# nellogrb/MultigridAnisotropicDiffusion

Measured on AMD Instinct MI355X. Metric: Mvoxel-smooths/s (and V-cycles/s) at 512^3 fp32; achieved HBM GB/s vs peak, higher is better.
Workload: dtype f32

## Files before the change

include/mad.h:

```cpp
#ifndef MAD_H
#define MAD_H

#include <stddef.h>
#include <stdint.h>

#ifdef __cplusplus
extern "C" {
#endif

#define MAD_ABI_VERSION 1

typedef enum mad_status {
  MAD_OK = 0,
  MAD_ERR_INVALID = 1,
  MAD_ERR_STATE = 2,
  MAD_ERR_DEVICE = 3,
  MAD_ERR_COMM = 4,
  MAD_ERR_SINGULAR = 5,
  MAD_ERR_UNSUPPORTED = 6,
  MAD_ERR_NOMEM = 7,
  MAD_ERR_NUMERIC = 8,
  MAD_ERR_NOT_CONVERGED = 9
} mad_status;

// ... 17 lines not shown
#define MAD_REFINE_SWITCH_RELRES 1e-5
#define MAD_REFINE_FP32_MIN_RATE 0.5
#define MAD_MIN_SLAB_PLANES 4
#define MAD_MIN_SLAB_VOXELS 131072
#define MAD_COARSE_DENSE_MAX 8192
#define MAD_COARSE_BLOCK_UNKNOWNS 2048
#define MAD_COARSE_DENSE_LIMIT 16384

typedef enum mad_tensor_kind {
  MAD_TENSOR_AUTO = 0,
  MAD_TENSOR_ISOTROPIC = 1,
  MAD_TENSOR_DIAGONAL = 2,
  MAD_TENSOR_FULL = 3
} mad_tensor_kind;

typedef enum mad_which { MAD_X = 0 , MAD_B = 1 , MAD_R = 2  } mad_which;

typedef struct mad_desc {
  uint32_t abi_version;
  int32_t dim;
  int64_t size[3];
  double spacing[3];
  int32_t cycle;
  int32_t smoother;
  uint32_t iterations_per_grid;
  uint32_t max_cycles;
  uint32_t number_of_steps;
  double time_step;
  double tolerance;
  double omega;
  int32_t verbose;
  int32_t precision;
  int32_t stall_guard;
  int32_t device;
  int32_t tensor_kind;
  int32_t nranks;
  int32_t rank;
  int32_t gs_kernel;
  uint32_t options;
  int32_t min_slab_planes;
  int32_t min_slab_voxels;
  int32_t coarse_dense_max;
  int32_t coarse_block_unknowns;
  int32_t reserved[3];
} mad_desc;

#define MAD_OPT_EAGER_RANK_VCYCLE 1u
#define MAD_OPT_OVERLAP_RANK_SWEEP 2u
#define MAD_OPT_PEER_HALO 4u
#define MAD_OPT_COARSE_NO_CHAIN 8u
#define MAD_OPT_BENCHMARK_TRACE 16u
#define MAD_OPT_NO_PLACEMENT_TUNE 32u
#define MAD_OPT_NO_RECORD_B 64u

typedef struct mad_stats {
  uint32_t steps;
  uint32_t total_cycles;
  uint32_t last_cycles;
  int32_t stalled;
  double last_relres;
  double setup_ms;
  double solve_ms;
  uint32_t num_levels;
  int32_t tensor_kind;
  int32_t colors;
  int32_t reserved[5];
} mad_stats;

typedef struct mad_ctx mad_ctx;

int mad_desc_init(mad_desc *d);
int mad_max_depth(int32_t dim, const int64_t size[3]);
int mad_create(const mad_desc *d, mad_ctx **out);
void mad_destroy(mad_ctx *ctx);
const char *mad_last_error(const mad_ctx *ctx);
int mad_get_desc(const mad_ctx *ctx, mad_desc *out);

int mad_set_tensor(mad_ctx *ctx, const void *host_aos, int32_t dtype);
int mad_set_tensor_device(mad_ctx *ctx, const void *dev_aos, int32_t dtype);
int mad_tensor_planes(const mad_ctx *ctx, int64_t *first_plane, int64_t *nplanes);
int mad_set_tensor_planes(mad_ctx *ctx, const void *host_aos, int32_t dtype,
                          int64_t first_plane, int64_t nplanes);

int mad_setup(mad_ctx *ctx);

int mad_run(mad_ctx *ctx, const void *host_in, int32_t in_dtype, void *host_out,
            int32_t out_dtype, mad_stats *stats);
int mad_run_device(mad_ctx *ctx, const void *dev_in, int32_t in_dtype, void *dev_out,
                   int32_t out_dtype, mad_stats *stats);
int mad_get_step_stats(const mad_ctx *ctx, uint32_t step, uint32_t *cycles, double *relres);
int mad_get_cycle_trace(const mad_ctx *ctx, uint32_t cap, uint32_t *step, double *relres,
                        double *seconds, uint32_t *count);
int mad_placement_trials(const mad_ctx *ctx, uint32_t cap, double *ms, uint32_t *count);

int mad_num_levels(const mad_ctx *ctx);
int mad_plan_level(const mad_desc *d, int32_t level, int64_t size[3], double spacing[3],
                   int32_t centering[3], int64_t *z_begin, int64_t *z_end,
                   int32_t *distributed);
int mad_level_info(const mad_ctx *ctx, int32_t level, int64_t size[3], double spacing[3],
                   int32_t centering[3]);

int mad_upload(mad_ctx *ctx, int32_t level, int32_t which, const double *host);
int mad_download(mad_ctx *ctx, int32_t level, int32_t which, double *host);
int mad_fill(mad_ctx *ctx, int32_t level, int32_t which, double value);
int mad_smooth(mad_ctx *ctx, int32_t level, uint32_t sweeps);
int mad_residual(mad_ctx *ctx, int32_t level, double *norm_out);
// ... 34 lines not shown
```

multigridanisotropicdiffusion_amd/_capi.py:

```python
import ctypes
import os

_HERE = os.path.dirname(os.path.abspath(__file__))
LIB_PATH = os.path.join(_HERE, "libmad_hip.so")

ABI_VERSION = 1

OK, ERR_INVALID, ERR_STATE, ERR_DEVICE, ERR_COMM, ERR_SINGULAR, ERR_UNSUPPORTED, ERR_NOMEM, \
    ERR_NUMERIC, ERR_NOT_CONVERGED = range(10)
VCYCLE, FMG, SMOOTHER = 0, 1, 2
GAUSS_SEIDEL, GAUSS_SEIDEL_LEX, WEIGHTED_JACOBI = 0, 1, 2
U8, I8, U16, I16, U32, I32, F32, F64 = range(8)
FP32, FP64, FP32_REFINE, PRECISION_AUTO = 0, 1, 2, 3
VED_HESSIAN_RECURSIVE, VED_HESSIAN_FIR = 0, 1
TENSOR_AUTO, TENSOR_ISOTROPIC, TENSOR_DIAGONAL, TENSOR_FULL = range(4)
X, B, R = 0, 1, 2
OPT_EAGER_RANK_VCYCLE = 1
OPT_OVERLAP_RANK_SWEEP = 2
OPT_PEER_HALO = 4
OPT_COARSE_NO_CHAIN = 8
OPT_BENCHMARK_TRACE = 16
OPT_NO_PLACEMENT_TUNE = 32
OPT_NO_RECORD_B = 64
VED_OPT_LINE_WALK = 1
CED_EED, CED_CED = 0, 1
PM_WEICKERT, PM_EXPONENTIAL, PM_RATIONAL = 0, 1, 2

EXPORTS = (
    "mad_desc_init", "mad_max_depth", "mad_create", "mad_destroy", "mad_last_error",
    "mad_get_desc", "mad_set_tensor", "mad_set_tensor_device", "mad_tensor_planes",
    "mad_set_tensor_planes", "mad_setup", "mad_run",
    "mad_run_device", "mad_get_step_stats", "mad_get_cycle_trace", "mad_placement_trials", "mad_num_levels", "mad_plan_level",
    "mad_level_info", "mad_upload",
    "mad_download", "mad_fill", "mad_smooth", "mad_residual", "mad_norm", "mad_restrict",
    "mad_residual_restrict",
    "mad_interpolate", "mad_prolongate_add", "mad_coarse_solve", "mad_vcycle", "mad_fmg",
    "mad_synchronize", "mad_bench_smooth", "mad_bench_launch_times", "mad_smooth_kernel_name", "mad_bench_vcycle", "mad_bench_synth_tensor",
    "mad_bench_synth_level", "mad_comm_unique_id", "mad_comm_init", "mad_comm_init_local", "mad_comm_init_solo",
    "mad_comm_init_rccl_solo",
    "mad_comm_selftest", "mad_slab_range", "mad_comm_allreduce_host", "mad_comm_version",
    "mad_ved_desc_init", "mad_ved_create", "mad_ved_destroy", "mad_ved_last_error",
    "mad_ved_run", "mad_ved_run_device", "mad_ved_comm_init", "mad_ved_comm_init_local",
    "mad_ved_comm_init_solo",
    "mad_ved_tensor", "mad_ved_hessian",
)

CED_EXPORTS = (
    "mad_ced_desc_init", "mad_ced_create", "mad_ced_destroy", "mad_ced_last_error",
    "mad_ced_run", "mad_ced_run_device", "mad_ced_tensor", "mad_ced_structure_tensor",
)

PM_EXPORTS = (
    "mad_pm_desc_init", "mad_pm_create", "mad_pm_destroy", "mad_pm_last_error",
    "mad_pm_run", "mad_pm_run_device", "mad_pm_tensor", "mad_pm_gradient",
)

VED_MAX_SCALES = 16


class MadDesc(ctypes.Structure):
    _fields_ = [
        ("abi_version", ctypes.c_uint32),
        ("dim", ctypes.c_int32),
        ("size", ctypes.c_int64 * 3),
        ("spacing", ctypes.c_double * 3),
        ("cycle", ctypes.c_int32),
        ("smoother", ctypes.c_int32),
        ("iterations_per_grid", ctypes.c_uint32),
        ("max_cycles", ctypes.c_uint32),
        ("number_of_steps", ctypes.c_uint32),
        ("time_step", ctypes.c_double),
        ("tolerance", ctypes.c_double),
        ("omega", ctypes.c_double),
        ("verbose", ctypes.c_int32),
        ("precision", ctypes.c_int32),
        ("stall_guard", ctypes.c_int32),
# ... 304 lines not shown
```

multigridanisotropicdiffusion_amd/csrc/mad_kernels.hpp:

```cpp
#pragma once
#include <hip/hip_runtime.h>

#include <climits>
#include <type_traits>
#include <cstdint>

namespace mad {

enum { KISO = 1, KDIAG = 2, KFULL = 3 };

template <int DIM, int KIND>
struct CoefLayout {
  static constexpr int NA = (KIND == KISO) ? 1 : DIM;
  static constexpr int NG = DIM;
  static constexpr int NE = (KIND == KFULL) ? DIM * (DIM - 1) / 2 : 0;
  static constexpr int N = NA + NG + NE;
};

inline int coef_count(int dim, int kind) {
  int na = (kind == KISO) ? 1 : dim;
  int ne = (kind == KFULL) ? dim * (dim - 1) / 2 : 0;
  return na + dim + ne;
}

// ... 248 lines not shown
#pragma unroll
    for (int q = 0; q < NW / 3; ++q) {
      auto v = __builtin_amdgcn_raw_buffer_load_b96(r, (int)voff, 12 * q, 0);
      w[3 * q] = v[0]; w[3 * q + 1] = v[1]; w[3 * q + 2] = v[2];
    }
  } else {
    int q = 0;
#pragma unroll
    for (; q + 4 <= NW; q += 4) {
      auto v = __builtin_amdgcn_raw_buffer_load_b128(r, (int)voff, 4 * q, 0);
      w[q] = v[0]; w[q + 1] = v[1]; w[q + 2] = v[2]; w[q + 3] = v[3];
    }
    if constexpr (NW % 4 == 3) {
      auto v = __builtin_amdgcn_raw_buffer_load_b96(r, (int)voff, 4 * (NW - 3), 0);
      w[NW - 3] = v[0]; w[NW - 2] = v[1]; w[NW - 1] = v[2];
    } else if constexpr (NW % 4 == 2) {
      auto v = __builtin_amdgcn_raw_buffer_load_b64(r, (int)voff, 4 * (NW - 2), 0);
      w[NW - 2] = v[0]; w[NW - 1] = v[1];
    } else if constexpr (NW % 4 == 1) {
      w[NW - 1] = __builtin_amdgcn_raw_buffer_load_b32(r, (int)voff, 4 * (NW - 1), 0);
    }
  }
  __builtin_memcpy(out, w, NB);
}

template <int NC, int TX, int TY>
struct FusedGeom {
  static constexpr int H = NC;
  static constexpr int RX = TX + 2 * H;
  static constexpr int RY = TY + 2 * H;
  static constexpr int HALF = ((RX / 2 + 15) / 32) * 32 + 16;
  static constexpr int PITCH = 2 * HALF + 1;
  static constexpr int PLANE = RY * PITCH;
  static constexpr int NP = NC + 2;
  static constexpr int rows(int c) { return (NC == 4) ? (TY + 2 * (NC - 1 - c)) / 2 : TY + 2 * (NC - 1 - c); }
  static constexpr int cols(int c) { return (TX + 2 * (NC - 1 - c)) / 2; }
};



template <typename T>
struct PeerOut {
  T* dst[2];
  uint32_t* sig[2];
};

template <typename T, int KIND, int TX, int TY, int NT, int MINW, int LEAD = 2, bool BREC = false,
          bool PEER = false, bool BL = false, bool ZU = false, bool BS = false>
__global__ void __launch_bounds__(NT, MINW) gs_fused3_k(const T* __restrict__ uin, T* __restrict__ uout,
                                                        const T* __restrict__ b, const T* __restrict__ cf,
                                                        Geo g, Rat<T> rat, int zc, int ntx, int nty,
                                                        int zbase, int zstride, int flip_last,
                                                        uint32_t* __restrict__ sig, PeerOut<T> po) {
  constexpr int NC = (KIND == KFULL) ? 4 : 2;
  using FG = FusedGeom<NC, TX, TY>;
  constexpr int H = FG::H, RX = FG::RX, RY = FG::RY, HALF = FG::HALF, PITCH = FG::PITCH;
  constexpr int PLANE = FG::PLANE, NP = FG::NP;
  constexpr int UPT = (RX * RY + NT - 1) / NT;
  constexpr int OPT = (TX * TY + NT - 1) / NT;
  constexpr int NCF = CoefLayout<3, KIND>::N;
  constexpr int RS = NCF + (BREC ? 1 : 0);
  constexpr uint32_t TS = sizeof(T);
  static_assert(TX % 2 == 0 && TY % 2 == 0 && (H % 2) == 0, "even tile geometry");
  static_assert(FG::rows(0) * FG::cols(0) <= NT, "one stage point per thread");
  static_assert(!(BL && BREC), "b rides in the record");
  static_assert(!(BS && (BL || BREC)), "one form of b");
  constexpr int NB = BL ? NC : 0;
  extern __shared__ __align__(16) unsigned char fused_smem[];

  int bid = blockIdx.x;
  {
    const int nb = gridDim.x, q = nb >> 3, r = nb & 7, xcd = bid & 7, idx = bid >> 3;
    bid = (xcd < r ? xcd * (q + 1) : r * (q + 1) + (xcd - r) * q) + idx;
  }
  const int tiles = ntx * nty;
  const int chunk = bid / tiles;
  const int tile = bid - chunk * tiles;
  const int tyi = tile / ntx;
  const int txi = tile - tyi * ntx;
  const int rx0 = txi * TX - H;
  const int ry0 = tyi * TY - H;
  const int tid = threadIdx.x;
  const int wbase = __builtin_amdgcn_readfirstlane(tid & ~63);
  auto wave_in = [&](int c) { return wbase < FG::rows(c) * FG::cols(c); };
  const int nx = g.nx, ny = g.ny;
  const int sy = (int)g.sy, hx0 = g.hx0;
  const bool interior = rx0 >= 2 && rx0 + RX <= nx - 2 && ry0 >= 2 && ry0 + RY <= ny - 2;

  const int p0 = zbase + chunk * zstride;
  const int p1 = min(p0 + zc, g.nz);
  const bool flip = flip_last != 0 && chunk == (int)(gridDim.x / tiles) - 1;
  int64_t sz = g.sz;
  int zlo_g = g.zlo_ghost, zhi_g = g.zhi_ghost, zpar = g.zoff;
  int z0 = p0, z1 = p1;
  if (flip) {
    const int64_t top = (int64_t)(g.nz - 1) * g.sz;
    uin += top;
    uout += top;
    b += top;
    cf += top * RS;
    sz = -g.sz;
    zlo_g = g.zhi_ghost;
    zhi_g = g.zlo_ghost;
    zpar = g.zoff + g.nz - 1;
    z0 = g.nz - p1;
    z1 = g.nz - p0;
  }
  const int zlo = zlo_g ? -GHOST : 0;
  const int zhi = zhi_g ? g.nz + GHOST : g.nz;
  const int ulo = zlo_g ? -(GHOST - 1) : 0;
  const int uhi = zhi_g ? g.nz + GHOST - 1 : g.nz;
  T* const pdst = PEER ? po.dst[flip ? 1 : 0] : nullptr;
  uint32_t* const psig = PEER ? po.sig[flip ? 1 : 0] : (sig ? sig + (flip ? 1 : 0) : nullptr);
  const bool signals = (PEER ? pdst != nullptr : sig != nullptr) && z0 == 0 && zlo_g;
  const int kbeg = (z0 - (NC - 1)) - ((z0 - (NC - 1) + zpar) & 1);
  const int kend = z1 + NC - 2;

  auto mirror = [](int v, int n) { return v < 0 ? min(-v, n - 1) : (v >= n ? max(2 * (n - 1) - v, 0) : v); };

  uint32_t usrc[UPT];
  int udst[UPT];
#pragma unroll
  for (int e = 0; e < UPT; ++e) {
    const int q = tid + e * NT;
    const int lj = q / RX, li = q - (q / RX) * RX;
    int gi = rx0 + li, gj = ry0 + lj;
    if (!interior) {
      gi = mirror(gi, nx);
      gj = mirror(gj, ny);
    }
    usrc[e] = (uint32_t)(gj * sy + gi) * TS;
    udst[e] = (q < RX * RY) ? (int)((lj * PITCH + (li & 1) * HALF + (li >> 1)) * TS) : -1;
  }
  int olds[OPT], oglb[OPT];
#pragma unroll
  for (int e = 0; e < OPT; ++e) {
    const int q = tid + e * NT;
    const int lj = H + q / TX, li = H + (q - (q / TX) * TX);
    const int gi = rx0 + li, gj = ry0 + lj;
    const bool ok = q < TX * TY && gi < nx && gj < ny;
    olds[e] = (int)((lj * PITCH + (li & 1) * HALF + (li >> 1)) * TS);
    oglb[e] = ok ? (int)((gj * sy + gi) * TS) : -1;
  }

  constexpr int NPM = (NC == 4) ? 1 : 2;
  uint32_t pl[NC][NPM], pg[NC][NPM], pb[NC][NPM];
  uint32_t vmask = 0, gmask = 0;
  uint32_t omask = 0;
#pragma unroll
  for (int c = 0; c < NC; ++c) {
    const int cols = FG::cols(c);
    const bool has = tid < FG::rows(c) * cols;
    const int r = has ? tid / cols : 0;
    const int t = has ? tid - (tid / cols) * cols : 0;
    const int l0 = c + 1;
#pragma unroll
    for (int PM = 0; PM < 2; ++PM) {
      int li, lj;
      if (NC == 4) {
        li = l0 + (1 ^ PM) + 2 * t;
        lj = l0 + (((c >> 1) ^ PM ^ l0) & 1) + 2 * r;
      } else {
        lj = l0 + r;
        li = l0 + ((c ^ PM ^ r) & 1) + 2 * t;
      }
      const int gi = rx0 + li, gj = ry0 + lj;
      const bool ok = has && gi >= 0 && gi < nx && gj >= 0 && gj < ny;
      vmask |= (ok ? 1u : 0u) << (c * 2 + PM);
      const uint32_t gb = (ok && gi == 1 ? 1u : 0u) | (ok && gi == nx - 2 ? 2u : 0u) |
                          (ok && gj == 1 ? 4u : 0u) | (ok && gj == ny - 2 ? 8u : 0u);
      gmask |= gb << (4 * (c * 2 + PM));
      omask |= (uint32_t)(li & 1) << (c * 2 + PM);
      if (PM < NPM) {
        pl[c][PM] = (uint32_t)(lj * PITCH + (li & 1) * HALF + (li >> 1)) * TS;
        pg[c][PM] = (uint32_t)(lj * sy + (li & 1) * hx0 + (li >> 1)) * (TS * RS);
        pb[c][PM] = (uint32_t)(lj * sy + li) * TS;
      }
    }
  }
  struct PD {
    int l;
    int64_t g, b;
  };
  auto pdelta = [&](int c, int PM) -> PD {
    if (NC != 4 || PM == 0) return PD{0, 0, 0};
    const int dy = 1 - 2 * (((c >> 1) ^ (c + 1)) & 1);
    const bool odd0 = (c & 1) != 0;
    return PD{dy * PITCH + (odd0 ? -HALF : HALF - 1), (int64_t)dy * sy + (odd0 ? -hx0 : hx0 - 1),
              (int64_t)dy * sy - 1};
  };
  const int64_t cbase = (int64_t)ry0 * sy + (rx0 >> 1);
  const int64_t bbase = (int64_t)ry0 * sy + rx0;

  auto slot = [](int m) { return (m + NP * 64) % NP; };
  auto plane_ok = [&](int m) { return m >= zlo && m < zhi; };
  auto stage_on = [&](int c, int m) {
    const int h = NC - 1 - c;
    return m >= z0 - h && m < z1 + h && m >= ulo && m < uhi;
  };
  unsigned char* lbytes = fused_smem;

  T up[UPT];
  T bp[BL ? UPT : 1];
  T raw[NC][RS];
  T bv[NC];
  auto bslot = [](int m) { return NP + (m + NB * 64) % (NB > 0 ? NB : 1); };
  auto load_bplane = [&](int m) {
    if constexpr (BL) {
      m = min(max(m, zlo), zhi - 1);
      const __amdgpu_buffer_rsrc_t rs = buf_rsrc(b + (int64_t)m * sz);
#pragma unroll
      for (int e = 0; e < UPT; ++e) bp[e] = buf_load<T>(rs, usrc[e], 0u);
    }
  };
  auto put_bplane = [&](int m) {
    if constexpr (BL) {
      unsigned char* P = lbytes + bslot(m) * (PLANE * TS);
#pragma unroll
      for (int e = 0; e < UPT; ++e) {
        if (e < UPT - 1 || udst[e] >= 0) *reinterpret_cast<T*>(P + udst[e]) = bp[e];
      }
    }
  };
  auto load_plane = [&](int m) {
    if constexpr (ZU) {
#pragma unroll
      for (int e = 0; e < UPT; ++e) up[e] = T(0);
    } else {
      m = min(max(m, zlo), zhi - 1);
      const __amdgpu_buffer_rsrc_t rs = buf_rsrc(uin + (int64_t)m * sz);
#pragma unroll
      for (int e = 0; e < UPT; ++e) up[e] = buf_load<T>(rs, usrc[e], 0u);
    }
  };
  auto put_plane = [&](int m) {
    unsigned char* P = lbytes + slot(m) * (PLANE * TS);
#pragma unroll
    for (int e = 0; e < UPT; ++e) {
      if (e < UPT - 1 || udst[e] >= 0) *reinterpret_cast<T*>(P + udst[e]) = up[e];
    }
  };
  auto load_stage = [&](int c, int k, int PM) {
    const int m = min(max(k - c, zlo), zhi - 1);
    {
      const PD d = pdelta(c, PM);
      buf_load_rec<T, RS>(buf_rsrc(cf + ((int64_t)m * sz + cbase + d.g) * RS), pg[c][PM % NPM],
                          raw[c]);
      if constexpr (BS)
        bv[c] = buf_load<T>(buf_rsrc(b + (int64_t)m * sz + cbase + d.g), pg[c][PM % NPM] / (uint32_t)RS, 0u);
      else if constexpr (!BREC && !BL)
        bv[c] = buf_load<T>(buf_rsrc(b + (int64_t)m * sz + bbase + d.b), pb[c][PM % NPM], 0u);
    }
  };
  auto stage = [&](int c, int k, int PM) {
    const int m = k - c;
    if (!stage_on(c, m) || !wave_in(c)) return;
    const int zm = (m == 0 && !zlo_g) ? 1 : m - 1;
    const int zp = (m == g.nz - 1 && !zhi_g) ? g.nz - 2 : m + 1;
    const uint32_t o = pl[c][PM % NPM] + (uint32_t)(pdelta(c, PM).l * (int)TS);
    unsigned char* A0 = lbytes + slot(m) * (PLANE * TS) + o;
    const unsigned char* Am = lbytes + slot(flip ? zp : zm) * (PLANE * TS) + o;
    const unsigned char* Ap = lbytes + slot(flip ? zm : zp) * (PLANE * TS) + o;
    bool odd;
    if (NC == 4) {
      odd = ((c + 1 + (1 ^ PM)) & 1) != 0;
    } else {
      odd = ((omask >> (c * 2 + PM)) & 1u) != 0;
    }
    const int ox_p = odd ? 1 - HALF : HALF;
    const int ox_m = odd ? -HALF : HALF - 1;
    auto rd = [](const unsigned char* p, int off) { return *reinterpret_cast<const T*>(p + off * (int)TS); };
    T nb[18];
    nb[0] = rd(A0, ox_p);
    nb[1] = rd(A0, ox_m);
    nb[2] = rd(A0, PITCH);
    nb[3] = rd(A0, -PITCH);
    nb[4] = rd(Ap, 0);
    nb[5] = rd(Am, 0);
    if (KIND == KFULL) {
      nb[6] = rd(A0, ox_p + PITCH);
      nb[7] = rd(A0, ox_p - PITCH);
      nb[8] = rd(A0, ox_m + PITCH);
      nb[9] = rd(A0, ox_m - PITCH);
      nb[10] = rd(Ap, ox_p);
      nb[11] = rd(Am, ox_p);
      nb[12] = rd(Ap, ox_m);
      nb[13] = rd(Am, ox_m);
      nb[14] = rd(Ap, PITCH);
      nb[15] = rd(Am, PITCH);
      nb[16] = rd(Ap, -PITCH);
      nb[17] = rd(Am, -PITCH);
    }
    Coefs<T> q;
    coefs_from_raw<T, 3, KIND>(raw[c], rat, q);
    T D, S;
    stencil_combine<T, 3, KIND>(q, nb, D, S);
    T bval;
    if constexpr (BREC)
      bval = raw[c][NCF];
    else if constexpr (BL)
      bval = *reinterpret_cast<const T*>(lbytes + bslot(m) * (PLANE * TS) + o);
    else
      bval = bv[c];
    const T v = gs_update(bval, S, D);
    const int bit = c * 2 + PM;
    if (interior) {
      if (NC == 2 || FG::rows(c) * FG::cols(c) < NT) {
        if ((vmask >> bit) & 1u) *reinterpret_cast<T*>(A0) = v;
      } else {
        *reinterpret_cast<T*>(A0) = v;
      }
    } else if ((vmask >> bit) & 1u) {
      *reinterpret_cast<T*>(A0) = v;
      const uint32_t gb = (gmask >> (4 * bit)) & 15u;
      if (gb) {
        const int xs[3] = {0, (gb & 1u) ? -1 : 0, (gb & 2u) ? 1 : 0};
        const int ys[3] = {0, (gb & 4u) ? -2 * PITCH : 0, (gb & 8u) ? 2 * PITCH : 0};
#pragma unroll
        for (int a = 0; a < 3; ++a)
#pragma unroll
          for (int bq = 0; bq < 3; ++bq) {
            if ((a == 0 && bq == 0) || (a > 0 && xs[a] == 0) || (bq > 0 && ys[bq] == 0)) continue;
            *reinterpret_cast<T*>(A0 + (xs[a] + ys[bq]) * (int)TS) = v;
          }
      }
    }
  };

  for (int m = kbeg - 1; m <= kbeg; ++m)
    if (plane_ok(m)) {
      load_plane(m);
      put_plane(m);
    }
  load_plane(kbeg + 1);
  load_bplane(kbeg);
#pragma unroll
  for (int c = 0; c < LEAD; ++c) load_stage(c, kbeg, c & 1);

  for (int k0 = kbeg; k0 <= kend; k0 += 2) {
#pragma unroll
    for (int u = 0; u < 2; ++u) {
      const int k = k0 + u;
      if (k <= kend) {
        asm volatile("" : "+v"(vmask), "+v"(gmask), "+v"(omask));
        if (plane_ok(k + 1)) put_plane(k + 1);
        load_plane(k + 2);
        put_bplane(k);
        load_bplane(k + 1);
        __syncthreads();
#pragma unroll
        for (int c = 0; c < NC; ++c) {
          stage(c, k, (u ^ c) & 1);
          {
            constexpr int L = LEAD < NC ? LEAD : NC;
            const int c2 = (c + L) % NC, dk = (c + L) / NC;
            load_stage(c2, k + dk, (u ^ dk ^ c2) & 1);
          }
          __syncthreads();
        }
        const int mo = k - NC + 1;
        if (mo >= z0 && mo < z1) {
          const unsigned char* P = lbytes + slot(mo) * (PLANE * TS);
          const __amdgpu_buffer_rsrc_t ro = buf_rsrc(uout + (int64_t)mo * sz);
#pragma unroll
          for (int e = 0; e < OPT; ++e)
            if (oglb[e] >= 0)
              buf_store<T>(*reinterpret_cast<const T*>(P + olds[e]), ro, (uint32_t)oglb[e]);
          if constexpr (PEER) {
            if (signals && mo < GHOST) {
              const __amdgpu_buffer_rsrc_t rp = buf_rsrc(pdst + (int64_t)mo * sz);
#pragma unroll
              for (int e = 0; e < OPT; ++e)
                if (oglb[e] >= 0)
                  buf_store<T>(*reinterpret_cast<const T*>(P + olds[e]), rp, (uint32_t)oglb[e]);
            }
          }
          if (signals && mo == GHOST - 1) {
            if (PEER) {
              __builtin_amdgcn_s_waitcnt(0);
              __syncthreads();
              if (tid == 0) __hip_atomic_fetch_add(psig, 1u, __ATOMIC_RELAXED, __HIP_MEMORY_SCOPE_SYSTEM);
            } else {
              __threadfence();
              __syncthreads();
              if (tid == 0) __hip_atomic_fetch_add(psig, 1u, __ATOMIC_RELEASE, __HIP_MEMORY_SCOPE_SYSTEM);
            }
          }
        }
      }
    }
  }
}

__device__ __forceinline__ uint32_t peer_pattern(int rank, int64_t e) {
  return (uint32_t)(rank + 1) * 1021u + (uint32_t)(e % 4093);
}
template <typename T>
__global__ void __launch_bounds__(256) peer_ping_k(PeerOut<T> po, int64_t ghost_n, int64_t top_off, int rank) {
  const int side = blockIdx.y;
  T* d = po.dst[side];
  if (!d) return;
  T* base = d - (side ? top_off : 0);
  const int64_t stride = (int64_t)gridDim.x * 256;
  for (int64_t e0 = (int64_t)blockIdx.x * 256; e0 < ghost_n; e0 += stride) {
    const int64_t e = e0 + threadIdx.x;
    const __amdgpu_buffer_rsrc_t r = buf_rsrc(base + e0);
    if (e < ghost_n) buf_store<T>((T)peer_pattern(rank, e), r, threadIdx.x * (uint32_t)sizeof(T));
  }
  __builtin_amdgcn_s_waitcnt(0);
  __syncthreads();
  if (threadIdx.x == 0) __hip_atomic_fetch_add(po.sig[side], 1u, __ATOMIC_RELAXED, __HIP_MEMORY_SCOPE_SYSTEM);
}

template <typename T>
__global__ void __launch_bounds__(256) peer_pong_k(const T* mlo, const T* mhi, const uint32_t* clo,
                                                   const uint32_t* chi, int rlo, int rhi, int64_t ghost_n,
                                                   uint32_t expect, uint32_t* okw, uint64_t tmo) {
  __shared__ int arrived;
  const int side = blockIdx.y;
  const T* m = side ? mhi : mlo;
  const uint32_t* cnt = side ? chi : clo;
  const int sender = side ? rhi : rlo;
  if (!m) return;
  if (threadIdx.x == 0) {
    int ok = 1;
    const uint64_t t0 = wall_clock64();
    while (__hip_atomic_load(cnt, __ATOMIC_ACQUIRE, __HIP_MEMORY_SCOPE_SYSTEM) < expect) {
      __builtin_amdgcn_s_sleep(2);
      if (wall_clock64() - t0 > tmo) {
        ok = 0;
        break;
      }
    }
    arrived = ok;
  }
  __syncthreads();
  bool bad = !arrived;
  if (arrived) {
    const int64_t stride = (int64_t)gridDim.x * 256;
    for (int64_t e = (int64_t)blockIdx.x * 256 + threadIdx.x; e < ghost_n; e += stride)
      bad |= m[e] != (T)peer_pattern(sender, e);
  }
  if (__syncthreads_or(bad) && threadIdx.x == 0) atomicAnd(okw, 0u);
}
// ... 88 lines not shown
__device__ __forceinline__ double block_sum(double v) {
  __shared__ double red[NT / 64];
  const int tid = threadIdx.x + blockDim.x * (threadIdx.y + blockDim.y * threadIdx.z);
  v = wave_sum(v);
  if ((tid & 63) == 0) red[tid >> 6] = v;
  __syncthreads();
  double s = 0.0;
  if (tid == 0) {
#pragma unroll
    for (int w = 0; w < NT / 64; ++w) s += red[w];
  }
  return s;
}

template <typename T, int DIM, int KIND>
__global__ void __launch_bounds__(256) wj_k(const T* __restrict__ u, T* __restrict__ uo,
                                            const T* __restrict__ b, const T* __restrict__ cf,
                                            Geo g, Rat<T> rat, T omega) {
  const int k = (DIM == 3) ? (int)blockIdx.z : 0;
  const int j = blockIdx.y * blockDim.y + threadIdx.y;
  const int i = blockIdx.x * blockDim.x + threadIdx.x;
  if (i >= g.nx || j >= g.ny) return;
  const int64_t p = i + g.sy * j + g.sz * k;
  T D, S;
  stencil_terms<T, DIM, KIND>(u, cf, g, rat, i, j, k, p, D, S);
  T v = (b[p] + S) * div_fast(omega, D);
  v += (T(1) - omega) * u[p];
  uo[p] = v;
}

template <typename T, int DIM, int KIND>
__global__ void __launch_bounds__(256) residual_k(const T* __restrict__ u, const T* __restrict__ b,
                                                  T* __restrict__ r, const T* __restrict__ cf,
                                                  Geo g, Rat<T> rat, double* __restrict__ part) {
  const int k = (DIM == 3) ? (int)blockIdx.z : 0;
  const int j = blockIdx.y * blockDim.y + threadIdx.y;
  const int i = blockIdx.x * blockDim.x + threadIdx.x;
  double sq = 0.0;
  if (i < g.nx && j < g.ny) {
    const int64_t p = i + g.sy * j + g.sz * k;
    T D, S;
    stencil_terms<T, DIM, KIND>(u, cf, g, rat, i, j, k, p, D, S);
    const T rv = resid_value(b[p], D, u[p], S);
    r[p] = rv;
    sq = (double)rv * (double)rv;
  }
  if (part) {
    const double s = block_sum<256>(sq);
    if (threadIdx.x == 0 && threadIdx.y == 0)
      part[blockIdx.x + gridDim.x * (blockIdx.y + gridDim.y * blockIdx.z)] = s;
  }
}

template <typename T, int KIND, int TX, int TY, bool BREC = false, typename TE = T, typename TB = T>
__global__ void __launch_bounds__(TX * TY) resid3_k(const T* __restrict__ u, const TB* __restrict__ b,
                                                    T* __restrict__ r, const T* __restrict__ cf,
                                                    Geo g, Rat<T> rat, int zc, int ntx,
                                                    double* __restrict__ part,
                                                    TE* __restrict__ be = nullptr,
                                                    TE* __restrict__ xe = nullptr,
                                                    const TE* __restrict__ ue = nullptr,
                                                    T* __restrict__ uo = nullptr,
                                                    TE* __restrict__ bse = nullptr) {
  constexpr int NT = TX * TY;
  constexpr int RX = TX + 2, RY = TY + 2, PL = RX * RY;
  constexpr int UPT = (PL + NT - 1) / NT;
  constexpr int NCF = CoefLayout<3, KIND>::N;
  constexpr int RS = NCF + (BREC ? 1 : 0);
  constexpr uint32_t TS = sizeof(T);
  __shared__ T ring[4 * PL];
  const int tiles_per_plane = ntx * ((g.ny + TY - 1) / TY);
  const int chunk = blockIdx.x / tiles_per_plane;
  const int tile = blockIdx.x - chunk * tiles_per_plane;
  const int tyi = tile / ntx, txi = tile - (tile / ntx) * ntx;
  const int x0 = txi * TX, y0 = tyi * TY;
  const int tid = threadIdx.x;
  const int tx = tid % TX, ty = tid / TX;
  const int nx = g.nx, ny = g.ny, sy = (int)g.sy, hx0 = g.hx0;
  const int64_t sz = g.sz;
  const int z0 = chunk * zc, z1 = min(z0 + zc, g.nz);
  const int zlo = g.zlo_ghost ? -1 : 0, zhi = g.zhi_ghost ? g.nz + 1 : g.nz;
  auto mirror = [](int v, int n) { return v < 0 ? min(-v, n - 1) : (v >= n ? max(2 * (n - 1) - v, 0) : v); };
  int u_dst[UPT];
  uint32_t u_src[UPT];
#pragma unroll
  for (int e = 0; e < UPT; ++e) {
    const int q = tid + e * NT;
    const int lj = q / RX, li = q - (q / RX) * RX;
    u_dst[e] = q < PL ? q : -1;
    u_src[e] = (uint32_t)(mirror(y0 - 1 + lj, ny) * sy + mirror(x0 - 1 + li, nx)) * TS;
  }
  const int i = x0 + tx, j = y0 + ty;
  const bool ok = i < nx && j < ny;
  const uint32_t rec_off = ok ? (uint32_t)(ty * sy + (tx & 1) * hx0 + (tx >> 1)) * (TS * RS) : 0u;
  const uint32_t pt_off = ok ? (uint32_t)(ty * sy + tx) * TS : 0u;
  const uint32_t pt_off_b = ok ? (uint32_t)(ty * sy + tx) * (uint32_t)sizeof(TB) : 0u;
  const int64_t rbase = (int64_t)y0 * sy + (x0 >> 1), pbase = (int64_t)y0 * sy + x0;
  const int il = (ty + 1) * RX + (tx + 1);
  constexpr int oyp = RX, oym = -RX;

  T up[UPT];
  T raw[RS];
  T bv = T(0);
  auto load_plane = [&](int m) {
    m = min(max(m, zlo), zhi - 1);
    const __amdgpu_buffer_rsrc_t rs = buf_rsrc(u + (int64_t)m * sz);
#pragma unroll
    for (int e = 0; e < UPT; ++e) up[e] = buf_load<T>(rs, u_src[e], 0u);
    if (ue) {
      const __amdgpu_buffer_rsrc_t re = buf_rsrc(ue + (int64_t)m * sz);
#pragma unroll
      for (int e = 0; e < UPT; ++e)
        up[e] = up[e] + (T)buf_load<TE>(re, (u_src[e] / TS) * (uint32_t)sizeof(TE), 0u);
    }
  };
  auto put_plane = [&](int m) {
    T* P = ring + (m & 3) * PL;
#pragma unroll
    for (int e = 0; e < UPT; ++e)
      if (e < UPT - 1 || u_dst[e] >= 0) P[u_dst[e]] = up[e];
  };
  auto load_pt = [&](int m) {
    m = min(max(m, 0), g.nz - 1);
    buf_load_rec<T, RS>(buf_rsrc(cf + ((int64_t)m * sz + rbase) * RS), rec_off, raw);
    if constexpr (!BREC) bv = (T)buf_load<TB>(buf_rsrc(b + (int64_t)m * sz + pbase), pt_off_b, 0u);
  };

  if (z0 - 1 >= zlo) {
    load_plane(z0 - 1);
    put_plane(z0 - 1);
  }
  load_plane(z0);
  put_plane(z0);
  load_plane(z0 + 1);
  load_pt(z0);
  double sq = 0.0;
  for (int m = z0; m < z1; ++m) {
    if (m + 1 < zhi) put_plane(m + 1);
    load_plane(m + 2);
    __syncthreads();
    const int zm = (m == 0 && !g.zlo_ghost) ? m + 1 : m - 1;
    const int zp = (m == g.nz - 1 && !g.zhi_ghost) ? m - 1 : m + 1;
    const T* P0 = ring + (m & 3) * PL + il;
    const T* Pm = ring + (zm & 3) * PL + il;
    const T* Pp = ring + (zp & 3) * PL + il;
    T nb[18];
    nb[0] = P0[1];
    nb[1] = P0[-1];
    nb[2] = P0[oyp];
    nb[3] = P0[oym];
    nb[4] = Pp[0];
    nb[5] = Pm[0];
    if (KIND == KFULL) {
      nb[6] = P0[1 + oyp];
      nb[7] = P0[1 + oym];
      nb[8] = P0[-1 + oyp];
      nb[9] = P0[-1 + oym];
      nb[10] = Pp[1];
      nb[11] = Pm[1];
      nb[12] = Pp[-1];
      nb[13] = Pm[-1];
      nb[14] = Pp[oyp];
      nb[15] = Pm[oyp];
      nb[16] = Pp[oym];
      nb[17] = Pm[oym];
    }
    Coefs<T> q;
    coefs_from_raw<T, 3, KIND>(raw, rat, q);
    T D, S;
    stencil_combine<T, 3, KIND>(q, nb, D, S);
    const T rv = resid_value(BREC ? raw[NCF] : bv, D, P0[0], S);
    load_pt(m + 1);
    if (ok) {
      if (r) buf_store<T>(rv, buf_rsrc(r + (int64_t)m * sz + pbase), pt_off);
      if (be) {
        const int64_t p = (int64_t)m * sz + pbase + ty * sy + tx;
        be[p] = (TE)rv;
        if (bse) bse[(int64_t)m * sz + rbase + rec_off / (TS * RS)] = (TE)rv;
        if (xe) xe[p] = TE(0);
        if (uo) uo[p] = P0[0];
      }
      sq += (double)rv * (double)rv;
    }
  }
  if (part) {
    const double s = block_sum<NT>(sq);
    if (tid == 0) part[blockIdx.x] = s;
  }
}

template <typename T, int KIND, int TX, int TY, bool BREC = false>
__global__ void __launch_bounds__(TX * TY) wj3_k(const T* __restrict__ u, T* __restrict__ uo,
                                                 const T* __restrict__ b, const T* __restrict__ cf,
                                                 Geo g, Rat<T> rat, T omega, int zc, int ntx) {
  constexpr int NT = TX * TY;
  constexpr int RX = TX + 2, RY = TY + 2, PL = RX * RY;
  constexpr int UPT = (PL + NT - 1) / NT;
  constexpr int NCF = CoefLayout<3, KIND>::N;
  constexpr int RS = NCF + (BREC ? 1 : 0);
  constexpr uint32_t TS = sizeof(T);
  __shared__ T ring[4 * PL];
  const int tiles_per_plane = ntx * ((g.ny + TY - 1) / TY);
  const int chunk = blockIdx.x / tiles_per_plane;
  const int tile = blockIdx.x - chunk * tiles_per_plane;
  const int tyi = tile / ntx, txi = tile - (tile / ntx) * ntx;
  const int x0 = txi * TX, y0 = tyi * TY;
  const int tid = threadIdx.x;
  const int tx = tid % TX, ty = tid / TX;
  const int nx = g.nx, ny = g.ny, sy = (int)g.sy, hx0 = g.hx0;
  const int64_t sz = g.sz;
  const int z0 = chunk * zc, z1 = min(z0 + zc, g.nz);
  const int zlo = g.zlo_ghost ? -1 : 0, zhi = g.zhi_ghost ? g.nz + 1 : g.nz;
  auto mirror = [](int v, int n) { return v < 0 ? min(-v, n - 1) : (v >= n ? max(2 * (n - 1) - v, 0) : v); };
  int u_dst[UPT];
  uint32_t u_src[UPT];
#pragma unroll
  for (int e = 0; e < UPT; ++e) {
    const int q = tid + e * NT;
    const int lj = q / RX, li = q - (q / RX) * RX;
    u_dst[e] = q < PL ? q : -1;
    u_src[e] = (uint32_t)(mirror(y0 - 1 + lj, ny) * sy + mirror(x0 - 1 + li, nx)) * TS;
  }
  const int i = x0 + tx, j = y0 + ty;
  const bool ok = i < nx && j < ny;
  const uint32_t rec_off = ok ? (uint32_t)(ty * sy + (tx & 1) * hx0 + (tx >> 1)) * (TS * RS) : 0u;
  const uint32_t pt_off = ok ? (uint32_t)(ty * sy + tx) * TS : 0u;
  const int64_t rbase = (int64_t)y0 * sy + (x0 >> 1), pbase = (int64_t)y0 * sy + x0;
  const int il = (ty + 1) * RX + (tx + 1);
  constexpr int oyp = RX, oym = -RX;

  T up[UPT];
  T raw[RS];
  T bv = T(0);
  auto load_plane = [&](int m) {
    m = min(max(m, zlo), zhi - 1);
    const __amdgpu_buffer_rsrc_t rs = buf_rsrc(u + (int64_t)m * sz);
#pragma unroll
    for (int e = 0; e < UPT; ++e) up[e] = buf_load<T>(rs, u_src[e], 0u);
// ... 192 lines not shown
  rtaps4<A>(min(J, gc.ny - 1), gc.ny, cy, iy, wy);
  int src_off[EPT];
#pragma unroll
  for (int q = 0; q < EPT; ++q) {
    const int e = min(tid + q * NT, FP - 1);
    const int ly = e / FX, lx = e - (e / FX) * FX;
    src_off[q] = min(max(fy0 + ly, 0), gf.ny - 1) * (int)gf.sy + min(max(fx0 + lx, 0), gf.nx - 1);
  }
  const int K0 = chunk * kc, K1 = min(K0 + kc, gc.nz);
  int iz[4];
  A wz[4];
  rtaps4<A>(K0 + gc.zoff, ncz, cz, iz, wz);
  const int f_lo = iz[0];
  rtaps4<A>(K1 - 1 + gc.zoff, ncz, cz, iz, wz);
  const int f_hi = max(max(iz[0], iz[1]), max(iz[2], iz[3]));
  T reg[EPT];
  auto fetch = [&](int f) {
    const T* src = fine + gf.sz * (int64_t)(f - fz_shift);
#pragma unroll
    for (int q = 0; q < EPT; ++q) reg[q] = src[src_off[q]];
  };
  A win[4];
  int K = K0;
  rtaps4<A>(K + gc.zoff, ncz, cz, iz, wz);
  fetch(f_lo);
  for (int f = f_lo; f <= f_hi; ++f) {
    __syncthreads();
#pragma unroll
    for (int q = 0; q < EPT; ++q)
      if (tid + q * NT < FP) tile[tid + q * NT] = reg[q];
    if (f < f_hi) fetch(f + 1);
    __syncthreads();
    A vz = A(0);
#pragma unroll
    for (int bq = 0; bq < 4; ++bq) {
      const T* row = tile + (iy[bq] - fy0) * FX - fx0;
      A vy = A(0);
#pragma unroll
      for (int a = 0; a < 4; ++a) vy = fma(wx[a], (A)row[ix[a]], vy);
      vz = fma(wy[bq], vy, vz);
    }
    win[f & 3] = vz;
    while (K < K1 && max(max(iz[0], iz[1]), max(iz[2], iz[3])) == f) {
      A v = A(0);
#pragma unroll
      for (int c = 0; c < 4; ++c) v = fma(wz[c], win[iz[c] & 3], v);
      if (ok) coarse[I + gc.sy * J + gc.sz * (int64_t)K] = (T)v;
      ++K;
      if (K < K1) rtaps4<A>(K + gc.zoff, ncz, cz, iz, wz);
    }
  }
}

template <typename T, int KIND, int CX, int CY, int NT, bool BREC = false>
__global__ void __launch_bounds__(NT) resid_restrict3_k(
    const T* __restrict__ u, const T* __restrict__ b, const T* __restrict__ cf, Geo gf, Rat<T> rat,
    T* __restrict__ coarse, T* __restrict__ zx, Geo gc, int cx, int cy, int cz, int kc, int ntx,
    int fzs, int ncz) {
  static_assert(CX * CY <= NT, "one coarse point per thread");
  constexpr int FX = 2 * CX + 2, FY = 2 * CY + 2, FP = FX * FY;
  constexpr int UX = FX + 2, UY = FY + 2, UP = UX * UY;
  constexpr int UPT = (UP + NT - 1) / NT;
  constexpr int RPT = (FP + NT - 1) / NT;
  constexpr int NCF = CoefLayout<3, KIND>::N;
  constexpr int RS = NCF + (BREC ? 1 : 0);
  constexpr uint32_t TS = sizeof(T);
  __shared__ T ring[4 * UP];
  __shared__ T rt[FP];
  const int tiles = ntx * ((gc.ny + CY - 1) / CY);
  const int chunk = blockIdx.x / tiles;
  const int t = blockIdx.x - chunk * tiles;
  const int tyi = t / ntx, txi = t - (t / ntx) * ntx;
  const int I0 = txi * CX, J0 = tyi * CY;
  const int tid = threadIdx.x;
  const int nx = gf.nx, ny = gf.ny, nz = gf.nz, sy = (int)gf.sy, hx0 = gf.hx0;
  const int64_t sz = gf.sz;
  const int fx0 = 2 * I0 - 1, fy0 = 2 * J0 - 1;
  const int ux0 = fx0 - 1, uy0 = fy0 - 1;
  auto mirror = [](int v, int n) { return v < 0 ? min(-v, n - 1) : (v >= n ? max(2 * (n - 1) - v, 0) : v); };
  const bool cthr = tid < CX * CY;
  const int I = I0 + tid % CX, J = J0 + (tid / CX) % CY;
  const bool ok = cthr && I < gc.nx && J < gc.ny;
  int ix[4], iy[4];
  T wx[4], wy[4];
  rtaps4<T>(min(I, gc.nx - 1), gc.nx, cx, ix, wx);
  rtaps4<T>(min(J, gc.ny - 1), gc.ny, cy, iy, wy);
  int u_dst[UPT];
  uint32_t u_src[UPT];
#pragma unroll
  for (int e = 0; e < UPT; ++e) {
    const int q = tid + e * NT;
    const int lj = min(q, UP - 1) / UX, li = min(q, UP - 1) - (min(q, UP - 1) / UX) * UX;
    u_dst[e] = q < UP ? q : -1;
    u_src[e] = (uint32_t)(mirror(uy0 + lj, ny) * sy + mirror(ux0 + li, nx)) * TS;
  }
  int r_il[RPT];
  uint32_t r_rec[RPT], r_pt[RPT];
#pragma unroll
  for (int e = 0; e < RPT; ++e) {
    const int q = min(tid + e * NT, FP - 1);
    const int ry = q / FX, rx = q - (q / FX) * FX;
    const int xf = min(max(fx0 + rx, 0), nx - 1), yf = min(max(fy0 + ry, 0), ny - 1);
    r_il[e] = (yf - uy0) * UX + (xf - ux0);
    r_rec[e] = (uint32_t)(yf * sy + (xf & 1) * hx0 + (xf >> 1)) * (TS * RS);
    r_pt[e] = (uint32_t)(yf * sy + xf) * TS;
  }
  const int K0 = chunk * kc, K1 = min(K0 + kc, gc.nz);
  int iz[4];
  T wz[4];
  auto ztaps = [&](int Kl) {
    rtaps4<T>(Kl + gc.zoff, ncz, cz, iz, wz);
#pragma unroll
    for (int c = 0; c < 4; ++c) iz[c] -= fzs;
  };
  ztaps(K0);
  const int f_lo = iz[0];
  ztaps(K1 - 1);
  const int f_hi = max(max(iz[0], iz[1]), max(iz[2], iz[3]));
  const int ulo = gf.zlo_ghost ? -2 : 0, uhi = gf.zhi_ghost ? nz + 2 : nz;

  T up[UPT];
  T raw[RPT][RS];
  T bv[RPT];
  auto load_plane = [&](int m) {
    m = min(max(m, ulo), uhi - 1);
    const __amdgpu_buffer_rsrc_t rs = buf_rsrc(u + (int64_t)m * sz);
#pragma unroll
    for (int e = 0; e < UPT; ++e) up[e] = buf_load<T>(rs, u_src[e], 0u);
  };
  auto put_plane = [&](int m) {
    T* P = ring + (m & 3) * UP;
#pragma unroll
    for (int e = 0; e < UPT; ++e)
      if (u_dst[e] >= 0) P[u_dst[e]] = up[e];
  };
  const int wbase = __builtin_amdgcn_readfirstlane(tid & ~63);
  auto wave_in = [&](int e) { return wbase + e * NT < FP; };
  auto load_pts = [&](int m) {
    m = min(max(m, ulo), uhi - 1);
    const __amdgpu_buffer_rsrc_t rr = buf_rsrc(cf + (int64_t)m * sz * RS);
    const __amdgpu_buffer_rsrc_t rb = buf_rsrc(b + (int64_t)m * sz);
#pragma unroll
    for (int e = 0; e < RPT; ++e) {
      if (e > 0 && !wave_in(e)) continue;
      buf_load_rec<T, RS>(rr, r_rec[e], raw[e]);
      if constexpr (!BREC) bv[e] = buf_load<T>(rb, r_pt[e], 0u);
    }
  };

  if (f_lo - 1 >= ulo) {
    load_plane(f_lo - 1);
    put_plane(f_lo - 1);
  }
  load_plane(f_lo);
  put_plane(f_lo);
  load_plane(f_lo + 1);
  load_pts(f_lo);
  T win[4];
  int K = K0;
  ztaps(K);
  for (int f = f_lo; f <= f_hi; ++f) {
    if (f + 1 < uhi) put_plane(f + 1);
    load_plane(f + 2);
    __syncthreads();
    const int zm = (f == 0 && !gf.zlo_ghost) ? f + 1 : f - 1;
    const int zp = (f == nz - 1 && !gf.zhi_ghost) ? f - 1 : f + 1;
#pragma unroll
    for (int e = 0; e < RPT; ++e) {
      if (e > 0 && !wave_in(e)) continue;
      const T* P0 = ring + (f & 3) * UP + r_il[e];
      const T* Pm = ring + (zm & 3) * UP + r_il[e];
      const T* Pp = ring + (zp & 3) * UP + r_il[e];
      T nb[18];
      nb[0] = P0[1];
      nb[1] = P0[-1];
      nb[2] = P0[UX];
      nb[3] = P0[-UX];
      nb[4] = Pp[0];
      nb[5] = Pm[0];
      if (KIND == KFULL) {
        nb[6] = P0[1 + UX];
        nb[7] = P0[1 - UX];
        nb[8] = P0[-1 + UX];
        nb[9] = P0[-1 - UX];
        nb[10] = Pp[1];
        nb[11] = Pm[1];
        nb[12] = Pp[-1];
        nb[13] = Pm[-1];
        nb[14] = Pp[UX];
        nb[15] = Pm[UX];
        nb[16] = Pp[-UX];
        nb[17] = Pm[-UX];
      }
      Coefs<T> q;
      coefs_from_raw<T, 3, KIND>(raw[e], rat, q);
      T D, S;
      stencil_combine<T, 3, KIND>(q, nb, D, S);
      const T rv = resid_value(BREC ? raw[e][NCF] : bv[e], D, P0[0], S);
      if (tid + e * NT < FP) rt[tid + e * NT] = rv;
    }
    if (f < f_hi) load_pts(f + 1);
    __syncthreads();
    {
#pragma clang fp contract(off)
      T vz = T(0);
#pragma unroll
      for (int bq = 0; bq < 4; ++bq) {
        const T* row = rt + (iy[bq] - fy0) * FX - fx0;
        T vy = T(0);
#pragma unroll
        for (int a = 0; a < 4; ++a) vy = fma(wx[a], row[ix[a]], vy);
        vz = fma(wy[bq], vy, vz);
      }
      win[f & 3] = vz;
      while (K < K1 && max(max(iz[0], iz[1]), max(iz[2], iz[3])) == f) {
        T v = T(0);
#pragma unroll
        for (int c = 0; c < 4; ++c) v = fma(wz[c], win[iz[c] & 3], v);
        if (ok) {
          const int64_t o = I + gc.sy * J + gc.sz * (int64_t)K;
          coarse[o] = v;
          if (zx) {
            zx[o] = T(0);
            if (K == 0 && gc.zlo_ghost) {
#pragma unroll
              for (int g = 1; g <= GHOST; ++g) zx[o - gc.sz * (int64_t)g] = T(0);
            }
            if (K == gc.nz - 1 && gc.zhi_ghost) {
#pragma unroll
              for (int g = 1; g <= GHOST; ++g) zx[o + gc.sz * (int64_t)g] = T(0);
            }
          }
        }
        ++K;
        if (K < K1) ztaps(K);
      }
    }
  }
}

template <typename T, int V>
struct alignas(sizeof(T) * V) VecT {
  T v[V];
};
template <typename T, int ADD, int TX, int TY, int G = 8, int VX = 1>
__global__ void __launch_bounds__(TX * TY) interp3_k(const T* __restrict__ coarse, Geo gc,
                                                     T* __restrict__ fine, Geo gf, int cx, int cy,
                                                     int cz, int ncz, int kc, int ntx, int kbase,
                                                     int kend) {
#pragma clang fp contract(off)
  constexpr int NT = TX * TY;
  constexpr int FX = TX * VX;
// ... 475 lines not shown
```

multigridanisotropicdiffusion_amd/csrc/mad_solver.hip:

```cpp
#include <hip/hip_runtime.h>
#include <rocblas/rocblas.h>
#include <rocsolver/rocsolver.h>

#include <algorithm>
#include <chrono>
#include <cmath>
#include <cstdio>
#include <cstdlib>
#include <cstring>
#include <memory>
#include <mutex>
#include <stdexcept>
#include <string>
#include <thread>
#include <type_traits>
#include <vector>

#include "../../include/mad.h"
#include "mad_alloc.hpp"
#include "mad_coarse.hpp"
#include "mad_comm.hpp"
#include "mad_kernels.hpp"

using namespace mad;
// ... 239 lines not shown
  virtual void bench_vcycle(unsigned n, double* total_ms) = 0;
  virtual void synth_level(int l, int which, uint64_t seed) = 0;
  virtual std::string smooth_kernel(int l) = 0;
  virtual std::vector<double> placement_ms() const { return {}; }
};

mad_ctx::~mad_ctx() {
  solver.reset();
  if (tensor64) (void)hipFree(tensor64);
  comm.destroy();
  if (stream) (void)hipStreamDestroy(stream);
  if (comm_stream) (void)hipStreamDestroy(comm_stream);
}

namespace {

template <typename T>
struct LevelData {
  Geo g{};
  int cent[3] = {0, 0, 0};
  T* alloc[4] = {nullptr, nullptr, nullptr, nullptr};
  T* x = nullptr;
  T* b = nullptr;
  T* r = nullptr;
  T* t = nullptr;
  T* cf = nullptr;
  T* cf_alloc = nullptr;
  T* bs = nullptr;
  T* bs_alloc = nullptr;
  Rat<T> rat{};
  int64_t ghost = 0;
  bool b_halo_ok = false;
  bool brec = false;
  bool brec_ok = false;
  bool x_halo_ok = false;
  bool x_halo_pending = false;
  hipEvent_t ev_bnd = nullptr;
  hipEvent_t ev_halo = nullptr;
  uint32_t* sig = nullptr;
  uint32_t sig_epoch = 0;
  T* phys[2] = {nullptr, nullptr};
  char* win = nullptr;
  char* win_lo = nullptr;
  char* win_hi = nullptr;
  bool win_ipc = false;
  bool peer = false;
  bool x_peer_pending = false;
  uint32_t peer_tiles = 0;
  bool peer_pc = false;
  int peer_seq = 0;
  int peer_buf = 0;
  bool b_peer_pending = false;
  bool x_zero_lazy = false;
};
constexpr int BOUNDARY_PLANES = 8;
#ifndef MAD_FUSED_B_SPLIT
#define MAD_FUSED_B_SPLIT 1
#endif
inline int boundary_planes() { return BOUNDARY_PLANES; }

template <typename T>
class Solver final : public SolverBase {
 public:
  ~Solver() override { release(); }

  void setup(mad_ctx* c) override {
    c_ = c;
    release();
    const int dim = c->dim;
    const int nl = c->nlev;
    lv_.resize(nl);
    ncoef_ = coef_count(dim, c->kind);
    int64_t part_need = 1;
    for (int l = 0; l < nl; ++l) {
      const LevelGeom& G = c->geom[l];
      LevelData<T>& L = lv_[l];
      L.g.nx = (int)G.n[0];
      L.g.ny = (int)G.n[1];
      L.g.nz = (int)(G.z1 - G.z0);
      L.g.zoff = (int)G.z0;
      L.g.zlo_ghost = (G.distributed && G.z0 > 0) ? 1 : 0;
      L.g.zhi_ghost = (G.distributed && G.z1 < G.n[2]) ? 1 : 0;
      L.g.sy = G.n[0];
      L.g.sz = G.n[0] * G.n[1];
      L.g.N = L.g.sz * L.g.nz;
      L.g.hx0 = (L.g.nx + 1) / 2;
      for (int d = 0; d < 3; ++d) L.cent[d] = G.cent[d];
      L.rat.r[0] = T(1);
      L.rat.r[1] = (T)((G.h[0] * G.h[0]) / (G.h[1] * G.h[1]));
      L.rat.r[2] = (T)((G.h[0] * G.h[0]) / (G.h[2] * G.h[2]));
      L.ghost = (dim == 3) ? (int64_t)GHOST * L.g.sz : 0;
      const int64_t margin = margin_elems(L.g);
      const int64_t tot = L.g.N + 2 * (L.ghost + margin);
      bool brec_on = c->d.cycle == MAD_SMOOTHER && !(c->d.options & MAD_OPT_NO_RECORD_B);
      if (c->d.precision == MAD_FP32_REFINE) brec_on = false;
      L.brec = (dim == 3 && l == 0 && brec_on);
      L.g.rs = ncoef_ + (L.brec ? 1 : 0);
      const int64_t cplane = L.g.sz * L.g.rs;
      const int64_t cgp = (dim == 3) ? GHOST : 0;
      const int64_t cmargin = margin * L.g.rs;
      const int64_t ctot = (L.g.nz + 2 * cgp) * cplane + 2 * cmargin;
      for (int a = 0; a < 4; ++a) {
        level_alloc((void**)&L.alloc[a], sizeof(T) * tot);
        HIP_CHECK(hipMemsetAsync(L.alloc[a], 0, sizeof(T) * tot, c->stream));
      }
      level_alloc((void**)&L.cf_alloc, sizeof(T) * ctot);
// ... 311 lines not shown
    L.x_peer_pending = false;
    const int buf = L.peer_buf;
    if (c_->comm.mode() == Comm::LOCAL) c_->comm.local_barrier(c_->stream);
    const size_t bytes = (size_t)L.ghost * sizeof(T);
    char* dlo = L.g.zlo_ghost ? (char*)(L.x - L.ghost) : nullptr;
    char* dhi = L.g.zhi_ghost ? (char*)(L.x + (int64_t)L.g.nz * L.g.sz) : nullptr;
    const unsigned blocks = (unsigned)std::min<size_t>(64, std::max<size_t>(1, (bytes / 16 + 255) / 256));
    hipLaunchKernelGGL(peer_unpack_k, dim3(blocks, 2), dim3(256), 0, c_->stream, dlo,
                       (const char*)mailbox(L.win, L, buf, 0), dhi, (const char*)mailbox(L.win, L, buf, 1),
                       (uint64_t)bytes, peer_ctl(L.win, L), buf * 2, L.peer_tiles, peer_timeout_ticks_);
    HIP_CHECK(hipGetLastError());
  }
  void peer_resolve_all() {
    for (size_t l = 0; l < lv_.size(); ++l) {
      peer_resolve((int)l);
      peer_resolve_b((int)l);
    }
  }
  void peer_resolve_b(int l) {
    LevelData<T>& L = lv_[l];
    if (!L.b_peer_pending) return;
    L.b_peer_pending = false;
    if (c_->comm.mode() == Comm::LOCAL) c_->comm.local_barrier(c_->stream);
    const size_t bytes = (size_t)L.ghost * sizeof(T);
    char* dlo = L.g.zlo_ghost ? (char*)(L.b - L.ghost) : nullptr;
    char* dhi = L.g.zhi_ghost ? (char*)(L.b + (int64_t)L.g.nz * L.g.sz) : nullptr;
    const unsigned blocks = push_blocks(L);
    hipLaunchKernelGGL(peer_unpack_k, dim3(blocks, 2), dim3(256), 0, c_->stream, dlo,
                       (const char*)mailbox(L.win, L, 2, 0), dhi, (const char*)mailbox(L.win, L, 2, 1),
                       (uint64_t)bytes, peer_ctl(L.win, L), 8, blocks, peer_timeout_ticks_);
    HIP_CHECK(hipGetLastError());
  }
  void peer_push_b(int l) {
    LevelData<T>& L = lv_[l];
    const int64_t top_off = (int64_t)(L.g.nz - GHOST) * L.g.sz;
    hipLaunchKernelGGL((peer_push_k<T>), dim3(push_blocks(L), 2), dim3(256), 0, c_->stream, L.b, top_off,
                       peer_out(L, 2), (int64_t)L.ghost, (int64_t)(GHOST - 1) * L.g.sz);
    HIP_CHECK(hipGetLastError());
    L.b_halo_ok = true;
    L.b_peer_pending = true;
  }
  void b_halo(int l) {
    LevelData<T>& L = lv_[l];
    if (L.b_peer_pending) peer_resolve_b(l);
    if (!L.b_halo_ok) {
      halo(l, L.b, GHOST);
      L.b_halo_ok = true;
    }
  }
  void b_changed(int l) {
    LevelData<T>& L = lv_[l];
    if (L.b_peer_pending) peer_resolve_b(l);
    L.b_halo_ok = L.brec_ok = false;
  }
  static uint32_t push_blocks(const LevelData<T>& L) {
    const size_t bytes = (size_t)L.ghost * sizeof(T);
    return (uint32_t)std::min<size_t>(64, std::max<size_t>(1, (bytes / 16 + 255) / 256));
  }
  void peer_push(int l) {
    LevelData<T>& L = lv_[l];
    const int buf = L.peer_seq & 1;
    ++L.peer_seq;
    const int64_t top_off = (int64_t)(L.g.nz - GHOST) * L.g.sz;
    hipLaunchKernelGGL((peer_push_k<T>), dim3(push_blocks(L), 2), dim3(256), 0, c_->stream, L.x, top_off,
                       peer_out(L, buf), (int64_t)L.ghost, (int64_t)(GHOST - 1) * L.g.sz);
    HIP_CHECK(hipGetLastError());
    L.peer_buf = buf;
    L.x_halo_ok = true;
    L.x_peer_pending = true;
  }
  void check_device_errors() override { peer_check(); }
  void peer_check() {
    for (auto& L : lv_) {
      if (!L.win) continue;
      uint32_t err = 0;
      HIP_CHECK(hipMemcpyAsync(&err, peer_ctl(L.win, L) + 5, sizeof err, hipMemcpyDeviceToHost, c_->stream));
      HIP_CHECK(hipStreamSynchronize(c_->stream));
      if (err) throw CommError("peer halo: a neighbour's edge planes never arrived (wait timed out)");
    }
  }

  T* arr(int l, int which) {
    LevelData<T>& L = lv_[l];
    if (which == MAD_X) return L.x;
    if (which == MAD_B) return L.b;
    return L.r;
  }

  void upload(int l, int which, const double* h) override {
    LevelData<T>& L = lv_[l];
    if (which == MAD_B) b_changed(l);
    if (which == MAD_X) x_changed(l);
    double* tmp = scratch64(L.g.N);
    HIP_CHECK(hipMemcpyAsync(tmp, h, sizeof(double) * L.g.N, hipMemcpyHostToDevice, c_->stream));
    hipLaunchKernelGGL((convert_k<double, T>), dim3(flat_blocks(L.g.N)), dim3(256), 0, c_->stream,
                       tmp, arr(l, which), L.g.N);
    HIP_CHECK(hipGetLastError());
    HIP_CHECK(hipStreamSynchronize(c_->stream));
  }

  void download(int l, int which, double* h) override {
    peer_check();
    LevelData<T>& L = lv_[l];
    double* tmp = scratch64(L.g.N);
    hipLaunchKernelGGL((convert_k<T, double>), dim3(flat_blocks(L.g.N)), dim3(256), 0, c_->stream,
                       arr(l, which), tmp, L.g.N);
    HIP_CHECK(hipGetLastError());
    HIP_CHECK(hipMemcpyAsync(h, tmp, sizeof(double) * L.g.N, hipMemcpyDeviceToHost, c_->stream));
    HIP_CHECK(hipStreamSynchronize(c_->stream));
  }

  void fill(int l, int which, double v) override {
    LevelData<T>& L = lv_[l];
    if (which == MAD_B) b_changed(l);
    if (which == MAD_X) x_changed(l);
    hipLaunchKernelGGL((fill_k<T>), dim3(flat_blocks(L.g.N)), dim3(256), 0, c_->stream, arr(l, which),
                       L.g.N, (T)v);
    HIP_CHECK(hipGetLastError());
  }

  void synth_level(int l, int which, uint64_t seed) override {
    LevelData<T>& L = lv_[l];
    if (which == MAD_B) b_changed(l);
    if (which == MAD_X) x_changed(l);
    const LevelGeom& G = c_->geom[l];
    hipLaunchKernelGGL((synth_image_k<T>), grid_for(L.g.nx, L.g.ny, L.g.nz, BLK), BLK, 0, c_->stream,
                       arr(l, which), L.g, G.n[0], G.n[1], seed);
    HIP_CHECK(hipGetLastError());
  }

  void wait_all_pending() {
    for (auto& L : lv_)
      if (L.x_halo_pending) {
        HIP_CHECK(hipStreamWaitEvent(c_->stream, L.ev_halo, 0));
        L.x_halo_pending = false;
      }
  }

  void halo(int l, T* a, int depth = 1) {
    if (!c_->comm.active() || !c_->geom[l].distributed) return;
    LevelData<T>& L = lv_[l];
    if (a == L.x && L.x_peer_pending) peer_resolve(l);
    wait_all_pending();
    if (a == L.x && L.x_halo_ok && depth <= GHOST) return;
    c_->comm.exchange_planes(a, L.g.sz, L.g.nz, depth, L.g.zlo_ghost, L.g.zhi_ghost, sizeof(T),
                             std::is_same<T, double>::value, c_->stream);
    if (a == L.x && depth == GHOST) L.x_halo_ok = true;
  }

  void x_changed(int l) {
    if (lv_[l].x_peer_pending) peer_resolve(l);
    lv_[l].x_halo_ok = false;
    lv_[l].x_zero_lazy = false;
  }

  static constexpr int XFER_BLOCKS = 1024;
  static int xfer_blocks() { return XFER_BLOCKS; }

  static int64_t margin_elems(const Geo& g) { return 48 * g.sy + 512; }

  bool use_fused(int l) const {
    const int v = c_->d.gs_kernel;
    if (c_->dim != 3 || c_->d.smoother != MAD_GAUSS_SEIDEL) return false;
    if (v == 1) return false;
    if (v >= 2) return true;
    const Geo& g = lv_[l].g;
#ifndef MAD_FUSED_RANK_MIN_VOXELS
#define MAD_FUSED_RANK_MIN_VOXELS ((int64_t)4 << 20)
#define MAD_FUSED_RANK_MIN_PLANES 64
#endif
    if (c_->geom[l].distributed)
      return (int64_t)g.nx * g.ny * g.nz >= (int64_t)MAD_FUSED_RANK_MIN_VOXELS && g.nz >= MAD_FUSED_RANK_MIN_PLANES;
    return (int64_t)g.nx * g.ny * g.nz >= (int64_t)4 << 20 && g.nz >= 64;
  }

  struct FusedCfg {
    int blocks = 256;
  };
#ifndef MAD_FUSED_BLOCKS
#define MAD_FUSED_BLOCKS 256
#endif
  static FusedCfg fused_cfg() {
    FusedCfg f;
    f.blocks = MAD_FUSED_BLOCKS;
    return f;
  }

  struct ZRange {
    int zbase, zc, zstride, nchunks;
  };
  static ZRange whole_range(int nz, int tiles, const FusedCfg& fc) {
    int chunks = (fc.blocks + tiles - 1) / tiles;
    chunks = std::max(1, std::min(chunks, std::max(1, nz / 16)));
    const int zc = (nz + chunks - 1) / chunks;
    return ZRange{0, zc, zc, (nz + zc - 1) / zc};
  }

  ZRange part_range(LevelData<T>& L, int tiles, const FusedCfg& fc, int part, int* flip,
                    uint32_t** sig) {
    const int nz = L.g.nz;
    ZRange zr = whole_range(nz, tiles, fc);
    *flip = (c_->d.gs_kernel == 4 && part == 0) ? 1 : 0;
    *sig = nullptr;
    if (part == 3 || part == 4) {
      REQUIRE(zr.nchunks >= 2 && zr.zc >= GHOST, MAD_ERR_UNSUPPORTED, "slab too thin for the single-launch sweep");
      *flip = 1;
      *sig = part == 3 ? L.sig : nullptr;
    } else if (part == 1) {
      zr = ZRange{0, boundary_planes(), nz - boundary_planes(), 2};
    } else if (part == 2) {
      const int ni = nz - 2 * boundary_planes();
      int chunks = std::max(1, std::min((fc.blocks + tiles - 1) / tiles, std::max(1, ni / 16)));
      const int zc = (ni + chunks - 1) / chunks;
      zr = ZRange{boundary_planes(), zc, zc, (ni + zc - 1) / zc};
    }
    return zr;
  }

  template <int KD, int TX, int TY, int NT>
  void launch_fused(LevelData<T>& L, const FusedCfg& fc, int part, bool zu = false) {
    const int ntx = (L.g.nx + TX - 1) / TX, nty = (L.g.ny + TY - 1) / TY;
    const int tiles = ntx * nty;
    int flip = 0;
    uint32_t* sig = nullptr;
    const ZRange zr = part_range(L, tiles, fc, part, &flip, &sig);
    const unsigned nb = (unsigned)(tiles * zr.nchunks);
    constexpr int NC = (KD == KFULL) ? 4 : 2;
    using FG = FusedGeom<NC, TX, TY>;
    constexpr size_t lds_u = sizeof(T) * FG::NP * FG::PLANE;
    REQUIRE(lds_u <= 160 * 1024, MAD_ERR_UNSUPPORTED,
            "fused GS tile needs " + std::to_string(lds_u) + " B of LDS (> 160 KiB)");
    constexpr size_t lds_bl = sizeof(T) * (FG::NP + NC) * FG::PLANE;
    constexpr bool bl_fits = lds_bl <= 160 * 1024;
    const bool bl = fused_b_lds(L);
    const size_t lds = bl ? lds_bl : lds_u;
    constexpr int MW = sizeof(T) == 8 ? 2 : 4;
    const PeerOut<T> po = part == 4 ? peer_out(L, buffer_index(L, L.t)) : PeerOut<T>{{nullptr, nullptr}, {nullptr, nullptr}};
    auto run = [&](auto kern) {
      {
        static std::mutex attr_mu;
        static std::vector<const void*> attr;
        std::lock_guard<std::mutex> lk(attr_mu);
        if (std::find(attr.begin(), attr.end(), (const void*)kern) == attr.end()) {
          HIP_CHECK(hipFuncSetAttribute((const void*)kern, hipFuncAttributeMaxDynamicSharedMemorySize,
                                        (int)lds));
          attr.push_back((const void*)kern);
        }
      }
      hipLaunchKernelGGL(kern, dim3(nb), dim3(NT), lds, c_->stream, L.x, L.t, L.bs ? L.bs : L.b, L.cf, L.g,
                         L.rat, zr.zc, ntx, nty, zr.zbase, zr.zstride, flip, sig, po);
    };
    if (part == 4) {
      if (L.brec)
        run(gs_fused3_k<T, KD, TX, TY, NT, MW, 2, true, true>);
      else if constexpr (bl_fits) {
        if (L.bs)
          run(gs_fused3_k<T, KD, TX, TY, NT, MW, 2, false, true, false, false, true>);
        else
          bl ? run(gs_fused3_k<T, KD, TX, TY, NT, MW, 2, false, true, true>)
             : run(gs_fused3_k<T, KD, TX, TY, NT, MW, 2, false, true>);
      } else
        run(gs_fused3_k<T, KD, TX, TY, NT, MW, 2, false, true>);
    } else if (L.brec) {
      run(gs_fused3_k<T, KD, TX, TY, NT, MW, 2, true>);
    } else if constexpr (bl_fits) {
      if (zu) {
        REQUIRE(part == 0, MAD_ERR_STATE, "zero-iterate sweep on a rank slab");
        if (L.bs)
          run(gs_fused3_k<T, KD, TX, TY, NT, MW, 2, false, false, false, true, true>);
        else
          bl ? run(gs_fused3_k<T, KD, TX, TY, NT, MW, 2, false, false, true, true>)
             : run(gs_fused3_k<T, KD, TX, TY, NT, MW, 2, false, false, false, true>);
      } else if (L.bs) {
        run(gs_fused3_k<T, KD, TX, TY, NT, MW, 2, false, false, false, false, true>);
      } else {
        bl ? run(gs_fused3_k<T, KD, TX, TY, NT, MW, 2, false, false, true>)
           : run(gs_fused3_k<T, KD, TX, TY, NT, MW, 2>);
      }
    } else {
      REQUIRE(!zu, MAD_ERR_STATE, "zero-iterate sweep without its instance");
      run(gs_fused3_k<T, KD, TX, TY, NT, MW, 2>);
    }
  }

#ifndef MAD_FUSED_B_LDS
#define MAD_FUSED_B_LDS 1
#endif
  bool fused_b_lds(const LevelData<T>& L) const {
    return MAD_FUSED_B_LDS && sizeof(T) == 4 && !L.brec && !L.bs && &L == &lv_[0];
  }

#ifndef MAD_FUSED_F32_TY
#define MAD_FUSED_F32_TY 32
#endif
  void fused_shape(const LevelData<T>& L, int* tiles, int* nchunks) const {
    const FusedCfg fc = fused_cfg();
    const int tx = 64, ty = (c_->kind == KFULL && sizeof(T) == 4) ? MAD_FUSED_F32_TY : 16;
    *tiles = ((L.g.nx + tx - 1) / tx) * ((L.g.ny + ty - 1) / ty);
    *nchunks = whole_range(L.g.nz, *tiles, fc).nchunks;
  }

  void launch_fused_part(LevelData<T>& L, int part, bool zu = false) {
    const FusedCfg fc = fused_cfg();
    if (c_->kind == KFULL) {
      if constexpr (sizeof(T) == 4)
        launch_fused<KFULL, 64, MAD_FUSED_F32_TY, MAD_FUSED_F32_TY * 32>(L, fc, part, zu);
      else
        launch_fused<KFULL, 64, 16, 512>(L, fc, part, zu);
    } else if (c_->kind == KDIAG) {
      launch_fused<KDIAG, 64, 16, 1024>(L, fc, part, zu);
    } else {
      launch_fused<KISO, 64, 16, 1024>(L, fc, part, zu);
    }
    HIP_CHECK(hipGetLastError());
  }

  std::string smooth_kernel(int l) override {
    (void)l;
    const char* tn = sizeof(T) == 4 ? "float" : "double";
    const int dim = c_->dim, kind = c_->kind;
    char buf[160];
    if (c_->d.smoother == MAD_WEIGHTED_JACOBI) {
      const LevelData<T>& L = lv_[l];
      if (dim == 3 && L.g.nx >= 16 && L.g.ny >= 16)
        std::snprintf(buf, sizeof buf, "wj3_k<%s, %d, 64, 16, %s>", tn, kind, L.brec ? "true" : "false");
      else
        std::snprintf(buf, sizeof buf, "wj_k<%s, %d, %d>", tn, dim, kind);
    } else if (c_->d.smoother == MAD_GAUSS_SEIDEL_LEX) {
      std::snprintf(buf, sizeof buf, "gs_lex_plane_k<%s, %d, %d>", tn, dim, kind);
    } else if (!use_fused(l)) {
      std::snprintf(buf, sizeof buf, "gs_color_k<%s, %d, %d>", tn, dim, kind);
      if (lv_[l].peer) return std::string(buf) + " [rank slab: peer halo, edge planes pushed after the last colour pass]";
    } else {
      const int tx = 64, ty = (kind == KFULL && sizeof(T) == 4) ? MAD_FUSED_F32_TY : 16;
      const int nt = (kind == KFULL && sizeof(T) == 8) ? 512 : (kind == KFULL ? MAD_FUSED_F32_TY * 32 : 1024);
      const bool brec = lv_[l].brec;
      const LevelData<T>& L = lv_[l];
      std::snprintf(buf, sizeof buf, "gs_fused3_k<%s, %d, %d, %d, %d, %d, 2, %s, %s, %s, false, %s>", tn, kind, tx,
                    ty, nt, sizeof(T) == 8 ? 2 : 4, brec ? "true" : "false", L.peer ? "true" : "false",
                    fused_b_lds(L) ? "true" : "false", L.bs ? "true" : "false");
      if (L.peer) return std::string(buf) + " [rank slab: peer halo, edge planes stored by the sweep]";
      if (sweep_overlap(l)) {
        int tiles = 0, nchunks = 0;
        fused_shape(L, &tiles, &nchunks);
        const bool single = L.sig && nchunks >= 2;
        return std::string(buf) + (single ? " [rank slab: single launch, edge signals]"
                                          : " [rank slab: boundary + interior launches]");
      }
    }
    return buf;
  }

  void sync_brec(int l) {
    LevelData<T>& L = lv_[l];
    if (!L.brec || L.brec_ok) return;
    int p0 = 0, p1 = L.g.nz;
    if (c_->comm.active() && c_->geom[l].distributed) {
      if (!L.b_halo_ok) {
        halo(l, L.b, GHOST);
        L.b_halo_ok = true;
      }
      if (L.g.zlo_ghost) p0 = -GHOST;
      if (L.g.zhi_ghost) p1 = L.g.nz + GHOST;
    }
    dim3 gr = grid_for(L.g.nx, L.g.ny, p1 - p0, BLK);
    hipLaunchKernelGGL((brec_scatter_k<T>), gr, BLK, 0, c_->stream, L.b, L.cf, L.g, ncoef_, p0);
    HIP_CHECK(hipGetLastError());
    L.brec_ok = true;
  }
  void sync_bsplit(int l) {
    LevelData<T>& L = lv_[l];
    if (!L.bs || L.brec_ok) return;
    int p0 = 0, p1 = L.g.nz;
    if (c_->comm.active() && c_->geom[l].distributed) {
      b_halo(l);
      if (L.g.zlo_ghost) p0 = -GHOST;
      if (L.g.zhi_ghost) p1 = L.g.nz + GHOST;
    }
    dim3 gr = grid_for(L.g.nx, L.g.ny, p1 - p0, BLK);
    hipLaunchKernelGGL((bsplit_k<T>), gr, BLK, 0, c_->stream, L.b, L.bs, L.g, p0);
    HIP_CHECK(hipGetLastError());
    L.brec_ok = true;
  }

  bool sweep_overlap(int l) const {
    const LevelData<T>& L = lv_[l];
    if (!(c_->comm.active() && c_->geom[l].distributed && L.g.nz >= 3 * boundary_planes()))
      return false;
    if (c_->d.gs_kernel == 4) return true;
    if (!(c_->d.options & MAD_OPT_OVERLAP_RANK_SWEEP)) return false;
    if (c_->d.gs_kernel != 0) return true;
    int tiles = 0, nchunks = 0;
    fused_shape(L, &tiles, &nchunks);
    return 2 * tiles >= 128;
  }

  float fused_sweep(int l, hipEvent_t e0 = nullptr, hipEvent_t e1 = nullptr) {
    LevelData<T>& L = lv_[l];
    halo(l, L.x, GHOST);
    if (L.brec) {
      sync_brec(l);
    } else {
      b_halo(l);
      sync_bsplit(l);
    }
    if (e0) HIP_CHECK(hipEventRecord(e0, c_->stream));
    if (L.peer) {
      L.peer_buf = buffer_index(L, L.t);
      launch_fused_part(L, 4);
      if (e1) HIP_CHECK(hipEventRecord(e1, c_->stream));
      std::swap(L.x, L.t);
      std::swap(L.alloc[0], L.alloc[3]);
      L.x_halo_ok = true;
      L.x_peer_pending = true;
      return 0.f;
    }
    const bool overlap = sweep_overlap(l);
    int tiles = 0, nchunks = 0;
    if (overlap) fused_shape(L, &tiles, &nchunks);
    if (overlap && L.sig && nchunks >= 2) {
      launch_fused_part(L, 3);
      wait_all_pending();
      const uint32_t target = ++L.sig_epoch * (uint32_t)tiles;
      if (L.g.zlo_ghost)
        HIP_CHECK(hipStreamWaitValue32(c_->comm_stream, L.sig, target, hipStreamWaitValueGte, 0xFFFFFFFFu));
      if (L.g.zhi_ghost)
        HIP_CHECK(hipStreamWaitValue32(c_->comm_stream, L.sig + 1, target, hipStreamWaitValueGte,
                                       0xFFFFFFFFu));
      c_->comm.exchange_planes(L.t, L.g.sz, L.g.nz, GHOST, L.g.zlo_ghost, L.g.zhi_ghost, sizeof(T),
                               std::is_same<T, double>::value, c_->comm_stream);
      HIP_CHECK(hipEventRecord(L.ev_halo, c_->comm_stream));
    } else if (!overlap) {
      const bool zu = (zero_x0_ && &L == &lv_[0]) || L.x_zero_lazy;
      zero_x0_ = false;
      L.x_zero_lazy = false;
      launch_fused_part(L, 0, zu);
    } else {
      launch_fused_part(L, 1);
      wait_all_pending();
      HIP_CHECK(hipEventRecord(L.ev_bnd, c_->stream));
      HIP_CHECK(hipStreamWaitEvent(c_->comm_stream, L.ev_bnd, 0));
      c_->comm.exchange_planes(L.t, L.g.sz, L.g.nz, GHOST, L.g.zlo_ghost, L.g.zhi_ghost, sizeof(T),
                               std::is_same<T, double>::value, c_->comm_stream);
      HIP_CHECK(hipEventRecord(L.ev_halo, c_->comm_stream));
      launch_fused_part(L, 2);
    }
    if (e1) HIP_CHECK(hipEventRecord(e1, c_->stream));
    std::swap(L.x, L.t);
    std::swap(L.alloc[0], L.alloc[3]);
    if (overlap) {
      L.x_halo_ok = true;
      L.x_halo_pending = true;
    } else {
      L.x_halo_ok = false;
    }
    return 0.f;
  }

  void prep_wj(int l) {
    LevelData<T>& L = lv_[l];
    halo(l, L.x);
    if (L.brec) sync_brec(l);
  }
  void launch_wj(int l) {
    LevelData<T>& L = lv_[l];
    const T omega = (T)c_->d.omega;
    if (c_->dim == 3 && L.g.nx >= 16 && L.g.ny >= 16) {
      constexpr int TX = 64, TY = 16;
      const int ntx = (L.g.nx + TX - 1) / TX, nty = (L.g.ny + TY - 1) / TY;
      int chunks = std::max(1, std::min((1024 + ntx * nty - 1) / (ntx * nty), L.g.nz / 8));
      const int zc = (L.g.nz + chunks - 1) / chunks;
      chunks = (L.g.nz + zc - 1) / zc;
      const unsigned nb = (unsigned)(ntx * nty * chunks);
      auto go = [&](auto K) {
        constexpr int KD = decltype(K)::value;
        if (L.brec)
          hipLaunchKernelGGL((wj3_k<T, KD, TX, TY, true>), dim3(nb), dim3(TX * TY), 0, c_->stream,
                             L.x, L.t, L.b, L.cf, L.g, L.rat, omega, zc, ntx);
        else
          hipLaunchKernelGGL((wj3_k<T, KD, TX, TY>), dim3(nb), dim3(TX * TY), 0, c_->stream, L.x,
                             L.t, L.b, L.cf, L.g, L.rat, omega, zc, ntx);
      };
      if (c_->kind == KFULL) go(std::integral_constant<int, KFULL>{});
      else if (c_->kind == KDIAG) go(std::integral_constant<int, KDIAG>{});
      else go(std::integral_constant<int, KISO>{});
    } else {
      dispatch(c_->dim, c_->kind, [&](auto D, auto K) {
        hipLaunchKernelGGL((wj_k<T, D.value, K.value>), grid_for(L.g.nx, L.g.ny, L.g.nz, BLK), BLK,
                           0, c_->stream, L.x, L.t, L.b, L.cf, L.g, L.rat, omega);
      });
    }
    HIP_CHECK(hipGetLastError());
  }

  bool colour_ca(int l) const {
    return c_->dim == 3 && c_->comm.active() && c_->geom[l].distributed &&
           c_->ncolors <= GHOST;
  }

  void smooth(int l, unsigned n) override {
    LevelData<T>& L = lv_[l];
    const int dim = c_->dim;
    const int sm = c_->d.smoother;
    for (unsigned s = 0; s < n; ++s) {
      if (sm == MAD_WEIGHTED_JACOBI) {
        prep_wj(l);
        launch_wj(l);
        std::swap(L.x, L.t);
        std::swap(L.alloc[0], L.alloc[3]);
        x_changed(l);
      } else if (sm == MAD_GAUSS_SEIDEL_LEX) {
        REQUIRE(!c_->comm.active(), MAD_ERR_UNSUPPORTED,
                "lexicographic GS is a single-GPU parity mode");
        const int tmax = (L.g.nx - 1) + 2 * (L.g.ny - 1) + (dim == 3 ? 3 * (L.g.nz - 1) : 0);
        dim3 gr((unsigned)((L.g.ny + 255) / 256), (unsigned)(dim == 3 ? L.g.nz : 1), 1);
        for (int t = 0; t <= tmax; ++t) {
          dispatch(dim, c_->kind, [&](auto D, auto K) {
            hipLaunchKernelGGL((gs_lex_plane_k<T, D.value, K.value>), gr, dim3(256), 0, c_->stream,
                               L.x, L.b, L.cf, L.g, L.rat, t);
          });
        }
        HIP_CHECK(hipGetLastError());
      } else if (use_fused(l)) {
        fused_sweep(l);
      } else {
        const int nc = c_->ncolors;
        const int rows = (nc == 4) ? (L.g.ny + 1) / 2 : L.g.ny;
        if (colour_ca(l)) {
          halo(l, L.x, nc);
          b_halo(l);
          for (int col = 0; col < nc; ++col) {
            const int ext = nc - 1 - col;
            const int k0 = L.g.zlo_ghost ? -ext : 0, k1 = L.g.nz + (L.g.zhi_ghost ? ext : 0);
            dim3 gr = grid_for((L.g.nx + 1) / 2, rows, k1 - k0, BLK);
            dispatch(dim, c_->kind, [&](auto D, auto K) {
              hipLaunchKernelGGL((gs_color_k<T, D.value, K.value>), gr, BLK, 0, c_->stream, L.x, L.b,
                                 L.cf, L.g, L.rat, col, nc, k0);
            });
          }
          if (L.peer)
            peer_push(l);
          else
            x_changed(l);
        } else {
          dim3 gr = grid_for((L.g.nx + 1) / 2, rows, L.g.nz, BLK);
          for (int col = 0; col < nc; ++col) {
            halo(l, L.x);
            dispatch(dim, c_->kind, [&](auto D, auto K) {
              hipLaunchKernelGGL((gs_color_k<T, D.value, K.value>), gr, BLK, 0, c_->stream, L.x,
                                 L.b, L.cf, L.g, L.rat, col, nc, 0);
            });
            x_changed(l);
          }
        }
        HIP_CHECK(hipGetLastError());
      }
    }
  }

  double finish_norm2(int64_t nparts, bool global) {
    hipLaunchKernelGGL(reduce_final_k, dim3(1), dim3(256), 0, c_->stream, part_, nparts, scal_);
    HIP_CHECK(hipGetLastError());
    if (global && c_->comm.active()) {
      wait_all_pending();
      c_->comm.allreduce_sum_f64(scal_, 1, c_->stream);
    }
    HIP_CHECK(hipMemcpyAsync(hscal_, scal_, sizeof(double), hipMemcpyDeviceToHost, c_->stream));
    HIP_CHECK(hipStreamSynchronize(c_->stream));
    return hscal_[0];
  }

  double residual(int l, bool want_norm) override { return residual_impl(l, want_norm, true); }

  bool refine_emitted_ = false;
  bool refine_emitted_bs_ = false;
  bool refine_fold_ok() const {
    const LevelData<T>& L = lv_[0];
// ... 61 lines not shown
#ifdef MAD_NO_B32_RHS
        launch((const double*)b64_);
#else
        if (b32_exact_)
          launch((const float*)b32_);
        else
          launch((const double*)b64_);
#endif
      };
      refine_emitted_ = true;
      if (c_->kind == KFULL) go(std::integral_constant<int, KFULL>{});
      else if (c_->kind == KDIAG) go(std::integral_constant<int, KDIAG>{});
      else go(std::integral_constant<int, KISO>{});
      if (fold) {
        std::swap(u64_, r64_);
        if (!zero_sweep_ok())
          hipLaunchKernelGGL((fill_k<T>), dim3(flat_blocks(L.g.N)), dim3(256), 0, c_->stream, L.x, L.g.N, T(0));
      }
    } else {
      dim3 gr = grid_for(g.nx, g.ny, g.nz, BLK);
      nparts = (int64_t)gr.x * gr.y * gr.z;
      REQUIRE(nparts <= part_cap_, MAD_ERR_UNSUPPORTED, "residual partials buffer too small");
      dispatch(c_->dim, c_->kind, [&](auto D, auto K) {
        hipLaunchKernelGGL((residual_k<double, D.value, K.value>), gr, BLK, 0, c_->stream, u64_, b64_,
                           r64_, cf64_, g, rat64_, part_);
      });
      refine_emitted_ = refine_emitted_bs_ = false;
    }
    HIP_CHECK(hipGetLastError());
    return std::sqrt(finish_norm2(nparts, c_->geom[0].distributed));
  }

  double norm64(const double* a) {
    const int64_t n = lv_[0].g.N;
    unsigned nb = flat_blocks(n, 2048);
    hipLaunchKernelGGL((sumsq_k<double>), dim3(nb), dim3(256), 0, c_->stream, a, n, part_);
    HIP_CHECK(hipGetLastError());
    return std::sqrt(finish_norm2(nb, c_->geom[0].distributed));
  }

  double residual_impl(int l, bool want_norm, bool write_r) {
    LevelData<T>& L = lv_[l];
    halo(l, L.x);
    int64_t nparts = 0;
    if (c_->dim == 3 && L.g.nx >= 16 && L.g.ny >= 16) {
      constexpr int TX = 64, TY = 16;
      const int ntx = (L.g.nx + TX - 1) / TX, nty = (L.g.ny + TY - 1) / TY;
      int chunks = std::max(1, std::min((1024 + ntx * nty - 1) / (ntx * nty), L.g.nz / 8));
      const int zc = (L.g.nz + chunks - 1) / chunks;
      chunks = (L.g.nz + zc - 1) / zc;
      nparts = (int64_t)ntx * nty * chunks;
      REQUIRE(nparts <= part_cap_, MAD_ERR_UNSUPPORTED, "residual partials buffer too small");
      sync_brec(l);
      auto go = [&](auto K) {
        constexpr int KD = decltype(K)::value;
        T* rout = write_r ? L.r : nullptr;
        if (L.brec)
          hipLaunchKernelGGL((resid3_k<T, KD, TX, TY, true>), dim3((unsigned)nparts),
                             dim3(TX * TY), 0, c_->stream, L.x, L.b, rout, L.cf, L.g, L.rat, zc, ntx,
                             want_norm ? part_ : nullptr);
        else
          hipLaunchKernelGGL((resid3_k<T, KD, TX, TY>), dim3((unsigned)nparts), dim3(TX * TY), 0,
                             c_->stream, L.x, L.b, rout, L.cf, L.g, L.rat, zc, ntx,
                             want_norm ? part_ : nullptr);
      };
      if (c_->kind == KFULL) go(std::integral_constant<int, KFULL>{});
      else if (c_->kind == KDIAG) go(std::integral_constant<int, KDIAG>{});
      else go(std::integral_constant<int, KISO>{});
    } else {
      dim3 gr = grid_for(L.g.nx, L.g.ny, L.g.nz, BLK);
      nparts = (int64_t)gr.x * gr.y * gr.z;
      dispatch(c_->dim, c_->kind, [&](auto D, auto K) {
        hipLaunchKernelGGL((residual_k<T, D.value, K.value>), gr, BLK, 0, c_->stream, L.x, L.b,
                           L.r, L.cf, L.g, L.rat, want_norm ? part_ : nullptr);
      });
    }
    HIP_CHECK(hipGetLastError());
    if (!want_norm) return 0.0;
    return std::sqrt(finish_norm2(nparts, c_->geom[l].distributed));
  }

  double norm(int l, int which) override {
    LevelData<T>& L = lv_[l];
    unsigned nb = flat_blocks(L.g.N, 2048);
    hipLaunchKernelGGL((sumsq_k<T>), dim3(nb), dim3(256), 0, c_->stream, arr(l, which), L.g.N, part_);
    HIP_CHECK(hipGetLastError());
    return std::sqrt(finish_norm2(nb, c_->geom[l].distributed));
  }

  void restrict_(int l) override { restrict_arr(l, lv_[l].r, lv_[l + 1].b); }

  bool residual_restrict(int l) override { return resid_restrict(l); }
#ifndef MAD_RR_SMALL_VOXELS
#define MAD_RR_SMALL_VOXELS 65536
#endif
  bool resid_restrict(int l, bool zero_x = false) {
    LevelData<T>& F = lv_[l];
    LevelData<T>& C = lv_[l + 1];
    const bool dist = c_->geom[l].distributed;
    const LevelGeom& Gc = c_->geom[l + 1];
    const bool handover = dist && !Gc.distributed && C.cent[2] == 1 && F.g.nz % 2 == 0 &&
                          F.g.zoff % 2 == 0 && (int64_t)(F.g.nz / 2) * c_->comm.nranks() == (int64_t)Gc.n[2];
    if (c_->dim != 3 || (dist != Gc.distributed && !handover) || F.g.nx < 16 || F.g.ny < 16 || F.g.nz < 2)
      return false;
    if (dist) {
      halo(l, F.x, GHOST);
      if (!F.brec) b_halo(l);
    }
    sync_brec(l);
    b_changed(l + 1);
    T* zx = (zero_x && !handover) ? C.x : nullptr;
    if (zx && C.x_peer_pending) peer_resolve(l + 1);
    if (zx && lazy_zero_ok(l + 1)) {
      zx = nullptr;
      C.x_zero_lazy = true;
    }
    if (zero_x && !handover) C.x_halo_ok = dist;
    T* cb = C.b;
    Geo gcv = C.g;
    if (handover) {
      gcv.nz = F.g.nz / 2;
      gcv.zoff = F.g.zoff / 2;
      gcv.N = gcv.sz * gcv.nz;
      gcv.zlo_ghost = gcv.zhi_ghost = 0;
      cb = coarse_slab((int64_t)gcv.N);
    }
    constexpr int target = 1024;
    const int ncz = (int)c_->geom[l + 1].n[2];
    auto run = [&](auto CXc, auto CYc, auto NTc) {
      constexpr int CX = decltype(CXc)::value, CY = decltype(CYc)::value, NT = decltype(NTc)::value;
      const int ntx = (gcv.nx + CX - 1) / CX, nty = (gcv.ny + CY - 1) / CY;
      const int zdiv = gcv.N <= MAD_RR_SMALL_VOXELS ? 1 : 4;
      int chunks = std::max(1, std::min((target + ntx * nty - 1) / (ntx * nty), gcv.nz / zdiv));
      const int kc = (gcv.nz + chunks - 1) / chunks;
      chunks = (gcv.nz + kc - 1) / kc;
      const dim3 grid((unsigned)(ntx * nty * chunks)), block(NT);
      auto go = [&](auto K) {
        constexpr int KD = decltype(K)::value;
        if (F.brec)
          hipLaunchKernelGGL((resid_restrict3_k<T, KD, CX, CY, NT, true>), grid, block, 0, c_->stream,
                             F.x, F.b, F.cf, F.g, F.rat, cb, zx, gcv, C.cent[0], C.cent[1], C.cent[2],
                             kc, ntx, F.g.zoff, ncz);
        else
          hipLaunchKernelGGL((resid_restrict3_k<T, KD, CX, CY, NT>), grid, block, 0, c_->stream, F.x,
                             F.b, F.cf, F.g, F.rat, cb, zx, gcv, C.cent[0], C.cent[1], C.cent[2], kc,
                             ntx, F.g.zoff, ncz);
      };
      if (c_->kind == KFULL) go(std::integral_constant<int, KFULL>{});
      else if (c_->kind == KDIAG) go(std::integral_constant<int, KDIAG>{});
      else go(std::integral_constant<int, KISO>{});
    };
    run(std::integral_constant<int, 32>{}, std::integral_constant<int, 8>{},
        std::integral_constant<int, 512>{});
    HIP_CHECK(hipGetLastError());
    if (handover) {
      wait_all_pending();
      c_->comm.allgather_slabs(cb, C.b, (int64_t)gcv.nx * gcv.ny, (int64_t)Gc.n[2], sizeof(T), c_->stream);
      if (zero_x) fill(l + 1, MAD_X, 0.0);
    }
    if (dist && C.peer) peer_push_b(l + 1);
    return true;
  }

  void restrict_arr(int l, T* fine, T* coarse) {
    LevelData<T>& F = lv_[l];
    LevelData<T>& C = lv_[l + 1];
    b_changed(l + 1);
    REQUIRE(!c_->geom[l].distributed || c_->geom[l + 1].distributed, MAD_ERR_UNSUPPORTED,
            "restriction onto a replicated level");
    halo(l, fine);
    const int fz_shift = (c_->dim == 3) ? F.g.zoff : 0;
    dim3 gr = grid_for(C.g.nx, C.g.ny, C.g.nz, BLK);
    Geo gc = C.g;
    if (c_->dim == 3) gc.zoff = C.g.zoff;
    if (c_->dim == 3) {
      constexpr int CX = 32, CY = 8;
      const int ntx = (C.g.nx + CX - 1) / CX, nty = (C.g.ny + CY - 1) / CY;
      int chunks = std::max(1, std::min((xfer_blocks() + ntx * nty - 1) / (ntx * nty), C.g.nz / 4));
      const int kc = (C.g.nz + chunks - 1) / chunks;
      chunks = (C.g.nz + kc - 1) / kc;
      hipLaunchKernelGGL((restrict3_k<T, T, CX, CY>), dim3((unsigned)(ntx * nty * chunks)),
                         dim3(CX * CY), 0, c_->stream, fine, F.g, coarse, gc, C.cent[0], C.cent[1],
                         C.cent[2], fz_shift, (int)c_->geom[l + 1].n[2], kc, ntx);
      (void)gr;
    } else {
      hipLaunchKernelGGL((restrict_k<T, T, 2>), gr, BLK, 0, c_->stream, fine, F.g, coarse, C.g,
                         C.cent[0], C.cent[1], C.cent[2], 0);
    }
    HIP_CHECK(hipGetLastError());
  }

  void interpolate(int l, bool add) override {
    LevelData<T>& F = lv_[l];
    LevelData<T>& C = lv_[l + 1];
    const bool ghosts = interp_ghosts(l, add);
    halo(l + 1, C.x, ghosts ? 3 : 1);
    dim3 gr = grid_for(F.g.nx, F.g.ny, F.g.nz, BLK);
    if (c_->dim == 3) {
      launch_interp3(l, add, ghosts);
      if (ghosts) F.x_halo_ok = true;
      else x_changed(l);
    } else {
      if (add)
        hipLaunchKernelGGL((interp_k<T, 2, 1>), gr, BLK, 0, c_->stream, C.x, C.g, F.x, F.g,
                           C.cent[0], C.cent[1], C.cent[2]);
      else
        hipLaunchKernelGGL((interp_k<T, 2, 0>), gr, BLK, 0, c_->stream, C.x, C.g, F.x, F.g,
                           C.cent[0], C.cent[1], C.cent[2]);
    }
    HIP_CHECK(hipGetLastError());
  }

  void coarse_solve() override {
    const int l = c_->nlev - 1;
    LevelData<T>& L = lv_[l];
    const int n = (int)L.g.N;
    REQUIRE(!c_->geom[l].distributed, MAD_ERR_UNSUPPORTED, "coarsest level must be replicated");
    if (cblk_.active())
      cblk_.solve<T>(L.b, L.x, c_->stream);
    else
      hipLaunchKernelGGL((coarse_solve_k<T>), dim3((unsigned)((n + 3) / 4)), dim3(256), 0, c_->stream,
                         inv_, L.b, L.x, n);
    HIP_CHECK(hipGetLastError());
  }

  void vcycle_rec(int l) {
    const int nl = c_->nlev;
    if (l == nl - 1) {
      coarse_solve();
      if (c_->d.verbose) (void)verbose_line(l, -1, "direct solver");
      return;
    }
    const unsigned nu = c_->d.iterations_per_grid;
    const bool bt = l == 0 && c_->bench_trace() && c_->trace_active;
    if (c_->d.verbose || bt) {
      for (unsigned n = 0; n < nu; ++n) {
        smooth(l, 1);
        per_sweep_line(l, (int)n + 1, nullptr, bt);
      }
    } else {
      smooth(l, nu);
    }
    if (!resid_restrict(l, true)) {
      residual(l, false);
      restrict_down(l);
      fill(l + 1, MAD_X, 0.0);
    }
    vcycle_rec(l + 1);
    interpolate_up(l, true);
    if (c_->d.verbose || bt) per_sweep_line(l, 0, "initial", bt);
    if (c_->d.verbose || bt) {
      for (unsigned n = 0; n < nu; ++n) {
        smooth(l, 1);
        per_sweep_line(l, (int)n + 1, nullptr, bt);
      }
    } else {
      smooth(l, nu);
    }
  }

  void restrict_down(int l) {
    if (c_->geom[l].distributed && !c_->geom[l + 1].distributed) {
      gather_level(l, lv_[l].r);
      restrict_full(l, gathered_, lv_[l + 1].b);
    } else {
      restrict_arr(l, lv_[l].r, lv_[l + 1].b);
    }
  }

  void restrict_rhs_down(int l) {
    if (c_->geom[l].distributed && !c_->geom[l + 1].distributed) {
      gather_level(l, lv_[l].b);
      restrict_full(l, gathered_, lv_[l + 1].b);
    } else {
      restrict_arr(l, lv_[l].b, lv_[l + 1].b);
    }
  }

  void interpolate_up(int l, bool add) {
    if (c_->geom[l].distributed && !c_->geom[l + 1].distributed) {
      interp_from_replicated(l, add);
    } else {
      interpolate(l, add);
    }
  }

  void fmg_rec(int l) {
    const int nl = c_->nlev;
    if (l == nl - 1) {
      fill(l, MAD_X, 0.0);
    } else {
      restrict_rhs_down(l);
      fmg_rec(l + 1);
      interpolate_up(l, false);
    }
    for (unsigned n = 0; n < c_->d.iterations_per_grid; ++n) vcycle_rec(l);
  }

  bool vgraph_ranks_ok() const {
    return !(c_->d.options & MAD_OPT_EAGER_RANK_VCYCLE) &&
           (c_->comm.mode() == Comm::RCCL || c_->comm.mode() == Comm::SOLO) && c_->d.gs_kernel != 4;
  }

  struct HaloFlags {
    bool x_ok, b_ok, brec_ok;
  };
  std::vector<HaloFlags> halo_flags() const {
    std::vector<HaloFlags> v;
    for (auto& L : lv_) v.push_back({L.x_halo_ok, L.b_halo_ok, L.brec_ok});
    return v;
  }
  void ranks_graph_entry() {
    peer_resolve_all();
    if (lv_[0].peer)
      halo(0, lv_[0].x, GHOST);
    else
      lv_[0].x_halo_ok = false;
    if (!lv_[0].brec && !lv_[0].b_halo_ok) {
      halo(0, lv_[0].b, GHOST);
      lv_[0].b_halo_ok = true;
    }
    wait_all_pending();
    for (size_t l = 1; l < lv_.size(); ++l) {
      lv_[l].x_halo_ok = false;
      lv_[l].b_halo_ok = lv_[l].brec_ok = false;
    }
  }

  void vcycle_fast() {
    const bool ranks = c_->comm.active();
    if (c_->d.verbose || c_->bench_trace() || vgraph_failed_ || (ranks && !vgraph_ranks_ok()) ||
        (ranks && vcycles_eager_ < 1)) {
      if (ranks) ++vcycles_eager_;
      vcycle_rec(0);
      return;
    }
    sync_brec(0);
    sync_bsplit(0);
    if (ranks) ranks_graph_entry();
    const bool zu = zero_x0_;
    if (vgraph_) {
      bool same = vgraph_ptrs_.size() == lv_.size() && vgraph_zu_ == zu;
      for (size_t l = 0; same && l < lv_.size(); ++l)
        same = vgraph_ptrs_[l].first == lv_[l].x && vgraph_ptrs_[l].second == lv_[l].t &&
               vgraph_seq_[l] == (lv_[l].peer_seq & 1);
      if (!same) {
        HIP_CHECK(hipStreamSynchronize(c_->stream));
        (void)hipGraphExecDestroy(vgraph_);
        vgraph_ = nullptr;
      }
    }
    if (!vgraph_) {
      struct Snap {
        T* x;
        T* t;
        T* a0;
        T* a3;
        bool bh;
        int seq;
      };
      auto snap = [&] {
        std::vector<Snap> v;
        for (auto& L : lv_) v.push_back({L.x, L.t, L.alloc[0], L.alloc[3], L.b_halo_ok, L.peer_seq});
        return v;
      };
      auto restore = [&](const std::vector<Snap>& v) {
        for (size_t l = 0; l < lv_.size(); ++l) {
          lv_[l].x = v[l].x;
          lv_[l].t = v[l].t;
          lv_[l].alloc[0] = v[l].a0;
          lv_[l].alloc[3] = v[l].a3;
          lv_[l].b_halo_ok = v[l].bh;
          lv_[l].peer_seq = v[l].seq;
        }
      };
      const std::vector<Snap> before = snap();
      const std::vector<HaloFlags> flags_before = halo_flags();
      hipGraph_t gph = nullptr;
      HIP_CHECK(hipStreamBeginCapture(c_->stream, hipStreamCaptureModeThreadLocal));
      bool captured = true;
      try {
        vcycle_rec(0);
        if (ranks) {
          wait_all_pending();
          peer_resolve_all();
        }
      } catch (...) {
        (void)hipStreamEndCapture(c_->stream, &gph);
        if (gph) (void)hipGraphDestroy(gph);
        gph = nullptr;
        restore(before);
        if (!ranks) throw;
        captured = false;
      }
      if (captured && hipStreamEndCapture(c_->stream, &gph) != hipSuccess) {
        gph = nullptr;
        captured = false;
      }
      const std::vector<Snap> after = snap();
      bool same = captured;
      for (size_t l = 0; same && l < before.size(); ++l)
        same = before[l].x == after[l].x && before[l].t == after[l].t &&
               ((before[l].seq ^ after[l].seq) & 1) == 0;
      vgraph_exit_flags_ = halo_flags();
      restore(before);
      if (ranks) {
        for (size_t l = 0; l < lv_.size(); ++l) {
          lv_[l].x_halo_ok = flags_before[l].x_ok;
          lv_[l].b_halo_ok = flags_before[l].b_ok;
          lv_[l].brec_ok = flags_before[l].brec_ok;
          lv_[l].x_halo_pending = false;
        }
      }
      if (same && hipGraphInstantiate(&vgraph_, gph, nullptr, nullptr, 0) != hipSuccess) {
        vgraph_ = nullptr;
        same = false;
      }
      if (gph) (void)hipGraphDestroy(gph);
      zero_x0_ = zu;
      if (!same) {
        (void)hipGetLastError();
        vgraph_failed_ = true;
        vcycle_rec(0);
        return;
      }
      vgraph_zu_ = zu;
      zero_x0_ = false;
      vgraph_ptrs_.clear();
      vgraph_seq_.clear();
      for (auto& L : lv_) {
        vgraph_ptrs_.emplace_back(L.x, L.t);
        vgraph_seq_.push_back(L.peer_seq & 1);
      }
    }
    HIP_CHECK(hipGraphLaunch(vgraph_, c_->stream));
    zero_x0_ = false;
    if (ranks) c_->comm.graph_launched(c_->stream);
    if (ranks) {
      for (size_t l = 0; l < lv_.size(); ++l) {
        lv_[l].x_halo_ok = vgraph_exit_flags_[l].x_ok;
        lv_[l].b_halo_ok = vgraph_exit_flags_[l].b_ok;
        lv_[l].brec_ok = vgraph_exit_flags_[l].brec_ok;
        lv_[l].x_halo_pending = false;
      }
    } else {
      for (size_t l = 1; l < lv_.size(); ++l) lv_[l].b_halo_ok = lv_[l].brec_ok = false;
    }
  }

  void vcycle() override { vcycle_fast(); }

  void fmg() override { fmg_rec(0); }

  void per_sweep_line(int l, int it, const char* what, bool bench) {
    if (!c_->d.verbose) {
      const double rn = residual(l, true);
      c_->trace_push(c_->trace_rhs > 0.0 ? rn / c_->trace_rhs : rn);
      return;
    }
    const double rel = verbose_line(l, it, what);
    if (bench) {
      const double rn = rel * norm(l, MAD_B);
      c_->trace_push(c_->trace_rhs > 0.0 ? rn / c_->trace_rhs : rn);
    }
  }

  double verbose_line(int l, int it, const char* what) {
    const double bn = norm(l, MAD_B);
    const double rn = residual(l, true);
    const double rel = rn / bn;
    if (c_->comm.rank() != 0) return rel;
    std::string ind(l + 1, ' ');
    if (what && std::strcmp(what, "direct solver") == 0)
      std::printf("%sLevel %d, direct solver: relative residual = %g\n", ind.c_str(), l, rel);
    else if (what)
      std::printf("%sLevel %d, initial relative residual = %g\n", ind.c_str(), l, rel);
    else
      std::printf("%sLevel %d, iteration %d: relative residual = %g\n", ind.c_str(), l, it, rel);
    std::fflush(stdout);
    return rel;
  }

  void run(const void* in, int in_dtype, void* out, int out_dtype, bool dev_io,
           mad_stats* st) override {
    LevelData<T>& L0 = lv_[0];
    const int64_t N = L0.g.N;
    const mad_desc& d = c_->d;
    const unsigned nb = flat_blocks(N);
    const void* src = in;
    if (!dev_io) {
      void* stage = scratch_bytes(N * dtype_size(in_dtype));
      HIP_CHECK(hipMemcpyAsync(stage, in, N * dtype_size(in_dtype), hipMemcpyHostToDevice,
                               c_->stream));
      src = stage;
    }
    if (refine_) {
      convert_to(src, in_dtype, b64_, N, c_->stream);
      b32_exact_ = in_dtype == MAD_U8 || in_dtype == MAD_I8 || in_dtype == MAD_U16 || in_dtype == MAD_I16 ||
                   in_dtype == MAD_F32;
      if (b32_exact_) {
        hipLaunchKernelGGL((convert_k<double, float>), dim3(nb), dim3(256), 0, c_->stream, b64_, b32_, N);
        HIP_CHECK(hipGetLastError());
      }
    } else {
      convert_in(src, in_dtype, L0.b, N);
      L0.b_halo_ok = L0.brec_ok = false;
    }
    auto to_fp32_rhs = [&](const double* a) {
      hipLaunchKernelGGL((convert_k<double, T>), dim3(nb), dim3(256), 0, c_->stream, a, L0.b, N);
      HIP_CHECK(hipGetLastError());
      L0.b_halo_ok = L0.brec_ok = false;
    };
    auto x_to_u64 = [&] {
      hipLaunchKernelGGL((convert_k<T, double>), dim3(nb), dim3(256), 0, c_->stream, L0.x, u64_, N);
      HIP_CHECK(hipGetLastError());
    };
    auto rhs_norm = [&] { return refine_ ? norm64(b64_) : norm(0, MAD_B); };
    Event e0, e1;
    HIP_CHECK(hipEventRecord(e0, c_->stream));
    c_->step_cycles.clear();
    c_->step_relres.clear();
    c_->trace.clear();
    const bool bt = c_->bench_trace();
    FlagScope tracing(c_->trace_active);
    c_->trace_t0 = std::chrono::steady_clock::now();
    bool stalled_any = false;
    unsigned total = 0;
    double relres = 0.0;
    for (unsigned step = 0; step < d.number_of_steps; ++step) {
      if (d.verbose && d.number_of_steps > 1 && c_->comm.rank() == 0)
        std::printf("\n------------ Time step n. %u / %u------------\n", step + 1, d.number_of_steps);
#ifdef MAD_NO_REFINE_FP32_PHASE
      const bool fp32_phase = false;
#else
      const bool fp32_phase = refine_ && d.cycle != MAD_SMOOTHER && d.max_cycles >= 2;
#endif
      if (bt) {
        c_->trace_t0 = std::chrono::steady_clock::now();
        c_->trace_step = step;
        c_->trace_rhs = rhs_norm();
      }
      if (refine_ && (d.cycle == MAD_FMG || fp32_phase)) to_fp32_rhs(b64_);
      if (d.cycle == MAD_FMG) {
        if (d.verbose && c_->comm.rank() == 0) std::printf("|--- Full Multigrid Cycle ---|\n");
        fmg_rec(0);
        if (refine_ && !fp32_phase) x_to_u64();
      } else if (!refine_ || fp32_phase) {
        HIP_CHECK(hipMemcpyAsync(L0.x, L0.b, sizeof(T) * N, hipMemcpyDeviceToDevice, c_->stream));
        x_changed(0);
      } else {
        HIP_CHECK(hipMemcpyAsync(u64_, b64_, sizeof(double) * N, hipMemcpyDeviceToDevice, c_->stream));
      }
      const double rhsNorm = rhs_norm();
      REQUIRE(std::isfinite(rhsNorm), MAD_ERR_NUMERIC,
              "non-finite right-hand side norm (NaN/Inf in the input image)");
      unsigned it = 0;
      std::vector<double> hist;
      const unsigned window = (d.cycle == MAD_SMOOTHER) ? 50 : 5;
      bool stalled = false;
      auto rel = [&](double resNorm) {
        REQUIRE(std::isfinite(resNorm), MAD_ERR_NUMERIC,
                "non-finite residual norm (NaN/Inf in the tensor or the iterate)");
        return (rhsNorm > 0.0) ? resNorm / rhsNorm : resNorm;
      };
      auto cycle = [&](bool zero_x0) {
        if (d.cycle == MAD_SMOOTHER) {
          smooth(0, 1);
          return;
        }
        if (d.verbose && c_->comm.rank() == 0) std::printf("\n|--- VCycle n. %u ---|\n", it + 1);
        FlagScope zu(zero_x0_, zero_x0);
        vcycle_fast();
      };
      auto record = [&](double resNorm) {
        relres = rel(resNorm);
        if (d.verbose && d.cycle == MAD_SMOOTHER && c_->comm.rank() == 0)
          std::printf("Smoother iteration n. %u: relative residual = %g\n", it + 1, relres);
        ++it;
        hist.push_back(relres);
        if (!bt || d.cycle == MAD_SMOOTHER) {
          c_->trace_step = step;
          c_->trace_push(relres);
        }
      };
      if (fp32_phase) {
        do {
          cycle(false);
          record(residual_impl(0, true, false));
          if (hist.size() >= 2 && relres > MAD_REFINE_FP32_MIN_RATE * hist[hist.size() - 2]) break;
        } while (relres > std::max(d.tolerance, MAD_REFINE_SWITCH_RELRES) && it + 1 < d.max_cycles);
        x_to_u64();
      }
      auto patch_trace = [&] {
        if (!c_->trace.empty()) c_->trace.back().relres = relres;
      };
      if (refine_) {
        relres = rel(residual64());
        if (fp32_phase) {
          hist.back() = relres;
          patch_trace();
        }
      }
      if (!fp32_phase || (relres > d.tolerance && it < d.max_cycles)) do {
        if (!refine_) {
          cycle(false);
          record(residual_impl(0, true, false));
        } else {
          if (refine_emitted_) {
            L0.b_halo_ok = false;
            L0.brec_ok = refine_emitted_bs_;
            x_changed(0);
          } else {
            to_fp32_rhs(r64_);
            fill(0, MAD_X, 0.0);
          }
          cycle(refine_emitted_ && zero_sweep_ok());
          record(residual64(true));
          if (bt && d.cycle != MAD_SMOOTHER) patch_trace();
        }
        stalled = d.stall_guard && stalled_at(hist, window, d.tolerance);
      } while (relres > d.tolerance && it < d.max_cycles && !stalled);
      stalled_any |= stalled;
      total += it;
      c_->step_cycles.push_back(it);
      c_->step_relres.push_back(relres);
      if (refine_) {
        HIP_CHECK(hipMemcpyAsync(b64_, u64_, sizeof(double) * N, hipMemcpyDeviceToDevice, c_->stream));
        b32_exact_ = false;
      } else {
        HIP_CHECK(hipMemcpyAsync(L0.b, L0.x, sizeof(T) * N, hipMemcpyDeviceToDevice, c_->stream));
        L0.b_halo_ok = L0.brec_ok = false;
      }
    }
    HIP_CHECK(hipEventRecord(e1, c_->stream));
    if (refine_ && refine_emitted_ && zero_sweep_ok()) fill(0, MAD_X, 0.0);
    void* dst = out;
    if (!dev_io) dst = scratch_bytes(N * dtype_size(out_dtype));
    if (refine_) convert_from(u64_, dst, out_dtype, N, c_->stream);
    else convert_out(L0.x, dst, out_dtype, N);
    if (!dev_io)
      HIP_CHECK(hipMemcpyAsync(out, dst, N * dtype_size(out_dtype), hipMemcpyDeviceToHost,
                               c_->stream));
    HIP_CHECK(hipStreamSynchronize(c_->stream));
    peer_check();
    if (st) {
      std::memset(st, 0, sizeof(*st));
      st->steps = d.number_of_steps;
      st->total_cycles = total;
      st->last_cycles = c_->step_cycles.empty() ? 0 : c_->step_cycles.back();
      st->stalled = stalled_any ? 1 : 0;
      st->last_relres = relres;
      st->setup_ms = c_->setup_ms;
      st->solve_ms = elapsed(e0, e1);
      st->num_levels = (uint32_t)c_->nlev;
      st->tensor_kind = c_->kind;
      st->colors = c_->ncolors;
    }
  }

  void bench_smooth(int l, unsigned n, double* total_ms, double* kern_ms,
                    unsigned* launches) override {
    LevelData<T>& L = lv_[l];
    const int sm = c_->d.smoother;
    const bool fused = use_fused(l);
    const int nc = (sm == MAD_GAUSS_SEIDEL && !fused) ? c_->ncolors : 1;
    REQUIRE(sm != MAD_GAUSS_SEIDEL_LEX, MAD_ERR_UNSUPPORTED, "bench of the lexicographic mode");
    const unsigned nl = n * nc;
    std::vector<Event> ev(2 * nl);
    Event a, z;
    HIP_CHECK(hipEventRecord(a, c_->stream));
    const int rows = (nc == 4) ? (L.g.ny + 1) / 2 : L.g.ny;
    unsigned q = 0;
    for (unsigned s = 0; s < n; ++s) {
      if (sm == MAD_WEIGHTED_JACOBI) {
        prep_wj(l);
        HIP_CHECK(hipEventRecord(ev[2 * q], c_->stream));
        launch_wj(l);
        HIP_CHECK(hipEventRecord(ev[2 * q + 1], c_->stream));
        ++q;
        std::swap(L.x, L.t);
        std::swap(L.alloc[0], L.alloc[3]);
        x_changed(l);
      } else if (fused) {
        fused_sweep(l, ev[2 * q], ev[2 * q + 1]);
// ... 7 lines not shown
            hipLaunchKernelGGL((gs_color_k<T, D.value, K.value>), gr, BLK, 0, c_->stream, L.x,
                               L.b, L.cf, L.g, L.rat, col, nc);
          });
          HIP_CHECK(hipEventRecord(ev[2 * q + 1], c_->stream));
          ++q;
          x_changed(l);
        }
      }
    }
    HIP_CHECK(hipGetLastError());
    if (L.x_halo_pending) {
      HIP_CHECK(hipStreamWaitEvent(c_->stream, L.ev_halo, 0));
      L.x_halo_pending = false;
    }
    HIP_CHECK(hipEventRecord(z, c_->stream));
    HIP_CHECK(hipEventSynchronize(z));
    double ksum = 0.0;
    launch_ms.assign(q, 0.f);
    for (unsigned i = 0; i < q; ++i) {
      launch_ms[i] = elapsed(ev[2 * i], ev[2 * i + 1]);
      ksum += launch_ms[i];
    }
    *total_ms = elapsed(a, z);
    *kern_ms = q ? ksum / q : 0.0;
    *launches = q;
  }

  void bench_vcycle(unsigned n, double* total_ms) override {
    Event a, z;
    HIP_CHECK(hipEventRecord(a, c_->stream));
    for (unsigned s = 0; s < n; ++s) vcycle_fast();
    HIP_CHECK(hipEventRecord(z, c_->stream));
    HIP_CHECK(hipEventSynchronize(z));
    *total_ms = elapsed(a, z);
  }

 private:
  mad_ctx* c_ = nullptr;
  std::vector<LevelData<T>> lv_;
  bool refine_ = false;
  double* r64alloc_[3] = {nullptr, nullptr, nullptr};
  double* u64_ = nullptr;
  double* b64_ = nullptr;
  float* b32alloc_ = nullptr;
  float* b32_ = nullptr;
  bool b32_exact_ = false;
  double* r64_ = nullptr;
  double* cf64_alloc_ = nullptr;
  double* cf64_ = nullptr;
  Rat<double> rat64_{};
  int64_t part_cap_ = 0;
  hipGraphExec_t vgraph_ = nullptr;
  bool vgraph_zu_ = false;
  std::vector<std::pair<T*, T*>> vgraph_ptrs_;
  std::vector<int> vgraph_seq_;
  bool vgraph_failed_ = false;
  uint64_t peer_timeout_ticks_ = 0;
  int peer_fallbacks_ = 0;
  std::vector<HaloFlags> vgraph_exit_flags_;
  int vcycles_eager_ = 0;
  int ncoef_ = 0;
  double* part_ = nullptr;
  double* scal_ = nullptr;
  double* hscal_ = nullptr;
  double* inv_ = nullptr;
  CoarseBlocks cblk_;
  void* scratch_ = nullptr;
  size_t scratch_cap_ = 0;
  T* gathered_ = nullptr;
  T* full_x_ = nullptr;
  int64_t gathered_cap_ = 0;
  T* cslab_ = nullptr;
  int64_t cslab_cap_ = 0;

  void release() {
    if (c_ && c_->comm_stream) (void)hipStreamSynchronize(c_->comm_stream);
    if (c_ && c_->comm.mode() != Comm::LOCAL) {
      try {
        for (size_t l = 0; l < lv_.size(); ++l)
          if (lv_[l].x_peer_pending) peer_resolve((int)l);
      } catch (...) {
      }
    }
    if (c_ && c_->stream) (void)hipStreamSynchronize(c_->stream);
    if (vgraph_) (void)hipGraphExecDestroy(vgraph_);
    vgraph_ = nullptr;
    vgraph_ptrs_.clear();
    vgraph_seq_.clear();
    vgraph_failed_ = false;
    vcycles_eager_ = 0;
    for (auto& L : lv_) {
      if (L.ev_bnd) (void)hipEventDestroy(L.ev_bnd);
      if (L.ev_halo) (void)hipEventDestroy(L.ev_halo);
      if (L.sig) (void)hipFree(L.sig);
      Comm::close_window(L.win_lo, L.win_ipc);
      Comm::close_window(L.win_hi, L.win_ipc);
      if (L.win) (void)hipFree(L.win);
      for (auto& a : L.alloc)
        if (a) (void)hipFree(a);
      if (L.cf_alloc) (void)hipFree(L.cf_alloc);
      if (L.bs_alloc) (void)hipFree(L.bs_alloc);
    }
    lv_.clear();
    for (auto& a : r64alloc_)
      if (a) (void)hipFree(a), a = nullptr;
    if (cf64_alloc_) (void)hipFree(cf64_alloc_);
// ... 526 lines not shown
  d->iterations_per_grid = 2;
  d->max_cycles = 100;
  d->number_of_steps = 1;
  d->time_step = 0.01;
  d->tolerance = 1e-6;
  d->omega = 2.0 / 3.0;
  d->verbose = 0;
  d->precision = MAD_PRECISION_AUTO;
  d->stall_guard = 1;
  d->device = -1;
  d->tensor_kind = MAD_TENSOR_AUTO;
  d->nranks = 1;
  d->rank = 0;
  return MAD_OK;
}

int mad_max_depth(int32_t dim, const int64_t size[3]) {
  if ((dim != 2 && dim != 3) || !size) return -1;
  for (int q = 0; q < dim; ++q)
    if (size[q] < 1) return -1;
  int64_t n[3] = {size[0], size[1], dim == 3 ? size[2] : 1};
  return max_depth_rule(dim, n);
}

const char* mad_last_error(const mad_ctx* c) { return c ? c->err.c_str() : g_last_error.c_str(); }

int mad_create(const mad_desc* d, mad_ctx** out) {
  if (!out) return MAD_ERR_INVALID;
  *out = nullptr;
  std::unique_ptr<mad_ctx> c(new mad_ctx());
  int rc = guarded(nullptr, [&] {
    REQUIRE(d, MAD_ERR_INVALID, "null descriptor");
    REQUIRE(d->abi_version == MAD_ABI_VERSION, MAD_ERR_INVALID, "ABI version mismatch");
    REQUIRE(d->dim == 2 || d->dim == 3, MAD_ERR_INVALID, "dim must be 2 or 3");
    for (int q = 0; q < d->dim; ++q) {
      REQUIRE(d->size[q] >= 3, MAD_ERR_INVALID,
              "every image axis needs >= 3 voxels (one-sided tensor derivatives, GH.hxx:447-474)");
      REQUIRE(d->spacing[q] > 0.0, MAD_ERR_INVALID, "spacing must be positive");
    }
    REQUIRE(d->size[0] * d->size[1] * (d->dim == 3 ? d->size[2] : 1) < (int64_t)INT32_MAX * 8,
            MAD_ERR_INVALID, "image too large");
    REQUIRE(d->cycle >= MAD_VCYCLE && d->cycle <= MAD_SMOOTHER, MAD_ERR_INVALID, "bad cycle");
    REQUIRE(d->smoother >= MAD_GAUSS_SEIDEL && d->smoother <= MAD_WEIGHTED_JACOBI,
            MAD_ERR_INVALID, "bad smoother");
    REQUIRE(d->precision == MAD_FP32 || d->precision == MAD_FP64 || d->precision == MAD_FP32_REFINE ||
                d->precision == MAD_PRECISION_AUTO,
            MAD_ERR_INVALID, "bad precision");
    REQUIRE(d->nranks >= 1 && d->rank >= 0 && d->rank < d->nranks, MAD_ERR_INVALID,
            "bad rank / nranks");
    REQUIRE(d->gs_kernel == 0 || d->gs_kernel == 1 || d->gs_kernel == 3 || d->gs_kernel == 4,
            MAD_ERR_INVALID, "gs_kernel must be 0, 1, 3 or 4");
    REQUIRE((d->options & ~(MAD_OPT_EAGER_RANK_VCYCLE | MAD_OPT_OVERLAP_RANK_SWEEP | MAD_OPT_PEER_HALO |
                            MAD_OPT_COARSE_NO_CHAIN | MAD_OPT_BENCHMARK_TRACE |
                            MAD_OPT_NO_PLACEMENT_TUNE | MAD_OPT_NO_RECORD_B)) == 0,
            MAD_ERR_INVALID, "unknown option bits");
    REQUIRE(d->min_slab_planes >= 0, MAD_ERR_INVALID, "min_slab_planes must be >= 0");
    REQUIRE(d->min_slab_voxels >= 0, MAD_ERR_INVALID, "min_slab_voxels must be >= 0");
    REQUIRE(d->coarse_dense_max >= 0 && d->coarse_dense_max <= MAD_COARSE_DENSE_LIMIT, MAD_ERR_INVALID,
            "coarse_dense_max must be in [0, " + std::to_string(MAD_COARSE_DENSE_LIMIT) +
                "] (a dense inverse of n unknowns takes 8 n^2 bytes on the host and twice that on the device)");
    REQUIRE(d->coarse_block_unknowns >= 0, MAD_ERR_INVALID, "coarse_block_unknowns must be >= 0");
    REQUIRE(d->tensor_kind >= MAD_TENSOR_AUTO && d->tensor_kind <= MAD_TENSOR_FULL,
            MAD_ERR_INVALID, "bad tensor kind");
    c->d = *d;
    if (c->d.precision == MAD_PRECISION_AUTO)
      c->d.precision = d->tolerance < MAD_FP32_TOLERANCE_FLOOR ? MAD_FP32_REFINE : MAD_FP32;
    if (c->d.dim == 2) c->d.size[2] = 1;
    c->dim = d->dim;
    int dev = d->device;
    if (dev < 0) HIP_CHECK(hipGetDevice(&dev));
    c->device = dev;
    use_device(c.get());
    HIP_CHECK(hipStreamCreateWithFlags(&c->stream, hipStreamNonBlocking));
    HIP_CHECK(hipStreamCreateWithFlags(&c->comm_stream, hipStreamNonBlocking));
    compute_geometry(c.get());
  });
  if (rc != MAD_OK) return rc;
  *out = c.release();
  return MAD_OK;
}

void mad_destroy(mad_ctx* c) {
  if (!c) return;
  (void)hipSetDevice(c->device);
  if (c->stream) (void)hipStreamSynchronize(c->stream);
  delete c;
}

int mad_get_desc(const mad_ctx* c, mad_desc* out) {
  if (!c || !out) return MAD_ERR_INVALID;
  *out = c->d;
  return MAD_OK;
}

static int set_tensor_impl(mad_ctx* c, const void* p, int32_t dtype, bool dev, int64_t first,
                           int64_t nplanes) {
  if (!c) return MAD_ERR_INVALID;
  return guarded(c, [&] {
    REQUIRE(p, MAD_ERR_INVALID, "null tensor");
    REQUIRE(dtype == MAD_F32 || dtype == MAD_F64, MAD_ERR_INVALID, "tensor dtype must be F32/F64");
    REQUIRE(first <= c->tensor_lo && first + nplanes >= c->tensor_hi, MAD_ERR_INVALID,
            "tensor planes [" + std::to_string(first) + ", " + std::to_string(first + nplanes) +
                ") do not cover [" + std::to_string(c->tensor_lo) + ", " + std::to_string(c->tensor_hi) +
                ") (mad_tensor_planes)");
    use_device(c);
    const LevelGeom& G = c->geom[0];
    const int ncomp = c->dim * (c->dim + 1) / 2;
// ... 498 lines not shown
```

Measured before the change: 118,900.

## Emit residual from last fused GS sweep and reuse it in residual/restrict

Moves the fused 3D Gauss-Seidel kernel body into a header and adds an EMIT variant. For full tensors, the final color stage writes the pointwise residual to a compact buffer, and a validity flag tracks when that buffer is current. The residual, norm and residual-restrict kernels then read the stored residual instead of recomputing the full 19-point stencil from x, b and the coefficients. This cuts coefficient and iterate traffic after smoothing, but adds residual stores, per-level validity bookkeeping (including across graph replays) and an option to turn the reuse off.

```diff
diff --git a/include/mad.h b/include/mad.h
--- a/include/mad.h
+++ b/include/mad.h
@@ -93,6 +93,7 @@
 #define MAD_OPT_BENCHMARK_TRACE 16u
 #define MAD_OPT_NO_PLACEMENT_TUNE 32u
 #define MAD_OPT_NO_RECORD_B 64u
+#define MAD_OPT_NO_RESIDUAL_REUSE 128u
 
 typedef struct mad_stats {
   uint32_t steps;
diff --git a/multigridanisotropicdiffusion_amd/_capi.py b/multigridanisotropicdiffusion_amd/_capi.py
--- a/multigridanisotropicdiffusion_amd/_capi.py
+++ b/multigridanisotropicdiffusion_amd/_capi.py
@@ -22,6 +22,7 @@
 OPT_BENCHMARK_TRACE = 16
 OPT_NO_PLACEMENT_TUNE = 32
 OPT_NO_RECORD_B = 64
+OPT_NO_RESIDUAL_REUSE = 128
 VED_OPT_LINE_WALK = 1
 CED_EED, CED_CED = 0, 1
 PM_WEICKERT, PM_EXPONENTIAL, PM_RATIONAL = 0, 1, 2
diff --git a/multigridanisotropicdiffusion_amd/csrc/mad_gs_fused3_body.hpp b/multigridanisotropicdiffusion_amd/csrc/mad_gs_fused3_body.hpp
--- /dev/null
+++ b/multigridanisotropicdiffusion_amd/csrc/mad_gs_fused3_body.hpp
@@ -0,0 +1,347 @@
+  constexpr int NC = (KIND == KFULL) ? 4 : 2;
+  using FG = FusedGeom<NC, TX, TY>;
+  constexpr int H = FG::H, RX = FG::RX, RY = FG::RY, HALF = FG::HALF, PITCH = FG::PITCH;
+  constexpr int PLANE = FG::PLANE, NP = FG::NP;
+  constexpr int UPT = (RX * RY + NT - 1) / NT;
+  constexpr int OPT = (TX * TY + NT - 1) / NT;
+  constexpr int NCF = CoefLayout<3, KIND>::N;
+  constexpr int RS = NCF + (BREC ? 1 : 0);
+  constexpr uint32_t TS = sizeof(T);
+  static_assert(TX % 2 == 0 && TY % 2 == 0 && (H % 2) == 0, "even tile geometry");
+  static_assert(FG::rows(0) * FG::cols(0) <= NT, "one stage point per thread");
+  static_assert(!(BL && BREC), "b rides in the record");
+  static_assert(!(BS && (BL || BREC)), "one form of b");
+  static_assert(!EMIT || (KIND == KFULL && !PEER), "residual hand-over: FULL tensors, no rank slabs");
+  constexpr int NB = BL ? NC : 0;
+  extern __shared__ __align__(16) unsigned char fused_smem[];
+
+  int bid = blockIdx.x;
+  {
+    const int nb = gridDim.x, q = nb >> 3, r = nb & 7, xcd = bid & 7, idx = bid >> 3;
+    bid = (xcd < r ? xcd * (q + 1) : r * (q + 1) + (xcd - r) * q) + idx;
+  }
+  const int tiles = ntx * nty;
+  const int chunk = bid / tiles;
+  const int tile = bid - chunk * tiles;
+  const int tyi = tile / ntx;
+  const int txi = tile - tyi * ntx;
+  const int rx0 = txi * TX - H;
+  const int ry0 = tyi * TY - H;
+  const int tid = threadIdx.x;
+  const int wbase = __builtin_amdgcn_readfirstlane(tid & ~63);
+  auto wave_in = [&](int c) { return wbase < FG::rows(c) * FG::cols(c); };
+  const int nx = g.nx, ny = g.ny;
+  const int sy = (int)g.sy, hx0 = g.hx0;
+  const bool interior = rx0 >= 2 && rx0 + RX <= nx - 2 && ry0 >= 2 && ry0 + RY <= ny - 2;
+
+  const int p0 = zbase + chunk * zstride;
+  const int p1 = min(p0 + zc, g.nz);
+  const bool flip = !EMIT && flip_last != 0 && chunk == (int)(gridDim.x / tiles) - 1;
+  int64_t sz = g.sz;
+  int zlo_g = g.zlo_ghost, zhi_g = g.zhi_ghost, zpar = g.zoff;
+  int z0 = p0, z1 = p1;
+  if (flip) {
+    const int64_t top = (int64_t)(g.nz - 1) * g.sz;
+    uin += top;
+    uout += top;
+    b += top;
+    cf += top * RS;
+    sz = -g.sz;
+    zlo_g = g.zhi_ghost;
+    zhi_g = g.zlo_ghost;
+    zpar = g.zoff + g.nz - 1;
+    z0 = g.nz - p1;
+    z1 = g.nz - p0;
+  }
+  const int zlo = zlo_g ? -GHOST : 0;
+  const int zhi = zhi_g ? g.nz + GHOST : g.nz;
+  const int ulo = zlo_g ? -(GHOST - 1) : 0;
+  const int uhi = zhi_g ? g.nz + GHOST - 1 : g.nz;
+  T* const pdst = PEER ? po.dst[flip ? 1 : 0] : nullptr;
+  uint32_t* const psig = PEER ? po.sig[flip ? 1 : 0] : (sig ? sig + (flip ? 1 : 0) : nullptr);
+  const bool signals = !EMIT && (PEER ? pdst != nullptr : sig != nullptr) && z0 == 0 && zlo_g;
+  const int kbeg = (z0 - (NC - 1)) - ((z0 - (NC - 1) + zpar) & 1);
+  const int kend = z1 + NC - 2;
+
+  auto mirror = [](int v, int n) { return v < 0 ? min(-v, n - 1) : (v >= n ? max(2 * (n - 1) - v, 0) : v); };
+
+  uint32_t usrc[UPT];
+  int udst[UPT];
+#pragma unroll
+  for (int e = 0; e < UPT; ++e) {
+    const int q = tid + e * NT;
+    const int lj = q / RX, li = q - (q / RX) * RX;
+    int gi = rx0 + li, gj = ry0 + lj;
+    if (!interior) {
+      gi = mirror(gi, nx);
+      gj = mirror(gj, ny);
+    }
+    usrc[e] = (uint32_t)(gj * sy + gi) * TS;
+    udst[e] = (q < RX * RY) ? (int)((lj * PITCH + (li & 1) * HALF + (li >> 1)) * TS) : -1;
+  }
+  int olds[OPT], oglb[OPT];
+#pragma unroll
+  for (int e = 0; e < OPT; ++e) {
+    const int q = tid + e * NT;
+    const int lj = H + q / TX, li = H + (q - (q / TX) * TX);
+    const int gi = rx0 + li, gj = ry0 + lj;
+    const bool ok = q < TX * TY && gi < nx && gj < ny;
+    olds[e] = (int)((lj * PITCH + (li & 1) * HALF + (li >> 1)) * TS);
+    oglb[e] = ok ? (int)((gj * sy + gi) * TS) : -1;
+  }
+
+  constexpr int NPM = (NC == 4) ? 1 : 2;
+  uint32_t pl[NC][NPM], pg[NC][NPM], pb[NC][NPM];
+  uint32_t vmask = 0, gmask = 0;
+  uint32_t omask = 0;
+  uint32_t rco = 0;
+#pragma unroll
+  for (int c = 0; c < NC; ++c) {
+    const int cols = FG::cols(c);
+    const bool has = tid < FG::rows(c) * cols;
+    const int r = has ? tid / cols : 0;
+    const int t = has ? tid - (tid / cols) * cols : 0;
+    const int l0 = c + 1;
+    if (EMIT && c == NC - 1) rco = (uint32_t)(r * hx0 + t) * TS;
+#pragma unroll
+    for (int PM = 0; PM < 2; ++PM) {
+      int li, lj;
+      if (NC == 4) {
+        li = l0 + (1 ^ PM) + 2 * t;
+        lj = l0 + (((c >> 1) ^ PM ^ l0) & 1) + 2 * r;
+      } else {
+        lj = l0 + r;
+        li = l0 + ((c ^ PM ^ r) & 1) + 2 * t;
+      }
+      const int gi = rx0 + li, gj = ry0 + lj;
+      const bool ok = has && gi >= 0 && gi < nx && gj >= 0 && gj < ny;
+      vmask |= (ok ? 1u : 0u) << (c * 2 + PM);
+      const uint32_t gb = (ok && gi == 1 ? 1u : 0u) | (ok && gi == nx - 2 ? 2u : 0u) |
+                          (ok && gj == 1 ? 4u : 0u) | (ok && gj == ny - 2 ? 8u : 0u);
+      gmask |= gb << (4 * (c * 2 + PM));
+      omask |= (uint32_t)(li & 1) << (c * 2 + PM);
+      if (PM < NPM) {
+        pl[c][PM] = (uint32_t)(lj * PITCH + (li & 1) * HALF + (li >> 1)) * TS;
+        pg[c][PM] = (uint32_t)(lj * sy + (li & 1) * hx0 + (li >> 1)) * (TS * RS);
+        pb[c][PM] = (uint32_t)(lj * sy + li) * TS;
+      }
+    }
+  }
+  struct PD {
+    int l;
+    int64_t g, b;
+  };
+  auto pdelta = [&](int c, int PM) -> PD {
+    if (NC != 4 || PM == 0) return PD{0, 0, 0};
+    const int dy = 1 - 2 * (((c >> 1) ^ (c + 1)) & 1);
+    const bool odd0 = (c & 1) != 0;
+    return PD{dy * PITCH + (odd0 ? -HALF : HALF - 1), (int64_t)dy * sy + (odd0 ? -hx0 : hx0 - 1),
+              (int64_t)dy * sy - 1};
+  };
+  const int64_t cbase = (int64_t)ry0 * sy + (rx0 >> 1);
+  const int64_t bbase = (int64_t)ry0 * sy + rx0;
+  const int rcz = hx0 * ((ny + 1) >> 1);
+  T* const rcb = EMIT ? rc + ((int64_t)((ry0 + H) >> 1) * hx0 + ((rx0 + H) >> 1)) : nullptr;
+
+  auto slot = [](int m) { return (m + NP * 64) % NP; };
+  auto plane_ok = [&](int m) { return m >= zlo && m < zhi; };
+  auto stage_on = [&](int c, int m) {
+    const int h = NC - 1 - c;
+    return m >= z0 - h && m < z1 + h && m >= ulo && m < uhi;
+  };
+  unsigned char* lbytes = fused_smem;
+
+  T up[UPT];
+  T bp[BL ? UPT : 1];
+  T raw[NC][RS];
+  T bv[NC];
+  auto bslot = [](int m) { return NP + (m + NB * 64) % (NB > 0 ? NB : 1); };
+  auto load_bplane = [&](int m) {
+    if constexpr (BL) {
+      m = min(max(m, zlo), zhi - 1);
+      const __amdgpu_buffer_rsrc_t rs = buf_rsrc(b + (int64_t)m * sz);
+#pragma unroll
+      for (int e = 0; e < UPT; ++e) bp[e] = buf_load<T>(rs, usrc[e], 0u);
+    }
+  };
+  auto put_bplane = [&](int m) {
+    if constexpr (BL) {
+      unsigned char* P = lbytes + bslot(m) * (PLANE * TS);
+#pragma unroll
+      for (int e = 0; e < UPT; ++e) {
+        if (e < UPT - 1 || udst[e] >= 0) *reinterpret_cast<T*>(P + udst[e]) = bp[e];
+      }
+    }
+  };
+  auto load_plane = [&](int m) {
+    if constexpr (ZU) {
+#pragma unroll
+      for (int e = 0; e < UPT; ++e) up[e] = T(0);
+    } else {
+      m = min(max(m, zlo), zhi - 1);
+      const __amdgpu_buffer_rsrc_t rs = buf_rsrc(uin + (int64_t)m * sz);
+#pragma unroll
+      for (int e = 0; e < UPT; ++e) up[e] = buf_load<T>(rs, usrc[e], 0u);
+    }
+  };
+  auto put_plane = [&](int m) {
+    unsigned char* P = lbytes + slot(m) * (PLANE * TS);
+#pragma unroll
+    for (int e = 0; e < UPT; ++e) {
+      if (e < UPT - 1 || udst[e] >= 0) *reinterpret_cast<T*>(P + udst[e]) = up[e];
+    }
+  };
+  auto load_stage = [&](int c, int k, int PM) {
+    const int m = min(max(k - c, zlo), zhi - 1);
+    {
+      const PD d = pdelta(c, PM);
+      buf_load_rec<T, RS>(buf_rsrc(cf + ((int64_t)m * sz + cbase + d.g) * RS), pg[c][PM % NPM],
+                          raw[c]);
+      if constexpr (BS)
+        bv[c] = buf_load<T>(buf_rsrc(b + (int64_t)m * sz + cbase + d.g), pg[c][PM % NPM] / (uint32_t)RS, 0u);
+      else if constexpr (!BREC && !BL)
+        bv[c] = buf_load<T>(buf_rsrc(b + (int64_t)m * sz + bbase + d.b), pb[c][PM % NPM], 0u);
+    }
+  };
+  auto stage = [&](int c, int k, int PM) {
+    const int m = k - c;
+    if (!stage_on(c, m) || !wave_in(c)) return;
+    const int zm = (m == 0 && !zlo_g) ? 1 : m - 1;
+    const int zp = (m == g.nz - 1 && !zhi_g) ? g.nz - 2 : m + 1;
+    const uint32_t o = pl[c][PM % NPM] + (uint32_t)(pdelta(c, PM).l * (int)TS);
+    unsigned char* A0 = lbytes + slot(m) * (PLANE * TS) + o;
+    const unsigned char* Am = lbytes + slot(flip ? zp : zm) * (PLANE * TS) + o;
+    const unsigned char* Ap = lbytes + slot(flip ? zm : zp) * (PLANE * TS) + o;
+    bool odd;
+    if (NC == 4) {
+      odd = ((c + 1 + (1 ^ PM)) & 1) != 0;
+    } else {
+      odd = ((omask >> (c * 2 + PM)) & 1u) != 0;
+    }
+    const int ox_p = odd ? 1 - HALF : HALF;
+    const int ox_m = odd ? -HALF : HALF - 1;
+    auto rd = [](const unsigned char* p, int off) { return *reinterpret_cast<const T*>(p + off * (int)TS); };
+    T nb[18];
+    nb[0] = rd(A0, ox_p);
+    nb[1] = rd(A0, ox_m);
+    nb[2] = rd(A0, PITCH);
+    nb[3] = rd(A0, -PITCH);
+    nb[4] = rd(Ap, 0);
+    nb[5] = rd(Am, 0);
+    if (KIND == KFULL) {
+      nb[6] = rd(A0, ox_p + PITCH);
+      nb[7] = rd(A0, ox_p - PITCH);
+      nb[8] = rd(A0, ox_m + PITCH);
+      nb[9] = rd(A0, ox_m - PITCH);
+      nb[10] = rd(Ap, ox_p);
+      nb[11] = rd(Am, ox_p);
+      nb[12] = rd(Ap, ox_m);
+      nb[13] = rd(Am, ox_m);
+      nb[14] = rd(Ap, PITCH);
+      nb[15] = rd(Am, PITCH);
+      nb[16] = rd(Ap, -PITCH);
+      nb[17] = rd(Am, -PITCH);
+    }
+    Coefs<T> q;
+    coefs_from_raw<T, 3, KIND>(raw[c], rat, q);
+    T D, S;
+    stencil_combine<T, 3, KIND>(q, nb, D, S);
+    T bval;
+    if constexpr (BREC)
+      bval = raw[c][NCF];
+    else if constexpr (BL)
+      bval = *reinterpret_cast<const T*>(lbytes + bslot(m) * (PLANE * TS) + o);
+    else
+      bval = bv[c];
+    const T v = gs_update(bval, S, D);
+    const int bit = c * 2 + PM;
+    if constexpr (EMIT) {
+      if (c == NC - 1 && ((vmask >> bit) & 1u))
+        buf_store<T>(resid_value(bval, D, v, S), buf_rsrc(rcb + (int64_t)m * rcz), rco);
+    }
+    if (interior) {
+      if (NC == 2 || FG::rows(c) * FG::cols(c) < NT) {
+        if ((vmask >> bit) & 1u) *reinterpret_cast<T*>(A0) = v;
+      } else {
+        *reinterpret_cast<T*>(A0) = v;
+      }
+    } else if ((vmask >> bit) & 1u) {
+      *reinterpret_cast<T*>(A0) = v;
+      const uint32_t gb = (gmask >> (4 * bit)) & 15u;
+      if (gb) {
+        const int xs[3] = {0, (gb & 1u) ? -1 : 0, (gb & 2u) ? 1 : 0};
+        const int ys[3] = {0, (gb & 4u) ? -2 * PITCH : 0, (gb & 8u) ? 2 * PITCH : 0};
+#pragma unroll
+        for (int a = 0; a < 3; ++a)
+#pragma unroll
+          for (int bq = 0; bq < 3; ++bq) {
+            if ((a == 0 && bq == 0) || (a > 0 && xs[a] == 0) || (bq > 0 && ys[bq] == 0)) continue;
+            *reinterpret_cast<T*>(A0 + (xs[a] + ys[bq]) * (int)TS) = v;
+          }
+      }
+    }
+  };
+
+  for (int m = kbeg - 1; m <= kbeg; ++m)
+    if (plane_ok(m)) {
+      load_plane(m);
+      put_plane(m);
+    }
+  load_plane(kbeg + 1);
+  load_bplane(kbeg);
+#pragma unroll
+  for (int c = 0; c < LEAD; ++c) load_stage(c, kbeg, c & 1);
+
+  for (int k0 = kbeg; k0 <= kend; k0 += 2) {
+#pragma unroll
+    for (int u = 0; u < 2; ++u) {
+      const int k = k0 + u;
+      if (k <= kend) {
+        asm volatile("" : "+v"(vmask), "+v"(gmask), "+v"(omask));
+        if (plane_ok(k + 1)) put_plane(k + 1);
+        load_plane(k + 2);
+        put_bplane(k);
+        load_bplane(k + 1);
+        __syncthreads();
+#pragma unroll
+        for (int c = 0; c < NC; ++c) {
+          stage(c, k, (u ^ c) & 1);
+          {
+            constexpr int L = LEAD < NC ? LEAD : NC;
+            const int c2 = (c + L) % NC, dk = (c + L) / NC;
+            load_stage(c2, k + dk, (u ^ dk ^ c2) & 1);
+          }
+          __syncthreads();
+        }
+        const int mo = k - NC + 1;
+        if (mo >= z0 && mo < z1) {
+          const unsigned char* P = lbytes + slot(mo) * (PLANE * TS);
+          const __amdgpu_buffer_rsrc_t ro = buf_rsrc(uout + (int64_t)mo * sz);
+#pragma unroll
+          for (int e = 0; e < OPT; ++e)
+            if (oglb[e] >= 0)
+              buf_store<T>(*reinterpret_cast<const T*>(P + olds[e]), ro, (uint32_t)oglb[e]);
+          if constexpr (PEER) {
+            if (signals && mo < GHOST) {
+              const __amdgpu_buffer_rsrc_t rp = buf_rsrc(pdst + (int64_t)mo * sz);
+#pragma unroll
+              for (int e = 0; e < OPT; ++e)
+                if (oglb[e] >= 0)
+                  buf_store<T>(*reinterpret_cast<const T*>(P + olds[e]), rp, (uint32_t)oglb[e]);
+            }
+          }
+          if (signals && mo == GHOST - 1) {
+            if (PEER) {
+              __builtin_amdgcn_s_waitcnt(0);
+              __syncthreads();
+              if (tid == 0) __hip_atomic_fetch_add(psig, 1u, __ATOMIC_RELAXED, __HIP_MEMORY_SCOPE_SYSTEM);
+            } else {
+              __threadfence();
+              __syncthreads();
+              if (tid == 0) __hip_atomic_fetch_add(psig, 1u, __ATOMIC_RELEASE, __HIP_MEMORY_SCOPE_SYSTEM);
+            }
+          }
+        }
+      }
+    }
+  }
diff --git a/multigridanisotropicdiffusion_amd/csrc/mad_kernels.hpp b/multigridanisotropicdiffusion_amd/csrc/mad_kernels.hpp
--- a/multigridanisotropicdiffusion_amd/csrc/mad_kernels.hpp
+++ b/multigridanisotropicdiffusion_amd/csrc/mad_kernels.hpp
@@ -324,344 +324,29 @@
                                                         Geo g, Rat<T> rat, int zc, int ntx, int nty,
                                                         int zbase, int zstride, int flip_last,
                                                         uint32_t* __restrict__ sig, PeerOut<T> po) {
-  constexpr int NC = (KIND == KFULL) ? 4 : 2;
-  using FG = FusedGeom<NC, TX, TY>;
-  constexpr int H = FG::H, RX = FG::RX, RY = FG::RY, HALF = FG::HALF, PITCH = FG::PITCH;
-  constexpr int PLANE = FG::PLANE, NP = FG::NP;
-  constexpr int UPT = (RX * RY + NT - 1) / NT;
-  constexpr int OPT = (TX * TY + NT - 1) / NT;
-  constexpr int NCF = CoefLayout<3, KIND>::N;
-  constexpr int RS = NCF + (BREC ? 1 : 0);
-  constexpr uint32_t TS = sizeof(T);
-  static_assert(TX % 2 == 0 && TY % 2 == 0 && (H % 2) == 0, "even tile geometry");
-  static_assert(FG::rows(0) * FG::cols(0) <= NT, "one stage point per thread");
-  static_assert(!(BL && BREC), "b rides in the record");
-  static_assert(!(BS && (BL || BREC)), "one form of b");
-  constexpr int NB = BL ? NC : 0;
-  extern __shared__ __align__(16) unsigned char fused_smem[];
-
-  int bid = blockIdx.x;
-  {
-    const int nb = gridDim.x, q = nb >> 3, r = nb & 7, xcd = bid & 7, idx = bid >> 3;
-    bid = (xcd < r ? xcd * (q + 1) : r * (q + 1) + (xcd - r) * q) + idx;
-  }
-  const int tiles = ntx * nty;
-  const int chunk = bid / tiles;
-  const int tile = bid - chunk * tiles;
-  const int tyi = tile / ntx;
-  const int txi = tile - tyi * ntx;
-  const int rx0 = txi * TX - H;
-  const int ry0 = tyi * TY - H;
-  const int tid = threadIdx.x;
-  const int wbase = __builtin_amdgcn_readfirstlane(tid & ~63);
-  auto wave_in = [&](int c) { return wbase < FG::rows(c) * FG::cols(c); };
-  const int nx = g.nx, ny = g.ny;
-  const int sy = (int)g.sy, hx0 = g.hx0;
-  const bool interior = rx0 >= 2 && rx0 + RX <= nx - 2 && ry0 >= 2 && ry0 + RY <= ny - 2;
-
-  const int p0 = zbase + chunk * zstride;
-  const int p1 = min(p0 + zc, g.nz);
-  const bool flip = flip_last != 0 && chunk == (int)(gridDim.x / tiles) - 1;
-  int64_t sz = g.sz;
-  int zlo_g = g.zlo_ghost, zhi_g = g.zhi_ghost, zpar = g.zoff;
-  int z0 = p0, z1 = p1;
-  if (flip) {
-    const int64_t top = (int64_t)(g.nz - 1) * g.sz;
-    uin += top;
-    uout += top;
-    b += top;
-    cf += top * RS;
-    sz = -g.sz;
-    zlo_g = g.zhi_ghost;
-    zhi_g = g.zlo_ghost;
-    zpar = g.zoff + g.nz - 1;
-    z0 = g.nz - p1;
-    z1 = g.nz - p0;
-  }
-  const int zlo = zlo_g ? -GHOST : 0;
-  const int zhi = zhi_g ? g.nz + GHOST : g.nz;
-  const int ulo = zlo_g ? -(GHOST - 1) : 0;
-  const int uhi = zhi_g ? g.nz + GHOST - 1 : g.nz;
-  T* const pdst = PEER ? po.dst[flip ? 1 : 0] : nullptr;
-  uint32_t* const psig = PEER ? po.sig[flip ? 1 : 0] : (sig ? sig + (flip ? 1 : 0) : nullptr);
-  const bool signals = (PEER ? pdst != nullptr : sig != nullptr) && z0 == 0 && zlo_g;
-  const int kbeg = (z0 - (NC - 1)) - ((z0 - (NC - 1) + zpar) & 1);
-  const int kend = z1 + NC - 2;
-
-  auto mirror = [](int v, int n) { return v < 0 ? min(-v, n - 1) : (v >= n ? max(2 * (n - 1) - v, 0) : v); };
-
-  uint32_t usrc[UPT];
-  int udst[UPT];
-#pragma unroll
-  for (int e = 0; e < UPT; ++e) {
-    const int q = tid + e * NT;
-    const int lj = q / RX, li = q - (q / RX) * RX;
-    int gi = rx0 + li, gj = ry0 + lj;
-    if (!interior) {
-      gi = mirror(gi, nx);
-      gj = mirror(gj, ny);
-    }
-    usrc[e] = (uint32_t)(gj * sy + gi) * TS;
-    udst[e] = (q < RX * RY) ? (int)((lj * PITCH + (li & 1) * HALF + (li >> 1)) * TS) : -1;
-  }
-  int olds[OPT], oglb[OPT];
-#pragma unroll
-  for (int e = 0; e < OPT; ++e) {
-    const int q = tid + e * NT;
-    const int lj = H + q / TX, li = H + (q - (q / TX) * TX);
-    const int gi = rx0 + li, gj = ry0 + lj;
-    const bool ok = q < TX * TY && gi < nx && gj < ny;
-    olds[e] = (int)((lj * PITCH + (li & 1) * HALF + (li >> 1)) * TS);
-    oglb[e] = ok ? (int)((gj * sy + gi) * TS) : -1;
-  }
-
-  constexpr int NPM = (NC == 4) ? 1 : 2;
-  uint32_t pl[NC][NPM], pg[NC][NPM], pb[NC][NPM];
-  uint32_t vmask = 0, gmask = 0;
-  uint32_t omask = 0;
-#pragma unroll
-  for (int c = 0; c < NC; ++c) {
-    const int cols = FG::cols(c);
-    const bool has = tid < FG::rows(c) * cols;
-    const int r = has ? tid / cols : 0;
-    const int t = has ? tid - (tid / cols) * cols : 0;
-    const int l0 = c + 1;
-#pragma unroll
-    for (int PM = 0; PM < 2; ++PM) {
-      int li, lj;
-      if (NC == 4) {
-        li = l0 + (1 ^ PM) + 2 * t;
-        lj = l0 + (((c >> 1) ^ PM ^ l0) & 1) + 2 * r;
-      } else {
-        lj = l0 + r;
-        li = l0 + ((c ^ PM ^ r) & 1) + 2 * t;
-      }
-      const int gi = rx0 + li, gj = ry0 + lj;
-      const bool ok = has && gi >= 0 && gi < nx && gj >= 0 && gj < ny;
-      vmask |= (ok ? 1u : 0u) << (c * 2 + PM);
-      const uint32_t gb = (ok && gi == 1 ? 1u : 0u) | (ok && gi == nx - 2 ? 2u : 0u) |
-                          (ok && gj == 1 ? 4u : 0u) | (ok && gj == ny - 2 ? 8u : 0u);
-      gmask |= gb << (4 * (c * 2 + PM));
-      omask |= (uint32_t)(li & 1) << (c * 2 + PM);
-      if (PM < NPM) {
-        pl[c][PM] = (uint32_t)(lj * PITCH + (li & 1) * HALF + (li >> 1)) * TS;
-        pg[c][PM] = (uint32_t)(lj * sy + (li & 1) * hx0 + (li >> 1)) * (TS * RS);
-        pb[c][PM] = (uint32_t)(lj * sy + li) * TS;
-      }
-    }
-  }
-  struct PD {
-    int l;
-    int64_t g, b;
-  };
-  auto pdelta = [&](int c, int PM) -> PD {
-    if (NC != 4 || PM == 0) return PD{0, 0, 0};
-    const int dy = 1 - 2 * (((c >> 1) ^ (c + 1)) & 1);
-    const bool odd0 = (c & 1) != 0;
-    return PD{dy * PITCH + (odd0 ? -HALF : HALF - 1), (int64_t)dy * sy + (odd0 ? -hx0 : hx0 - 1),
-              (int64_t)dy * sy - 1};
-  };
-  const int64_t cbase = (int64_t)ry0 * sy + (rx0 >> 1);
-  const int64_t bbase = (int64_t)ry0 * sy + rx0;
-
-  auto slot = [](int m) { return (m + NP * 64) % NP; };
-  auto plane_ok = [&](int m) { return m >= zlo && m < zhi; };
-  auto stage_on = [&](int c, int m) {
-    const int h = NC - 1 - c;
-    return m >= z0 - h && m < z1 + h && m >= ulo && m < uhi;
-  };
-  unsigned char* lbytes = fused_smem;
-
-  T up[UPT];
-  T bp[BL ? UPT : 1];
-  T raw[NC][RS];
-  T bv[NC];
-  auto bslot = [](int m) { return NP + (m + NB * 64) % (NB > 0 ? NB : 1); };
-  auto load_bplane = [&](int m) {
-    if constexpr (BL) {
-      m = min(max(m, zlo), zhi - 1);
-      const __amdgpu_buffer_rsrc_t rs = buf_rsrc(b + (int64_t)m * sz);
-#pragma unroll
-      for (int e = 0; e < UPT; ++e) bp[e] = buf_load<T>(rs, usrc[e], 0u);
-    }
-  };
-  auto put_bplane = [&](int m) {
-    if constexpr (BL) {
-      unsigned char* P = lbytes + bslot(m) * (PLANE * TS);
-#pragma unroll
-      for (int e = 0; e < UPT; ++e) {
-        if (e < UPT - 1 || udst[e] >= 0) *reinterpret_cast<T*>(P + udst[e]) = bp[e];
-      }
-    }
-  };
-  auto load_plane = [&](int m) {
-    if constexpr (ZU) {
-#pragma unroll
-      for (int e = 0; e < UPT; ++e) up[e] = T(0);
-    } else {
-      m = min(max(m, zlo), zhi - 1);
-      const __amdgpu_buffer_rsrc_t rs = buf_rsrc(uin + (int64_t)m * sz);
-#pragma unroll
-      for (int e = 0; e < UPT; ++e) up[e] = buf_load<T>(rs, usrc[e], 0u);
-    }
-  };
-  auto put_plane = [&](int m) {
-    unsigned char* P = lbytes + slot(m) * (PLANE * TS);
-#pragma unroll
-    for (int e = 0; e < UPT; ++e) {
-      if (e < UPT - 1 || udst[e] >= 0) *reinterpret_cast<T*>(P + udst[e]) = up[e];
-    }
-  };
-  auto load_stage = [&](int c, int k, int PM) {
-    const int m = min(max(k - c, zlo), zhi - 1);
-    {
-      const PD d = pdelta(c, PM);
-      buf_load_rec<T, RS>(buf_rsrc(cf + ((int64_t)m * sz + cbase + d.g) * RS), pg[c][PM % NPM],
-                          raw[c]);
-      if constexpr (BS)
-        bv[c] = buf_load<T>(buf_rsrc(b + (int64_t)m * sz + cbase + d.g), pg[c][PM % NPM] / (uint32_t)RS, 0u);
-      else if constexpr (!BREC && !BL)
-        bv[c] = buf_load<T>(buf_rsrc(b + (int64_t)m * sz + bbase + d.b), pb[c][PM % NPM], 0u);
-    }
-  };
-  auto stage = [&](int c, int k, int PM) {
-    const int m = k - c;
-    if (!stage_on(c, m) || !wave_in(c)) return;
-    const int zm = (m == 0 && !zlo_g) ? 1 : m - 1;
-    const int zp = (m == g.nz - 1 && !zhi_g) ? g.nz - 2 : m + 1;
-    const uint32_t o = pl[c][PM % NPM] + (uint32_t)(pdelta(c, PM).l * (int)TS);
-    unsigned char* A0 = lbytes + slot(m) * (PLANE * TS) + o;
-    const unsigned char* Am = lbytes + slot(flip ? zp : zm) * (PLANE * TS) + o;
-    const unsigned char* Ap = lbytes + slot(flip ? zm : zp) * (PLANE * TS) + o;
-    bool odd;
-    if (NC == 4) {
-      odd = ((c + 1 + (1 ^ PM)) & 1) != 0;
-    } else {
-      odd = ((omask >> (c * 2 + PM)) & 1u) != 0;
-    }
-    const int ox_p = odd ? 1 - HALF : HALF;
-    const int ox_m = odd ? -HALF : HALF - 1;
-    auto rd = [](const unsigned char* p, int off) { return *reinterpret_cast<const T*>(p + off * (int)TS); };
-    T nb[18];
-    nb[0] = rd(A0, ox_p);
-    nb[1] = rd(A0, ox_m);
-    nb[2] = rd(A0, PITCH);
-    nb[3] = rd(A0, -PITCH);
-    nb[4] = rd(Ap, 0);
-    nb[5] = rd(Am, 0);
-    if (KIND == KFULL) {
-      nb[6] = rd(A0, ox_p + PITCH);
-      nb[7] = rd(A0, ox_p - PITCH);
-      nb[8] = rd(A0, ox_m + PITCH);
-      nb[9] = rd(A0, ox_m - PITCH);
-      nb[10] = rd(Ap, ox_p);
-      nb[11] = rd(Am, ox_p);
-      nb[12] = rd(Ap, ox_m);
-      nb[13] = rd(Am, ox_m);
-      nb[14] = rd(Ap, PITCH);
-      nb[15] = rd(Am, PITCH);
-      nb[16] = rd(Ap, -PITCH);
-      nb[17] = rd(Am, -PITCH);
-    }
-    Coefs<T> q;
-    coefs_from_raw<T, 3, KIND>(raw[c], rat, q);
-    T D, S;
-    stencil_combine<T, 3, KIND>(q, nb, D, S);
-    T bval;
-    if constexpr (BREC)
-      bval = raw[c][NCF];
-    else if constexpr (BL)
-      bval = *reinterpret_cast<const T*>(lbytes + bslot(m) * (PLANE * TS) + o);
-    else
-      bval = bv[c];
-    const T v = gs_update(bval, S, D);
-    const int bit = c * 2 + PM;
-    if (interior) {
-      if (NC == 2 || FG::rows(c) * FG::cols(c) < NT) {
-        if ((vmask >> bit) & 1u) *reinterpret_cast<T*>(A0) = v;
-      } else {
-        *reinterpret_cast<T*>(A0) = v;
-      }
-    } else if ((vmask >> bit) & 1u) {
-      *reinterpret_cast<T*>(A0) = v;
-      const uint32_t gb = (gmask >> (4 * bit)) & 15u;
-      if (gb) {
-        const int xs[3] = {0, (gb & 1u) ? -1 : 0, (gb & 2u) ? 1 : 0};
-        const int ys[3] = {0, (gb & 4u) ? -2 * PITCH : 0, (gb & 8u) ? 2 * PITCH : 0};
-#pragma unroll
-        for (int a = 0; a < 3; ++a)
-#pragma unroll
-          for (int bq = 0; bq < 3; ++bq) {
-            if ((a == 0 && bq == 0) || (a > 0 && xs[a] == 0) || (bq > 0 && ys[bq] == 0)) continue;
-            *reinterpret_cast<T*>(A0 + (xs[a] + ys[bq]) * (int)TS) = v;
-          }
-      }
-    }
-  };
-
-  for (int m = kbeg - 1; m <= kbeg; ++m)
-    if (plane_ok(m)) {
-      load_plane(m);
-      put_plane(m);
-    }
-  load_plane(kbeg + 1);
-  load_bplane(kbeg);
-#pragma unroll
-  for (int c = 0; c < LEAD; ++c) load_stage(c, kbeg, c & 1);
-
-  for (int k0 = kbeg; k0 <= kend; k0 += 2) {
-#pragma unroll
-    for (int u = 0; u < 2; ++u) {
-      const int k = k0 + u;
-      if (k <= kend) {
-        asm volatile("" : "+v"(vmask), "+v"(gmask), "+v"(omask));
-        if (plane_ok(k + 1)) put_plane(k + 1);
-        load_plane(k + 2);
-        put_bplane(k);
-        load_bplane(k + 1);
-        __syncthreads();
-#pragma unroll
-        for (int c = 0; c < NC; ++c) {
-          stage(c, k, (u ^ c) & 1);
-          {
-            constexpr int L = LEAD < NC ? LEAD : NC;
-            const int c2 = (c + L) % NC, dk = (c + L) / NC;
-            load_stage(c2, k + dk, (u ^ dk ^ c2) & 1);
-          }
-          __syncthreads();
-        }
-        const int mo = k - NC + 1;
-        if (mo >= z0 && mo < z1) {
-          const unsigned char* P = lbytes + slot(mo) * (PLANE * TS);
-          const __amdgpu_buffer_rsrc_t ro = buf_rsrc(uout + (int64_t)mo * sz);
-#pragma unroll
-          for (int e = 0; e < OPT; ++e)
-            if (oglb[e] >= 0)
-              buf_store<T>(*reinterpret_cast<const T*>(P + olds[e]), ro, (uint32_t)oglb[e]);
-          if constexpr (PEER) {
-            if (signals && mo < GHOST) {
-              const __amdgpu_buffer_rsrc_t rp = buf_rsrc(pdst + (int64_t)mo * sz);
-#pragma unroll
-              for (int e = 0; e < OPT; ++e)
-                if (oglb[e] >= 0)
-                  buf_store<T>(*reinterpret_cast<const T*>(P + olds[e]), rp, (uint32_t)oglb[e]);
-            }
-          }
-          if (signals && mo == GHOST - 1) {
-            if (PEER) {
-              __builtin_amdgcn_s_waitcnt(0);
-              __syncthreads();
-              if (tid == 0) __hip_atomic_fetch_add(psig, 1u, __ATOMIC_RELAXED, __HIP_MEMORY_SCOPE_SYSTEM);
-            } else {
-              __threadfence();
-              __syncthreads();
-              if (tid == 0) __hip_atomic_fetch_add(psig, 1u, __ATOMIC_RELEASE, __HIP_MEMORY_SCOPE_SYSTEM);
-            }
-          }
-        }
-      }
-    }
-  }
+  constexpr bool EMIT = false;
+  T* const rc = nullptr;
+#include "mad_gs_fused3_body.hpp"
+}
+template <typename T, int KIND, int TX, int TY, int NT, int MINW, int LEAD, bool BREC, bool BL, bool ZU, bool BS>
+__device__ __forceinline__ void gs_fused3_emit_body(const T* __restrict__ uin, T* __restrict__ uout,
+                                                    const T* __restrict__ b, const T* __restrict__ cf, Geo g,
+                                                    Rat<T> rat, int zc, int ntx, int nty, int zbase,
+                                                    int zstride, int flip_last, uint32_t* __restrict__ sig,
+                                                    PeerOut<T> po, T* __restrict__ rc) {
+  constexpr bool EMIT = true, PEER = false;
+#include "mad_gs_fused3_body.hpp"
+}
+template <typename T, int KIND, int TX, int TY, int NT, int MINW, int LEAD = 2, bool BREC = false,
+          bool BL = false, bool ZU = false, bool BS = false>
+__global__ void __launch_bounds__(NT, MINW) gs_fused3_emit_k(const T* __restrict__ uin, T* __restrict__ uout,
+                                                             const T* __restrict__ b,
+                                                             const T* __restrict__ cf, Geo g, Rat<T> rat,
+                                                             int zc, int ntx, int nty, int zbase, int zstride,
+                                                             T* __restrict__ rc) {
+  gs_fused3_emit_body<T, KIND, TX, TY, NT, MINW, LEAD, BREC, BL, ZU, BS>(
+      uin, uout, b, cf, g, rat, zc, ntx, nty, zbase, zstride, 0, nullptr,
+      PeerOut<T>{{nullptr, nullptr}, {nullptr, nullptr}}, rc);
 }
 
 __device__ __forceinline__ uint32_t peer_pattern(int rank, int64_t e) {
@@ -856,7 +541,8 @@
   }
 }
 
-template <typename T, int KIND, int TX, int TY, bool BREC = false, typename TE = T, typename TB = T>
+template <typename T, int KIND, int TX, int TY, bool BREC = false, typename TE = T, typename TB = T,
+          bool RU = false>
 __global__ void __launch_bounds__(TX * TY) resid3_k(const T* __restrict__ u, const TB* __restrict__ b,
                                                     T* __restrict__ r, const T* __restrict__ cf,
                                                     Geo g, Rat<T> rat, int zc, int ntx,
@@ -865,7 +551,9 @@
                                                     TE* __restrict__ xe = nullptr,
                                                     const TE* __restrict__ ue = nullptr,
                                                     T* __restrict__ uo = nullptr,
-                                                    TE* __restrict__ bse = nullptr) {
+                                                    TE* __restrict__ bse = nullptr,
+                                                    const T* __restrict__ rc = nullptr) {
+  static_assert(!RU || (KIND == KFULL && TX % 2 == 0 && TY % 2 == 0), "residual hand-over: FULL tensors");
   constexpr int NT = TX * TY;
   constexpr int RX = TX + 2, RY = TY + 2, PL = RX * RY;
   constexpr int UPT = (PL + NT - 1) / NT;
@@ -879,7 +567,8 @@
   const int tyi = tile / ntx, txi = tile - (tile / ntx) * ntx;
   const int x0 = txi * TX, y0 = tyi * TY;
   const int tid = threadIdx.x;
-  const int tx = tid % TX, ty = tid / TX;
+  const int tl = tid % TX, ty = tid / TX;
+  const int tx = RU ? (tl < TX / 2 ? 2 * tl : 2 * (tl - TX / 2) + 1) : tl;
   const int nx = g.nx, ny = g.ny, sy = (int)g.sy, hx0 = g.hx0;
   const int64_t sz = g.sz;
   const int z0 = chunk * zc, z1 = min(z0 + zc, g.nz);
@@ -902,6 +591,10 @@
   const int64_t rbase = (int64_t)y0 * sy + (x0 >> 1), pbase = (int64_t)y0 * sy + x0;
   const int il = (ty + 1) * RX + (tx + 1);
   constexpr int oyp = RX, oym = -RX;
+  const bool lastc = RU && ok && ((tx ^ ty) & 1) == 0;
+  const uint32_t rc_off = (uint32_t)((ty >> 1) * hx0 + (tx >> 1)) * TS;
+  const int64_t rcz = (int64_t)hx0 * ((ny + 1) >> 1), rcbase = (int64_t)(y0 >> 1) * hx0 + (x0 >> 1);
+  auto reused = [&](int m) { return RU && lastc && ((m + g.zoff + tx) & 1) != 0; };
 
   T up[UPT];
   T raw[RS];
@@ -926,8 +619,12 @@
   };
   auto load_pt = [&](int m) {
     m = min(max(m, 0), g.nz - 1);
-    buf_load_rec<T, RS>(buf_rsrc(cf + ((int64_t)m * sz + rbase) * RS), rec_off, raw);
-    if constexpr (!BREC) bv = (T)buf_load<TB>(buf_rsrc(b + (int64_t)m * sz + pbase), pt_off_b, 0u);
+    if (reused(m)) {
+      bv = buf_load<T>(buf_rsrc(rc + (int64_t)m * rcz + rcbase), rc_off, 0u);
+    } else {
+      buf_load_rec<T, RS>(buf_rsrc(cf + ((int64_t)m * sz + rbase) * RS), rec_off, raw);
+      if constexpr (!BREC) bv = (T)buf_load<TB>(buf_rsrc(b + (int64_t)m * sz + pbase), pt_off_b, 0u);
+    }
   };
 
   if (z0 - 1 >= zlo) {
@@ -948,32 +645,37 @@
     const T* P0 = ring + (m & 3) * PL + il;
     const T* Pm = ring + (zm & 3) * PL + il;
     const T* Pp = ring + (zp & 3) * PL + il;
-    T nb[18];
-    nb[0] = P0[1];
-    nb[1] = P0[-1];
-    nb[2] = P0[oyp];
-    nb[3] = P0[oym];
-    nb[4] = Pp[0];
-    nb[5] = Pm[0];
-    if (KIND == KFULL) {
-      nb[6] = P0[1 + oyp];
-      nb[7] = P0[1 + oym];
-      nb[8] = P0[-1 + oyp];
-      nb[9] = P0[-1 + oym];
-      nb[10] = Pp[1];
-      nb[11] = Pm[1];
-      nb[12] = Pp[-1];
-      nb[13] = Pm[-1];
-      nb[14] = Pp[oyp];
-      nb[15] = Pm[oyp];
-      nb[16] = Pp[oym];
-      nb[17] = Pm[oym];
-    }
-    Coefs<T> q;
-    coefs_from_raw<T, 3, KIND>(raw, rat, q);
-    T D, S;
-    stencil_combine<T, 3, KIND>(q, nb, D, S);
-    const T rv = resid_value(BREC ? raw[NCF] : bv, D, P0[0], S);
+    T rv;
+    if (reused(m)) {
+      rv = bv;
+    } else {
+      T nb[18];
+      nb[0] = P0[1];
+      nb[1] = P0[-1];
+      nb[2] = P0[oyp];
+      nb[3] = P0[oym];
+      nb[4] = Pp[0];
+      nb[5] = Pm[0];
+      if (KIND == KFULL) {
+        nb[6] = P0[1 + oyp];
+        nb[7] = P0[1 + oym];
+        nb[8] = P0[-1 + oyp];
+        nb[9] = P0[-1 + oym];
+        nb[10] = Pp[1];
+        nb[11] = Pm[1];
+        nb[12] = Pp[-1];
+        nb[13] = Pm[-1];
+        nb[14] = Pp[oyp];
+        nb[15] = Pm[oyp];
+        nb[16] = Pp[oym];
+        nb[17] = Pm[oym];
+      }
+      Coefs<T> q;
+      coefs_from_raw<T, 3, KIND>(raw, rat, q);
+      T D, S;
+      stencil_combine<T, 3, KIND>(q, nb, D, S);
+      rv = resid_value(BREC ? raw[NCF] : bv, D, P0[0], S);
+    }
     load_pt(m + 1);
     if (ok) {
       if (r) buf_store<T>(rv, buf_rsrc(r + (int64_t)m * sz + pbase), pt_off);
@@ -988,6 +690,12 @@
     }
   }
   if (part) {
+    if constexpr (RU) {
+      __shared__ double sqx[NT];
+      sqx[ty * TX + tx] = sq;
+      __syncthreads();
+      sq = sqx[tid];
+    }
     const double s = block_sum<NT>(sq);
     if (tid == 0) part[blockIdx.x] = s;
   }
@@ -1286,12 +994,13 @@
   }
 }
 
-template <typename T, int KIND, int CX, int CY, int NT, bool BREC = false>
+template <typename T, int KIND, int CX, int CY, int NT, bool BREC = false, bool RU = false>
 __global__ void __launch_bounds__(NT) resid_restrict3_k(
     const T* __restrict__ u, const T* __restrict__ b, const T* __restrict__ cf, Geo gf, Rat<T> rat,
     T* __restrict__ coarse, T* __restrict__ zx, Geo gc, int cx, int cy, int cz, int kc, int ntx,
-    int fzs, int ncz) {
+    int fzs, int ncz, const T* __restrict__ rc = nullptr) {
   static_assert(CX * CY <= NT, "one coarse point per thread");
+  static_assert(!RU || KIND == KFULL, "residual hand-over: FULL tensors");
   constexpr int FX = 2 * CX + 2, FY = 2 * CY + 2, FP = FX * FY;
   constexpr int UX = FX + 2, UY = FY + 2, UP = UX * UY;
   constexpr int UPT = (UP + NT - 1) / NT;
@@ -1330,15 +1039,25 @@
   }
   int r_il[RPT];
   uint32_t r_rec[RPT], r_pt[RPT];
+  uint32_t r_rc[RU ? RPT : 1];
+  int r_pos[RU ? RPT : 1];
+  uint32_t lcm = 0;
 #pragma unroll
   for (int e = 0; e < RPT; ++e) {
     const int q = min(tid + e * NT, FP - 1);
-    const int ry = q / FX, rx = q - (q / FX) * FX;
+    const int ry = q / FX, rq = q - (q / FX) * FX;
+    const int rx = RU ? (rq < FX / 2 ? 2 * rq : 2 * (rq - FX / 2) + 1) : rq;
     const int xf = min(max(fx0 + rx, 0), nx - 1), yf = min(max(fy0 + ry, 0), ny - 1);
     r_il[e] = (yf - uy0) * UX + (xf - ux0);
     r_rec[e] = (uint32_t)(yf * sy + (xf & 1) * hx0 + (xf >> 1)) * (TS * RS);
     r_pt[e] = (uint32_t)(yf * sy + xf) * TS;
-  }
+    if constexpr (RU) {
+      r_pos[e] = ry * FX + rx;
+      r_rc[e] = (uint32_t)((yf >> 1) * hx0 + (xf >> 1)) * TS;
+      lcm |= ((((xf ^ yf) & 1) == 0 ? 1u : 0u) | (uint32_t)(xf & 1) << 1) << (2 * e);
+    }
+  }
+  const int64_t rcz = (int64_t)hx0 * ((ny + 1) >> 1);
   const int K0 = chunk * kc, K1 = min(K0 + kc, gc.nz);
   int iz[4];
   T wz[4];
@@ -1370,6 +1089,9 @@
   };
   const int wbase = __builtin_amdgcn_readfirstlane(tid & ~63);
   auto wave_in = [&](int e) { return wbase + e * NT < FP; };
+  auto reused = [&](int e, int m) {
+    return RU && ((lcm >> (2 * e)) & 1u) != 0 && (((uint32_t)(m + gf.zoff) + (lcm >> (2 * e + 1))) & 1u) != 0;
+  };
   auto load_pts = [&](int m) {
     m = min(max(m, ulo), uhi - 1);
     const __amdgpu_buffer_rsrc_t rr = buf_rsrc(cf + (int64_t)m * sz * RS);
@@ -1377,8 +1099,12 @@
 #pragma unroll
     for (int e = 0; e < RPT; ++e) {
       if (e > 0 && !wave_in(e)) continue;
-      buf_load_rec<T, RS>(rr, r_rec[e], raw[e]);
-      if constexpr (!BREC) bv[e] = buf_load<T>(rb, r_pt[e], 0u);
+      if (reused(e, m)) {
+        if constexpr (RU) bv[e] = buf_load<T>(buf_rsrc(rc + (int64_t)m * rcz), r_rc[e], 0u);
+      } else {
+        buf_load_rec<T, RS>(rr, r_rec[e], raw[e]);
+        if constexpr (!BREC) bv[e] = buf_load<T>(rb, r_pt[e], 0u);
+      }
     }
   };
 
@@ -1394,6 +1120,7 @@
   int K = K0;
   ztaps(K);
   for (int f = f_lo; f <= f_hi; ++f) {
+    if constexpr (RU) asm volatile("" : "+v"(lcm));
     if (f + 1 < uhi) put_plane(f + 1);
     load_plane(f + 2);
     __syncthreads();
@@ -1405,33 +1132,38 @@
       const T* P0 = ring + (f & 3) * UP + r_il[e];
       const T* Pm = ring + (zm & 3) * UP + r_il[e];
       const T* Pp = ring + (zp & 3) * UP + r_il[e];
-      T nb[18];
-      nb[0] = P0[1];
-      nb[1] = P0[-1];
-      nb[2] = P0[UX];
-      nb[3] = P0[-UX];
-      nb[4] = Pp[0];
-      nb[5] = Pm[0];
-      if (KIND == KFULL) {
-        nb[6] = P0[1 + UX];
-        nb[7] = P0[1 - UX];
-        nb[8] = P0[-1 + UX];
-        nb[9] = P0[-1 - UX];
-        nb[10] = Pp[1];
-        nb[11] = Pm[1];
-        nb[12] = Pp[-1];
-        nb[13] = Pm[-1];
-        nb[14] = Pp[UX];
-        nb[15] = Pm[UX];
-        nb[16] = Pp[-UX];
-        nb[17] = Pm[-UX];
+      T rv;
+      if (reused(e, min(max(f, ulo), uhi - 1))) {
+        if constexpr (RU) rv = bv[e];
+      } else {
+        T nb[18];
+        nb[0] = P0[1];
+        nb[1] = P0[-1];
+        nb[2] = P0[UX];
+        nb[3] = P0[-UX];
+        nb[4] = Pp[0];
+        nb[5] = Pm[0];
+        if (KIND == KFULL) {
+          nb[6] = P0[1 + UX];
+          nb[7] = P0[1 - UX];
+          nb[8] = P0[-1 + UX];
+          nb[9] = P0[-1 - UX];
+          nb[10] = Pp[1];
+          nb[11] = Pm[1];
+          nb[12] = Pp[-1];
+          nb[13] = Pm[-1];
+          nb[14] = Pp[UX];
+          nb[15] = Pm[UX];
+          nb[16] = Pp[-UX];
+          nb[17] = Pm[-UX];
+        }
+        Coefs<T> q;
+        coefs_from_raw<T, 3, KIND>(raw[e], rat, q);
+        T D, S;
+        stencil_combine<T, 3, KIND>(q, nb, D, S);
+        rv = resid_value(BREC ? raw[e][NCF] : bv[e], D, P0[0], S);
       }
-      Coefs<T> q;
-      coefs_from_raw<T, 3, KIND>(raw[e], rat, q);
-      T D, S;
-      stencil_combine<T, 3, KIND>(q, nb, D, S);
-      const T rv = resid_value(BREC ? raw[e][NCF] : bv[e], D, P0[0], S);
-      if (tid + e * NT < FP) rt[tid + e * NT] = rv;
+      if (tid + e * NT < FP) rt[RU ? r_pos[e] : tid + e * NT] = rv;
     }
     if (f < f_hi) load_pts(f + 1);
     __syncthreads();
diff --git a/multigridanisotropicdiffusion_amd/csrc/mad_solver.hip b/multigridanisotropicdiffusion_amd/csrc/mad_solver.hip
--- a/multigridanisotropicdiffusion_amd/csrc/mad_solver.hip
+++ b/multigridanisotropicdiffusion_amd/csrc/mad_solver.hip
@@ -315,6 +315,7 @@
   int peer_buf = 0;
   bool b_peer_pending = false;
   bool x_zero_lazy = false;
+  bool rc_ok = false;
 };
 constexpr int BOUNDARY_PLANES = 8;
 #ifndef MAD_FUSED_B_SPLIT
@@ -732,6 +733,7 @@
     LevelData<T>& L = lv_[l];
     if (L.b_peer_pending) peer_resolve_b(l);
     L.b_halo_ok = L.brec_ok = false;
+    L.rc_ok = false;
   }
   static uint32_t push_blocks(const LevelData<T>& L) {
     const size_t bytes = (size_t)L.ghost * sizeof(T);
@@ -771,6 +773,7 @@
     LevelData<T>& L = lv_[l];
     if (which == MAD_B) b_changed(l);
     if (which == MAD_X) x_changed(l);
+    if (which == MAD_R) L.rc_ok = false;
     double* tmp = scratch64(L.g.N);
     HIP_CHECK(hipMemcpyAsync(tmp, h, sizeof(double) * L.g.N, hipMemcpyHostToDevice, c_->stream));
     hipLaunchKernelGGL((convert_k<double, T>), dim3(flat_blocks(L.g.N)), dim3(256), 0, c_->stream,
@@ -794,6 +797,7 @@
     LevelData<T>& L = lv_[l];
     if (which == MAD_B) b_changed(l);
     if (which == MAD_X) x_changed(l);
+    if (which == MAD_R) L.rc_ok = false;
     hipLaunchKernelGGL((fill_k<T>), dim3(flat_blocks(L.g.N)), dim3(256), 0, c_->stream, arr(l, which),
                        L.g.N, (T)v);
     HIP_CHECK(hipGetLastError());
@@ -803,6 +807,7 @@
     LevelData<T>& L = lv_[l];
     if (which == MAD_B) b_changed(l);
     if (which == MAD_X) x_changed(l);
+    if (which == MAD_R) L.rc_ok = false;
     const LevelGeom& G = c_->geom[l];
     hipLaunchKernelGGL((synth_image_k<T>), grid_for(L.g.nx, L.g.ny, L.g.nz, BLK), BLK, 0, c_->stream,
                        arr(l, which), L.g, G.n[0], G.n[1], seed);
@@ -832,6 +837,7 @@
     if (lv_[l].x_peer_pending) peer_resolve(l);
     lv_[l].x_halo_ok = false;
     lv_[l].x_zero_lazy = false;
+    lv_[l].rc_ok = false;
   }
 
   static constexpr int XFER_BLOCKS = 1024;
@@ -898,7 +904,7 @@
   }
 
   template <int KD, int TX, int TY, int NT>
-  void launch_fused(LevelData<T>& L, const FusedCfg& fc, int part, bool zu = false) {
+  void launch_fused(LevelData<T>& L, const FusedCfg& fc, int part, bool zu = false, bool emit = false) {
     const int ntx = (L.g.nx + TX - 1) / TX, nty = (L.g.ny + TY - 1) / TY;
     const int tiles = ntx * nty;
     int flip = 0;
@@ -930,6 +936,45 @@
       hipLaunchKernelGGL(kern, dim3(nb), dim3(NT), lds, c_->stream, L.x, L.t, L.bs ? L.bs : L.b, L.cf, L.g,
                          L.rat, zr.zc, ntx, nty, zr.zbase, zr.zstride, flip, sig, po);
     };
+    if (emit) {
+      REQUIRE(KD == KFULL && part == 0 && !flip, MAD_ERR_STATE, "residual hand-over on a sweep without its instance");
+      if constexpr (KD == KFULL) {
+        auto run_emit = [&](auto kern) {
+          {
+            static std::mutex attr_mu;
+            static std::vector<const void*> attr;
+            std::lock_guard<std::mutex> lk(attr_mu);
+            if (std::find(attr.begin(), attr.end(), (const void*)kern) == attr.end()) {
+              HIP_CHECK(hipFuncSetAttribute((const void*)kern, hipFuncAttributeMaxDynamicSharedMemorySize,
+                                            (int)lds));
+              attr.push_back((const void*)kern);
+            }
+          }
+          hipLaunchKernelGGL(kern, dim3(nb), dim3(NT), lds, c_->stream, L.x, L.t, L.bs ? L.bs : L.b, L.cf, L.g,
+                             L.rat, zr.zc, ntx, nty, zr.zbase, zr.zstride, L.r);
+        };
+        if (L.brec) {
+          run_emit(gs_fused3_emit_k<T, KD, TX, TY, NT, MW, 2, true>);
+        } else if constexpr (bl_fits) {
+          if (zu) {
+            if (L.bs)
+              run_emit(gs_fused3_emit_k<T, KD, TX, TY, NT, MW, 2, false, false, true, true>);
+            else
+              bl ? run_emit(gs_fused3_emit_k<T, KD, TX, TY, NT, MW, 2, false, true, true>)
+                 : run_emit(gs_fused3_emit_k<T, KD, TX, TY, NT, MW, 2, false, false, true>);
+          } else if (L.bs) {
+            run_emit(gs_fused3_emit_k<T, KD, TX, TY, NT, MW, 2, false, false, false, true>);
+          } else {
+            bl ? run_emit(gs_fused3_emit_k<T, KD, TX, TY, NT, MW, 2, false, true>)
+               : run_emit(gs_fused3_emit_k<T, KD, TX, TY, NT, MW, 2>);
+          }
+        } else {
+          REQUIRE(!zu, MAD_ERR_STATE, "zero-iterate sweep without its instance");
+          run_emit(gs_fused3_emit_k<T, KD, TX, TY, NT, MW, 2>);
+        }
+      }
+      return;
+    }
     if (part == 4) {
       if (L.brec)
         run(gs_fused3_k<T, KD, TX, TY, NT, MW, 2, true, true>);
@@ -980,13 +1025,14 @@
     *nchunks = whole_range(L.g.nz, *tiles, fc).nchunks;
   }
 
-  void launch_fused_part(LevelData<T>& L, int part, bool zu = false) {
+  void launch_fused_part(LevelData<T>& L, int part, bool zu = false, bool emit = false) {
     const FusedCfg fc = fused_cfg();
+    REQUIRE(!emit || c_->kind == KFULL, MAD_ERR_STATE, "residual hand-over needs the FULL tensor's colouring");
     if (c_->kind == KFULL) {
       if constexpr (sizeof(T) == 4)
-        launch_fused<KFULL, 64, MAD_FUSED_F32_TY, MAD_FUSED_F32_TY * 32>(L, fc, part, zu);
+        launch_fused<KFULL, 64, MAD_FUSED_F32_TY, MAD_FUSED_F32_TY * 32>(L, fc, part, zu, emit);
       else
-        launch_fused<KFULL, 64, 16, 512>(L, fc, part, zu);
+        launch_fused<KFULL, 64, 16, 512>(L, fc, part, zu, emit);
     } else if (c_->kind == KDIAG) {
       launch_fused<KDIAG, 64, 16, 1024>(L, fc, part, zu);
     } else {
@@ -1075,8 +1121,9 @@
     return 2 * tiles >= 128;
   }
 
-  float fused_sweep(int l, hipEvent_t e0 = nullptr, hipEvent_t e1 = nullptr) {
+  float fused_sweep(int l, hipEvent_t e0 = nullptr, hipEvent_t e1 = nullptr, bool emit = false) {
     LevelData<T>& L = lv_[l];
+    L.rc_ok = false;
     halo(l, L.x, GHOST);
     if (L.brec) {
       sync_brec(l);
@@ -1114,7 +1161,8 @@
       const bool zu = (zero_x0_ && &L == &lv_[0]) || L.x_zero_lazy;
       zero_x0_ = false;
       L.x_zero_lazy = false;
-      launch_fused_part(L, 0, zu);
+      launch_fused_part(L, 0, zu, emit);
+      L.rc_ok = emit;
     } else {
       launch_fused_part(L, 1);
       wait_all_pending();
@@ -1178,11 +1226,25 @@
            c_->ncolors <= GHOST;
   }
 
-  void smooth(int l, unsigned n) override {
+  bool reuse_level(int l) const {
+    const mad_desc& d = c_->d;
+    const Geo& g = lv_[l].g;
+    return !(d.options & MAD_OPT_NO_RESIDUAL_REUSE) && c_->dim == 3 && c_->kind == KFULL &&
+           d.smoother == MAD_GAUSS_SEIDEL && d.gs_kernel != 4 && !c_->geom[l].distributed && !d.verbose &&
+           !c_->bench_trace() && g.nx >= 16 && g.ny >= 16 && g.nz >= 2 && use_fused(l);
+  }
+  bool reuse_descent(int l) const {
+    return l + 1 < c_->nlev && reuse_level(l) && !c_->geom[l + 1].distributed;
+  }
+
+  void smooth(int l, unsigned n) override { smooth_n(l, n, reuse_descent(l)); }
+
+  void smooth_n(int l, unsigned n, bool emit_last) {
     LevelData<T>& L = lv_[l];
     const int dim = c_->dim;
     const int sm = c_->d.smoother;
     for (unsigned s = 0; s < n; ++s) {
+      L.rc_ok = false;
       if (sm == MAD_WEIGHTED_JACOBI) {
         prep_wj(l);
         launch_wj(l);
@@ -1202,7 +1264,7 @@
         }
         HIP_CHECK(hipGetLastError());
       } else if (use_fused(l)) {
-        fused_sweep(l);
+        fused_sweep(l, nullptr, nullptr, emit_last && s + 1 == n);
       } else {
         const int nc = c_->ncolors;
         const int rows = (nc == 4) ? (L.g.ny + 1) / 2 : L.g.ny;
@@ -1370,9 +1432,24 @@
       nparts = (int64_t)ntx * nty * chunks;
       REQUIRE(nparts <= part_cap_, MAD_ERR_UNSUPPORTED, "residual partials buffer too small");
       sync_brec(l);
+      const bool ru = L.rc_ok && !write_r && c_->kind == KFULL;
+      if (write_r) L.rc_ok = false;
       auto go = [&](auto K) {
         constexpr int KD = decltype(K)::value;
         T* rout = write_r ? L.r : nullptr;
+        if constexpr (KD == KFULL) {
+          if (ru) {
+            if (L.brec)
+              hipLaunchKernelGGL((resid3_k<T, KD, TX, TY, true, T, T, true>), dim3((unsigned)nparts),
+                                 dim3(TX * TY), 0, c_->stream, L.x, L.b, rout, L.cf, L.g, L.rat, zc, ntx,
+                                 want_norm ? part_ : nullptr, nullptr, nullptr, nullptr, nullptr, nullptr, L.r);
+            else
+              hipLaunchKernelGGL((resid3_k<T, KD, TX, TY, false, T, T, true>), dim3((unsigned)nparts),
+                                 dim3(TX * TY), 0, c_->stream, L.x, L.b, rout, L.cf, L.g, L.rat, zc, ntx,
+                                 want_norm ? part_ : nullptr, nullptr, nullptr, nullptr, nullptr, nullptr, L.r);
+            return;
+          }
+        }
         if (L.brec)
           hipLaunchKernelGGL((resid3_k<T, KD, TX, TY, true>), dim3((unsigned)nparts),
                              dim3(TX * TY), 0, c_->stream, L.x, L.b, rout, L.cf, L.g, L.rat, zc, ntx,
@@ -1386,6 +1463,7 @@
       else if (c_->kind == KDIAG) go(std::integral_constant<int, KDIAG>{});
       else go(std::integral_constant<int, KISO>{});
     } else {
+      L.rc_ok = false;
       dim3 gr = grid_for(L.g.nx, L.g.ny, L.g.nz, BLK);
       nparts = (int64_t)gr.x * gr.y * gr.z;
       dispatch(c_->dim, c_->kind, [&](auto D, auto K) {
@@ -1433,6 +1511,8 @@
       zx = nullptr;
       C.x_zero_lazy = true;
     }
+    if (zero_x) C.rc_ok = false;
+    const bool ru = F.rc_ok && !dist && !handover && c_->kind == KFULL;
     if (zero_x && !handover) C.x_halo_ok = dist;
     T* cb = C.b;
     Geo gcv = C.g;
@@ -1455,6 +1535,19 @@
       const dim3 grid((unsigned)(ntx * nty * chunks)), block(NT);
       auto go = [&](auto K) {
         constexpr int KD = decltype(K)::value;
+        if constexpr (KD == KFULL) {
+          if (ru) {
+            if (F.brec)
+              hipLaunchKernelGGL((resid_restrict3_k<T, KD, CX, CY, NT, true, true>), grid, block, 0, c_->stream,
+                                 F.x, F.b, F.cf, F.g, F.rat, cb, zx, gcv, C.cent[0], C.cent[1], C.cent[2],
+                                 kc, ntx, F.g.zoff, ncz, F.r);
+            else
+              hipLaunchKernelGGL((resid_restrict3_k<T, KD, CX, CY, NT, false, true>), grid, block, 0, c_->stream,
+                                 F.x, F.b, F.cf, F.g, F.rat, cb, zx, gcv, C.cent[0], C.cent[1], C.cent[2],
+                                 kc, ntx, F.g.zoff, ncz, F.r);
+            return;
+          }
+        }
         if (F.brec)
           hipLaunchKernelGGL((resid_restrict3_k<T, KD, CX, CY, NT, true>), grid, block, 0, c_->stream,
                              F.x, F.b, F.cf, F.g, F.rat, cb, zx, gcv, C.cent[0], C.cent[1], C.cent[2],
@@ -1557,8 +1650,9 @@
         per_sweep_line(l, (int)n + 1, nullptr, bt);
       }
     } else {
-      smooth(l, nu);
-    }
+      smooth_n(l, nu, reuse_descent(l));
+    }
+    if (nu == 0) lv_[l].rc_ok = false;
     if (!resid_restrict(l, true)) {
       residual(l, false);
       restrict_down(l);
@@ -1573,9 +1667,10 @@
         per_sweep_line(l, (int)n + 1, nullptr, bt);
       }
     } else {
-      smooth(l, nu);
-    }
-  }
+      smooth_n(l, nu, l == 0 && emit_post_ && reuse_level(0));
+    }
+  }
+  bool emit_post_ = false;
 
   void restrict_down(int l) {
     if (c_->geom[l].distributed && !c_->geom[l + 1].distributed) {
@@ -1658,7 +1753,7 @@
     if (ranks) ranks_graph_entry();
     const bool zu = zero_x0_;
     if (vgraph_) {
-      bool same = vgraph_ptrs_.size() == lv_.size() && vgraph_zu_ == zu;
+      bool same = vgraph_ptrs_.size() == lv_.size() && vgraph_zu_ == zu && vgraph_ep_ == emit_post_;
       for (size_t l = 0; same && l < lv_.size(); ++l)
         same = vgraph_ptrs_[l].first == lv_[l].x && vgraph_ptrs_[l].second == lv_[l].t &&
                vgraph_seq_[l] == (lv_[l].peer_seq & 1);
@@ -1721,6 +1816,9 @@
         same = before[l].x == after[l].x && before[l].t == after[l].t &&
                ((before[l].seq ^ after[l].seq) & 1) == 0;
       vgraph_exit_flags_ = halo_flags();
+      vgraph_exit_rc_.clear();
+      for (auto& L : lv_) vgraph_exit_rc_.push_back(L.rc_ok);
+      for (size_t l = 0; l < lv_.size(); ++l) lv_[l].rc_ok = false;
       restore(before);
       if (ranks) {
         for (size_t l = 0; l < lv_.size(); ++l) {
@@ -1743,6 +1841,7 @@
         return;
       }
       vgraph_zu_ = zu;
+      vgraph_ep_ = emit_post_;
       zero_x0_ = false;
       vgraph_ptrs_.clear();
       vgraph_seq_.clear();
@@ -1753,6 +1852,7 @@
     }
     HIP_CHECK(hipGraphLaunch(vgraph_, c_->stream));
     zero_x0_ = false;
+    for (size_t l = 0; l < lv_.size(); ++l) lv_[l].rc_ok = vgraph_exit_rc_[l];
     if (ranks) c_->comm.graph_launched(c_->stream);
     if (ranks) {
       for (size_t l = 0; l < lv_.size(); ++l) {
@@ -1823,11 +1923,13 @@
     } else {
       convert_in(src, in_dtype, L0.b, N);
       L0.b_halo_ok = L0.brec_ok = false;
+      L0.rc_ok = false;
     }
     auto to_fp32_rhs = [&](const double* a) {
       hipLaunchKernelGGL((convert_k<double, T>), dim3(nb), dim3(256), 0, c_->stream, a, L0.b, N);
       HIP_CHECK(hipGetLastError());
       L0.b_halo_ok = L0.brec_ok = false;
+      L0.rc_ok = false;
     };
     auto x_to_u64 = [&] {
       hipLaunchKernelGGL((convert_k<T, double>), dim3(nb), dim3(256), 0, c_->stream, L0.x, u64_, N);
@@ -1881,13 +1983,14 @@
                 "non-finite residual norm (NaN/Inf in the tensor or the iterate)");
         return (rhsNorm > 0.0) ? resNorm / rhsNorm : resNorm;
       };
-      auto cycle = [&](bool zero_x0) {
+      auto cycle = [&](bool zero_x0, bool norm_next) {
         if (d.cycle == MAD_SMOOTHER) {
-          smooth(0, 1);
+          smooth_n(0, 1, norm_next && reuse_level(0));
           return;
         }
         if (d.verbose && c_->comm.rank() == 0) std::printf("\n|--- VCycle n. %u ---|\n", it + 1);
         FlagScope zu(zero_x0_, zero_x0);
+        FlagScope ep(emit_post_, norm_next);
         vcycle_fast();
       };
       auto record = [&](double resNorm) {
@@ -1903,7 +2006,7 @@
       };
       if (fp32_phase) {
         do {
-          cycle(false);
+          cycle(false, true);
           record(residual_impl(0, true, false));
           if (hist.size() >= 2 && relres > MAD_REFINE_FP32_MIN_RATE * hist[hist.size() - 2]) break;
         } while (relres > std::max(d.tolerance, MAD_REFINE_SWITCH_RELRES) && it + 1 < d.max_cycles);
@@ -1921,7 +2024,7 @@
       }
       if (!fp32_phase || (relres > d.tolerance && it < d.max_cycles)) do {
         if (!refine_) {
-          cycle(false);
+          cycle(false, true);
           record(residual_impl(0, true, false));
         } else {
           if (refine_emitted_) {
@@ -1932,7 +2035,7 @@
             to_fp32_rhs(r64_);
             fill(0, MAD_X, 0.0);
           }
-          cycle(refine_emitted_ && zero_sweep_ok());
+          cycle(refine_emitted_ && zero_sweep_ok(), false);
           record(residual64(true));
           if (bt && d.cycle != MAD_SMOOTHER) patch_trace();
         }
@@ -1948,6 +2051,7 @@
       } else {
         HIP_CHECK(hipMemcpyAsync(L0.b, L0.x, sizeof(T) * N, hipMemcpyDeviceToDevice, c_->stream));
         L0.b_halo_ok = L0.brec_ok = false;
+        L0.rc_ok = false;
       }
     }
     HIP_CHECK(hipEventRecord(e1, c_->stream));
@@ -2061,6 +2165,8 @@
   int64_t part_cap_ = 0;
   hipGraphExec_t vgraph_ = nullptr;
   bool vgraph_zu_ = false;
+  bool vgraph_ep_ = false;
+  std::vector<bool> vgraph_exit_rc_;
   std::vector<std::pair<T*, T*>> vgraph_ptrs_;
   std::vector<int> vgraph_seq_;
   bool vgraph_failed_ = false;
@@ -2693,7 +2799,7 @@
             MAD_ERR_INVALID, "gs_kernel must be 0, 1, 3 or 4");
     REQUIRE((d->options & ~(MAD_OPT_EAGER_RANK_VCYCLE | MAD_OPT_OVERLAP_RANK_SWEEP | MAD_OPT_PEER_HALO |
                             MAD_OPT_COARSE_NO_CHAIN | MAD_OPT_BENCHMARK_TRACE |
-                            MAD_OPT_NO_PLACEMENT_TUNE | MAD_OPT_NO_RECORD_B)) == 0,
+                            MAD_OPT_NO_PLACEMENT_TUNE | MAD_OPT_NO_RECORD_B | MAD_OPT_NO_RESIDUAL_REUSE)) == 0,
             MAD_ERR_INVALID, "unknown option bits");
     REQUIRE(d->min_slab_planes >= 0, MAD_ERR_INVALID, "min_slab_planes must be >= 0");
     REQUIRE(d->min_slab_voxels >= 0, MAD_ERR_INVALID, "min_slab_voxels must be >= 0");
```

Result: no change. 121,100 (median of 3 runs) (+1.9%).
